# joeyee/Onet

Measured on AMD Instinct MI355X. Metric: training images/sec (twin 256x256 pass), higher is better.
Workload: dtype f32

## Files before the change

include/onet_hip.h:

```cpp
#ifndef ONET_HIP_H
#define ONET_HIP_H

#include <stdint.h>

#ifdef __cplusplus
extern "C" {
#endif

#define ONET_OK 0
#define ONET_EINVAL (-1)
#define ONET_EHIP (-2)

const char* onet_last_error(void);
int onet_abi_version(void);
int onet_device_info(int* cu_count, int* lds_bytes, int* wave_size, char* arch, int arch_len);

int onet_conv3x3_pack_weights(const float* w, float* wp_fwd, float* wp_dgrad,
                              int Cout, int Cin, void* stream);
int onet_convT2x2_pack_weights(const float* w, float* wp_fwd, float* wp_dgrad,
                               int Cin, int Cout, void* stream);
int onet_convT2x2_pack_weights_fused(const float* w, float* wq, int Cin, int Cout, void* stream);
int onet_convT2x2_fwd(const float* x, int64_t x_bs, const float* wq, const float* bias, float* y, int64_t y_bs,
                      int B, int Cin, int Ct, int h, int w, int Ho, int Wo, int pt, int pl, int operand_bf16,
        void* stream);
int onet_convT2x2_dgrad(const float* dy, int64_t dy_bs, const float* wp_dgrad, float* dx, int64_t dx_bs, int B,
                        int Cin, int Ct, int h, int w, int Ho, int Wo, int pt, int pl, int operand_bf16,
        void* stream);
int64_t onet_convT2x2_dgrad_dbias_ws_bytes(int B, int Ct, int h, int w);
int onet_convT2x2_dgrad_dbias(const float* dy, int64_t dy_bs, const float* wp_dgrad, float* dx, int64_t dx_bs, float* dbias,
                              void* ws, int64_t ws_bytes, int B, int Cin, int Ct, int h, int w, int Ho, int Wo, int pt, int pl, int operand_bf16,
        void* stream);
int64_t onet_convT2x2_wgrad_ws_bytes(int B, int Cin, int Ct, int h, int w);
int onet_convT2x2_wgrad(const float* x, int64_t x_bs, const float* dy, int64_t dy_bs, float* dw, void* ws,
                        int64_t ws_bytes, int B, int Cin, int Ct, int h, int w, int Ho, int Wo, int pt, int pl, int operand_bf16,
        void* stream);
int onet_convT2x2_dbias(const float* dy, int64_t dy_bs, float* dbias, double* scratch, int accumulate, int B,
                        int C, int h, int w, int Ho, int Wo, int pt, int pl, void* stream);

int onet_conv_fwd(const float* x, int64_t x_bs, const float* wp, float* z, int64_t z_bs,
                  float* bn_part, int B, int Cin, int Cout, int H, int W, int ks, void* stream);
int onet_conv_fwd_nparts(int B, int Cout, int H, int W);

int onet_conv3x3_pack_weights_winograd4(const float* w, float* wq_fwd, float* wq_dgrad,
                                        int Cout, int Cin, void* stream);
int onet_conv3x3_winograd4_fwd(const float* x, int64_t x_bs, const float* wq, float* z, int64_t z_bs,
                               int B, int Cin, int Cout, int H, int W, void* stream);
int onet_conv3x3_winograd4_nparts(int B, int H, int W);
int onet_conv3x3_winograd4_fwd_stats(const float* x, int64_t x_bs, const float* wq, float* z, int64_t z_bs,
                                     float* part, int B, int Cin, int Cout, int H, int W, void* stream);
int onet_conv3x3_winograd4_dgrad_bnreduce(const float* dz, int64_t dz_bs, const float* wq_dgrad, float* da,
                                          int64_t da_bs, const float* z_prev, int64_t z_prev_bs,
                                          const float* save_prev, int group_images, float* part2,
                                          int B, int Cdz, int Cda, int H, int W, void* stream);
int onet_convT2x2_fwd_p(const float* x, int64_t x_bs, const float* wq, const float* bias, void* yP, int64_t yP_bs, const void* y_amax,
                        int nparts, int B, int Cin, int Ct, int h, int w, int Ho, int Wo, int pt, int pl, int operand_bf16, void* stream);
int onet_convT2x2_pack_weights_slots(const float* w, void* wP, void* wdP, void* amax_ws, int Cin, int Ct, int nparts, void* stream);
int onet_convT2x2_fwd_slots(const void* xP, int64_t xP_bs, const void* x_amax, const void* wP, const float* bias, void* yP, int64_t yP_bs,
                            const void* y_amax, int nparts, int B, int Cin, int Ct, int h, int w, void* stream);
int onet_convT2x2_dgrad_slots(const void* dyP, int64_t dyP_bs, const void* dy_amax, const void* wdP, float* dx, int64_t dx_bs, int nparts, int B,
                              int Cin, int Ct, int h, int w, void* stream);
int64_t onet_convT2x2_wgrad_slots_ws_bytes(int B, int Cin, int Ct, int h, int w);
int onet_convT2x2_wgrad_slots(const void* xP, int64_t xP_bs, const void* x_amax, const void* dyP, int64_t dyP_bs, const void* dy_amax, float* dw,
                              float* dbias, void* ws, int64_t ws_bytes, int nparts, int B, int Cin, int Ct, int h, int w, void* stream);
int onet_convT2x2_out_bound(const float* w, const float* bias, int Cin, int Ct, const void* x_amax, void* y_amax, void* stream);

int onet_conv3x3_split_pack_weights(const float* w, void* wq_fwd, void* wq_dgrad, void* amax_ws, int Cout, int Cin, int fwd_f16,
                                    int dgrad_f16, void* stream);
int onet_absmax_slots(const float* x, int64_t n, void* slots, void* stream);
int onet_conv3x3_split_conv_amax(const float* x, int64_t x_bs, const void* x_amax, int scale_always, const void* wq, float* z, int64_t z_bs,
                                 float* part, int B, int Cin, int Cout, int H, int W, void* stream);
int onet_conv3x3_split_wgrad_f16(const float* x, int64_t x_bs, const void* x_amax, const float* save, int n_groups, const float* dz,
                                 int64_t dz_bs, const void* dz_amax, float* dw, void* ws, int64_t ws_bytes, int B, int Cin, int Cout,
                                 int H, int W, int accumulate, void* stream);
int onet_conv3x3_split_fwd(const float* x, int64_t x_bs, const void* wq, int wq_f16, float* z, int64_t z_bs, int B, int Cin, int Cout,
                           int H, int W, void* stream);
int onet_conv3x3_split_nparts(int B, int H, int W);
int onet_split_pack_act(const float* x, int64_t x_bs, void* xs, int64_t xs_bs, int B, int C, int H, int W, int f16, float scale,
                        const void* slots ,
                        void* stream);
int onet_conv3x3_split_dgrad_pre_bnreduce(const void* dzs, int64_t dzs_bs, const void* dz_amax, int scale_always, const void* wq, int wq_f16,
                                          float* da, int64_t da_bs, const void* z_prev, int z_bf16, int64_t z_bs, const float* save, int group_images,
                                          float* rec4, void* da_amax, int B, int Cin, int Cout, int H, int W, void* stream);
int onet_conv3x3_split_fwd_pre(const void* xs, int64_t xs_bs, const void* x_amax, int scale_always, const void* x_amax2, int split_ch,
                               const void* wq, int wq_f16, void* z, int z_bf16 , int64_t z_bs,
                               float* part, int B, int Cin, int Cout, int H, int W,
                               void* stream);
int onet_conv3x3_split_dgrad_pre_slots(const void* dzs, int64_t dzs_bs, const void* dz_amax, int scale_always, const void* wq, int wq_f16,
                                       float* da, int64_t da_bs, void* daP, int64_t daP_bs, int ch0, const void* daP_amax, int B, int Cin,
                                       int Cout, int H, int W, void* stream);
int onet_conv3x3_dgrad_bound(const float* w, int Cout, int Cin, int ci0, const void* dz_amax, void* out_slots, void* stream);
int onet_conv3x3_split_fwd_pre_act(const void* xs, int64_t xs_bs, const void* x_amax, int scale_always, const void* x_amax2, int split_ch,
                                   const void* wq, const float* save, void* aP, int64_t aP_bs, const void* aP_slots, void* a_amax, float* a,
                                   int64_t a_bs, int B, int Cin, int Cout, int H, int W, void* stream);
int onet_conv3x3_act_bound(const float* w, int Cout, int Cin, const float* save, const void* x_amax, const void* x_amax2, int split_ch,
                           void* out_slots, void* stream);
int onet_conv3x3_plain16_fwd_pre_act(const void* xs, int64_t xs_bs, const void* wq, const float* save, void* aP, int64_t aP_bs, void* a_amax,
                                     float* a, int64_t a_bs, int B, int Cin, int Cout, int H, int W, void* stream);
int onet_conv3x3_plain16_fwd_pre_head(const void* xs, int64_t xs_bs, const void* wq, const float* save, const float* L, int64_t L_bs, float* V,
                                      int B, int Cin, int Cout, int H, int W, void* stream);
int onet_conv3x3_split_fwd_pre_head(const void* xs, int64_t xs_bs, const void* x_amax, int scale_always, const void* x_amax2, int split_ch,
                                    const void* wq, const float* save, const float* L, int64_t L_bs, float* V, int B, int Cin, int Cout, int H,
                                    int W, void* stream);
int onet_softmax2_labels(const float* Vt, const float* Vd, float* S, int64_t* Y, int B, int HW, void* stream);
int onet_conv3x3_split_pre_nparts(int B, int H, int W);
int onet_conv3x3_split_wgrad_pre_ok(int B, int Cin, int Cout, int H, int W);
int onet_conv3x3_split_wgrad_pre(const void* xs, int64_t xs_bs, const void* x_amax, const void* x_amax2, int split_ch, const void* dzs,
                                 int64_t dzs_bs, const void* dz_amax, int f16, float* dw, void* ws, int64_t ws_bytes, int B, int Cin,
                                 int Cout, int H, int W, int accumulate, void* stream);
int onet_conv3x3_split_fwd_stats(const float* x, int64_t x_bs, const void* wq, int wq_f16, float* z, int64_t z_bs, float* part, int B,
                                 int Cin, int Cout, int H, int W, void* stream);
int onet_conv3x3_split_wgrad_ok(int B, int Cin, int Cout, int H, int W);
int onet_conv3x3_split_fwd_norm(const float* z_prev, int64_t z_bs, const float* save, int n_groups, const void* wq, int wq_f16,
                                const void* x_amax, float* z, int64_t zo_bs, float* part, int B, int Cin, int Cout, int H, int W,
                                void* stream);
int onet_conv3x3_split_wgrad_norm(const float* z_prev, int64_t z_bs, const float* save, int n_groups, const float* dz, int64_t dz_bs,
                                  float* dw, void* ws, int64_t ws_bytes, int B, int Cin, int Cout, int H, int W, int accumulate,
                                  void* stream);
int64_t onet_conv3x3_split_wgrad_ws_bytes(int B, int Cin, int Cout, int H, int W);
int onet_conv3x3_split_wgrad(const float* x, int64_t x_bs, const float* dz, int64_t dz_bs, float* dw, void* ws, int64_t ws_bytes,
                             int B, int Cin, int Cout, int H, int W, int accumulate, void* stream);

int onet_conv3x3_stem_nparts(int B, int Cin, int Cout, int H, int W);
int onet_conv3x3_stem_fwd_stats(const float* x, int64_t x_bs, const float* w, float* z, int64_t z_bs, float* part, int B, int Cin,
                                int Cout, int H, int W, int twin_B, float twin_bias, void* stream);

int onet_conv3x3_winograd4_wgrad_ok(int B, int Cin, int Cout, int H, int W);
int64_t onet_conv3x3_winograd4_wgrad_ws_bytes(int B, int Cin, int Cout, int H, int W);
int onet_conv3x3_winograd4_wgrad(const float* x, int64_t x_bs, const float* dz, int64_t dz_bs, float* dw, void* ws,
                                 int64_t ws_bytes, int B, int Cin, int Cout, int H, int W, int accumulate, void* stream);

int onet_conv_wgrad(const float* x, int64_t x_bs, const float* dz, int64_t dz_bs, float* dw,
                    void* ws, int64_t ws_bytes, int B, int Cin, int Cout, int H, int W, int ks,
                    int out_layout, int accumulate, void* stream);
int onet_conv3x3_stem_wgrad_bn(const float* x, int64_t x_bs, const float* da, int64_t da_bs, const float* z, int64_t z_bs, const float* save,
                               const float* coef, int group_images, float* dw, void* ws, int64_t ws_bytes, int B, int Cin, int Cout, int H,
                               int W, int accumulate, int twin_B, float twin_bias, void* stream);
int64_t onet_conv_wgrad_ws_bytes(int B, int Cin, int Cout, int H, int W, int ks);

int onet_bn_stats_partial(const float* z, int64_t z_bs, float* part, int nparts,
                          int B, int C, int HW, void* stream);
int onet_bn_finalize(const float* part, int nparts, int64_t count, const float* gamma, const float* beta, float* running_mean,
                     float* running_var, float momentum, float eps, float* save, void* act_amax, int C, void* stream);
int onet_bn_finalize_cm(const float* part, int nparts, int64_t c_stride, const float* gamma, const float* beta, float* running_mean,
                        float* running_var, float momentum, float eps, float* save, void* act_amax, int groups, int C, void* stream);
int onet_bn_eval_coeffs(const float* gamma, const float* beta, const float* running_mean,
                        const float* running_var, float eps, float* save, int C, void* stream);
int onet_bn_relu_apply(const void* z, int z_bf16, int64_t z_bs, float* a, int64_t a_bs, const float* save, void* amax, int group_images,
                       int B, int C, int HW, void* stream);
int onet_bn_relu_apply_pool(const float* z, int64_t z_bs, float* a, int64_t a_bs, float* y, int64_t y_bs, const float* save,
                            void* amax, int B, int C, int H, int W, void* stream);

int onet_bn_relu_bwd_reduce(const float* da, int64_t da_bs, const void* z, int z_bf16, int64_t z_bs, const float* save, float* part2,
                            int nparts, void* da_amax, int group_images, int B, int C, int HW, void* stream);
int onet_bn_bwd_finalize(const float* part2, int nparts, int64_t count, float* dgamma, float* dbeta, float* coef, int accumulate,
                         int groups, int C, const float* save, const void* da_amax, void* dz_amax, void* stream);
int onet_bn_bwd_finalize_cm(const float* part2, int nparts, int64_t c_stride, int64_t count, float* dgamma,
                            float* dbeta, float* coef, int accumulate, int C, void* stream);
int onet_bn_relu_bwd_apply(const float* da, int64_t da_bs, const float* z, int64_t z_bs, const float* save, const float* coef,
                           float* dz, int64_t dz_bs, void* amax, int group_images, int B, int C, int HW, void* stream);
int onet_bn_relu_apply_split(const void* z, int z_bf16, int64_t z_bs, void* xs, int64_t xs_bs, float* a, int64_t a_bs, const float* save,
                             const void* act_amax, int nparts, int group_images, int B, int C, int H, int W, void* stream);
int onet_bn_relu_apply_pool_split(const void* z, int z_bf16, int64_t z_bs, void* xs, int64_t xs_bs, float* a, int64_t a_bs, void* ys, int64_t ys_bs,
                                  float* y, int64_t y_bs, const float* save, const void* act_amax, int nparts, int group_images, int B, int C,
                                  int H, int W, void* stream);
int onet_bn_bwd_bound(const float* save, const float* coef, const void* da_amax, int64_t count, void* dz_amax, int C, void* stream);
int onet_bn_relu_bwd_apply_split(const float* da, int64_t da_bs, const void* z, int z_bf16, int64_t z_bs, const float* save, const float* coef,
                                 void* dzs, int64_t dzs_bs, const void* dz_amax, int nparts, int group_images, int B, int C, int H, int W,
                                 void* stream);
int onet_bn_relu_bwd_apply_split_gl(const float* L, int64_t L_bs, const float* g, const float* z, int64_t z_bs, const float* save,
                                    const float* coef, void* dzs, int64_t dzs_bs, const void* dz_amax, int nparts, int group_images, int B, int C,
                                    int H, int W, void* stream);

int onet_maxpool2_fwd(const float* x, int64_t x_bs, float* y, int64_t y_bs,
                      int B, int C, int H, int W, void* stream);
int onet_maxpool2_bwd(const float* x, int64_t x_bs, const float* dy, int64_t dy_bs, const float* add, int64_t add_bs,
                      const float* add2, int64_t add2_bs, float* dx, int64_t dx_bs, int B, int C, int H, int W, int accumulate,
                      void* stream);
int onet_maxpool2_bwd_bn_bands(int H, int W);
int onet_maxpool2_bwd_add_bnreduce(const float* x, int64_t x_bs, const float* dy, int64_t dy_bs, const float* add, int64_t add_bs,
                                        const float* add2, int64_t add2_bs, float* dx, int64_t dx_bs, const void* z, int z_bf16, int64_t z_bs,
                                        const float* save, int group_images, float* part2, void* dx_amax, int B, int C, int H, int W,
                                        void* stream);

int onet_pixel_shuffle2_bias(const float* sub, const float* bias, float* y, int64_t y_bs,
                             int B, int C, int h, int w, int Ho, int Wo, int pt, int pl, void* stream);
int onet_space_to_depth2(const float* dy, int64_t dy_bs, float* sub, float* dbias, double* scratch,
                         int accumulate, int B, int C, int h, int w, int Ho, int Wo, int pt, int pl,
                         void* stream);
int onet_copy_strided(const float* src, int64_t src_bs, float* dst, int64_t dst_bs,
                      int B, int64_t n, void* stream);

int onet_bilinear2x_fwd(const float* x, int64_t x_bs, float* y, int64_t y_bs, int B, int C,
                        int h, int w, int Ho, int Wo, int pt, int pl, void* stream);
int onet_bilinear2x_bwd(const float* dy, int64_t dy_bs, float* dx, int64_t dx_bs, int B, int C,
                        int h, int w, int Ho, int Wo, int pt, int pl, void* stream);

int onet_complement_clip(const float* x, float* y, float bias, int64_t n, void* stream);

int onet_head_softmax_fwd(const float* Lt, int64_t Lt_bs, const float* Ht, int64_t Ht_bs, const float* Ld, int64_t Ld_bs, const float* Hd,
                          int64_t Hd_bs, float* Vt, float* Vd, float* S, float* sLt, float* sLd, const float* h_save_t, const float* h_save_d,
                          int B, int C, int HW, void* stream);
int onet_head_softmax_bwd(const float* dVt, const float* dVd, const float* dS, const float* gsLt, const float* gsLd, const float* S,
                          const float* Lt, int64_t Lt_bs, const float* Ht, int64_t Ht_bs, const float* Ld, int64_t Ld_bs, const float* Hd,
                          int64_t Hd_bs, float* dLt, float* dHt, float* dLd, float* dHd, const float* h_save_t, const float* h_save_d, int B,
                          int C, int HW, void* stream);

int onet_head_grad_map(const float* dVt, const float* dVd, const float* dS, const float* S, float* g, int B, int HW, void* stream);
int onet_head_bwd_reduce(const float* L, int64_t L_bs, const float* z, int64_t z_bs, const float* g, const float* gsLt, const float* gsLd,
                         const float* save, float* dL, float* part2, int nparts, void* da_amax, int B, int C, int HW, void* stream);

int onet_jsd_fwd(const float* L, int64_t L_bs, const float* Si, int64_t Si_bs,
                 const float* Sp, int64_t Sp_bs, float* sums, double* part, float* jsd,
                 int B, int C, int HW, void* stream);
int onet_jsd_nparts(void);
int onet_jsd_bwd(const float* gscale, const float* sums, const float* Si, int64_t Si_bs,
                 const float* Sp, int64_t Sp_bs, float* gL, float* dSi, float* dSp,
                 int B, int HW, void* stream);
int onet_log1pexp_inplace(float* x, int64_t n, void* stream);
int onet_log1pexp_bwd(const float* x, const float* g, float* out, int64_t n, void* stream);

// ... 26 lines not shown
```

onet_amd/csrc/common.hpp:

```cpp
#pragma once
#include <hip/hip_runtime.h>
#include <stdint.h>
#include <atomic>
#include <stdio.h>
#include "../../include/onet_hip.h"

namespace onet {

void set_error(const char* fmt, ...);
int check_launch(const char* what);

#define ONET_REQUIRE(cond, ...)                    \
    do {                                           \
        if (!(cond)) {                             \
            onet::set_error(__VA_ARGS__);          \
            return ONET_EINVAL;                    \
        }                                          \
    } while (0)

static inline hipStream_t as_stream(void* s) { return reinterpret_cast<hipStream_t>(s); }

static inline int cdiv(int64_t a, int64_t b) { return (int)((a + b - 1) / b); }

struct PerDeviceOnce {
    std::atomic<uint64_t> seen{0};
    bool first() {
        int d = 0;
        (void)hipGetDevice(&d);
        const uint64_t bit = 1ull << (d & 63);
        return !(seen.fetch_or(bit, std::memory_order_relaxed) & bit);
    }
};

inline int device_cu_count() {
    static std::atomic<int> cached[64];
    int d = 0;
    (void)hipGetDevice(&d);
    int n = cached[d & 63].load(std::memory_order_relaxed);
    if (n <= 0) {
        if (hipDeviceGetAttribute(&n, hipDeviceAttributeMultiprocessorCount, d) != hipSuccess || n <= 0) n = 256;
        cached[d & 63].store(n, std::memory_order_relaxed);
    }
    return n;
}

__device__ __forceinline__ int xcd_block_id() {
    const int n = gridDim.x, q = n >> 3, r = n & 7, xcd = blockIdx.x & 7, j = blockIdx.x >> 3;
    return (xcd < r ? xcd * (q + 1) : r * (q + 1) + (xcd - r) * q) + j;
}

template <typename T>
__device__ __forceinline__ T wave_sum(T v) {
#pragma unroll
    for (int o = 32; o > 0; o >>= 1) v += __shfl_xor(v, o, 64);
    return v;
}

template <typename T, int NV>
__device__ __forceinline__ void block_sum_256(T (&v)[NV], T* smem ) {
    const int lane = threadIdx.x & 63, wid = threadIdx.x >> 6;
#pragma unroll
    for (int i = 0; i < NV; ++i) v[i] = wave_sum(v[i]);
    if (lane == 0) {
#pragma unroll
        for (int i = 0; i < NV; ++i) smem[wid * NV + i] = v[i];
    }
    __syncthreads();
    if (threadIdx.x == 0) {
#pragma unroll
        for (int i = 0; i < NV; ++i) v[i] = smem[i] + smem[NV + i] + smem[2 * NV + i] + smem[3 * NV + i];
    }
}

__device__ __forceinline__ void split2h_s(float a, float b, float s, unsigned& hi, unsigned& mid) {
    unsigned h, m;
    asm("v_fma_mixlo_f16 %0, %1, %3, 0 op_sel_hi:[0,0,0]\n\tv_fma_mixhi_f16 %0, %2, %3, 0 op_sel_hi:[0,0,0]"
        : "=&v"(h) : "v"(a), "v"(b), "v"(s));
    asm("v_fma_mixlo_f16 %0, %1, %3, -%4 op_sel:[0,0,0] op_sel_hi:[0,0,1]\n\tv_fma_mixhi_f16 %0, %2, %3, -%4 op_sel:[0,0,1] op_sel_hi:[0,0,1]"
        : "=&v"(m) : "v"(a), "v"(b), "v"(s), "v"(h));
    hi = h;
    mid = m;
}

constexpr int AMAX_SLOTS = 64, AMAX_STRIDE = 32;
__device__ __forceinline__ float amax_read(const unsigned* slots) {
    if (!slots) return 0.f;
    unsigned v = slots[(threadIdx.x & (AMAX_SLOTS - 1)) * AMAX_STRIDE];
#pragma unroll
    for (int o = 32; o > 0; o >>= 1) v = max(v, (unsigned)__shfl_xor((int)v, o, 64));
    return __builtin_bit_cast(float, __builtin_amdgcn_readfirstlane(v));
}
__device__ __forceinline__ float amax_scale(float amax, bool always, float& inv) {
    const unsigned bits = __builtin_bit_cast(unsigned, amax);
    const int e = (int)((bits >> 23) & 255u) - 127;
    int k = 0;
    if (bits != 0u && e < 128) k = (always || e >= 15) ? 13 - e : 0;
    k = max(-100, min(100, k));
    inv = __builtin_bit_cast(float, (unsigned)(127 - k) << 23);
    return __builtin_bit_cast(float, (unsigned)(127 + k) << 23);
}

int launch_wgrad_reduce(const float* slab, float* dw, int splitK, int taps, int Cout, int Cin, int out_layout, int accumulate,
                        hipStream_t st);

int convt_gemm_fwd(const float* x, int64_t x_bs, const float* wq, const float* bias, float* y, int64_t y_bs, void* y16, int64_t y16_bs,
                   int B, int Cin, int Ct, int h, int w, int Ho, int Wo, int pt, int pl, int prec, hipStream_t st, int y16_split = 0,
                   const void* out_slots = nullptr);
int convt_out_bound(const float* w, const float* bias, int Cin, int Ct, const void* x_slots, void* out_slots, hipStream_t st);
int64_t convt_gemm_dbias_ws_bytes(int B, int Ct, int h, int w);
int convt_gemm_dgrad(const float* dy, int64_t dy_bs, const float* wd, float* dx, int64_t dx_bs, float* dbias, float* dbias_ws, int B,
                     int Cin, int Ct, int h, int w, int Ho, int Wo, int pt, int pl, int prec, hipStream_t st);
int64_t convt_gemm_wgrad_ws_bytes(int B, int Cin, int Ct, int h, int w);
int convt_gemm_wgrad(const float* x, int64_t x_bs, const float* dy, int64_t dy_bs, float* dw, void* ws, int64_t ws_bytes, int B,
                     int Cin, int Ct, int h, int w, int Ho, int Wo, int pt, int pl, int prec, hipStream_t st);

}
```

onet_amd/csrc/conv_mfma.hip:

```cpp
#include <algorithm>
#include <cstdlib>
#include "common.hpp"

using namespace onet;

typedef float f32x16 __attribute__((ext_vector_type(16)));

__global__ void pack3x3_kernel(const float* __restrict__ w, float* __restrict__ wf,
                               float* __restrict__ wd, int Cout, int Cin) {
    int64_t n = (int64_t)Cout * Cin * 9;
    for (int64_t i = blockIdx.x * (int64_t)blockDim.x + threadIdx.x; i < n;
         i += (int64_t)gridDim.x * blockDim.x) {
        int t = (int)(i % 9);
        int64_t r = i / 9;
        int ci = (int)(r % Cin), co = (int)(r / Cin);
        float v = w[i];
        if (wf) wf[((int64_t)ci * 9 + t) * Cout + co] = v;
        if (wd) wd[((int64_t)co * 9 + (8 - t)) * Cin + ci] = v;
    }
}

__global__ void packT2x2_kernel(const float* __restrict__ w, float* __restrict__ wf,
                                float* __restrict__ wd, float* __restrict__ wq, int Cin, int Cout) {
    int64_t n = (int64_t)Cin * Cout * 4;
// ... 339 lines not shown
__global__ __launch_bounds__(256 * KS, KS == 3 ? 3 : 2) void conv_wgrad_kernel(WgArgs a) {
    using C = WgCfg<KS, PW>;
    constexpr int TAPS = C::TAPS, PAD = C::PAD, PR = C::PR, XR = C::XR, XC = C::XC;
    constexpr int DZ_STRIDE = C::DZ_STRIDE, X_STRIDE = C::X_STRIDE;
    constexpr int TG = KS;
    constexpr int NTAP = TAPS / TG;
    constexpr int NTHR = 256 * TG;
    constexpr int DZ_CSTEP = NTHR / 64;
    constexpr int NDZ = (64 + DZ_CSTEP - 1) / DZ_CSTEP;
    constexpr int ROWS_PER_K = NTHR / PW;
    constexpr int CH_PER_K = ROWS_PER_K / XR;
    constexpr int NXM = (64 + CH_PER_K - 1) / CH_PER_K;
    constexpr int NXH = (KS == 3) ? (64 * XR * 2 + NTHR - 1) / NTHR : 0;

    extern __shared__ __attribute__((aligned(16))) float smem[];
    float* dz_lds = smem;
    float* x_lds = smem + 64 * DZ_STRIDE;

    int bid = xcd_block_id();
    const int tiles = a.ciTiles * a.coTiles;
    const int ks = bid / tiles;
    const int tile = bid % tiles;
    const int ciT = tile % a.ciTiles;
    const int coT = tile / a.ciTiles;
    const int co0 = coT * 64, ci0 = ciT * 64;

    const int tid = threadIdx.x, lane = tid & 63, wid = tid >> 6;
    const int tg = wid >> 2, wm = (wid >> 1) & 1, wn = wid & 1;
    const int l31 = lane & 31, kh = lane >> 5;
    const int HW = a.H * a.W;

    f32x16 acc[NTAP];
#pragma unroll
    for (int t = 0; t < NTAP; ++t)
#pragma unroll
        for (int r = 0; r < 16; ++r) acc[t][r] = 0.f;

    const float* a_ptr = dz_lds + (wm * 32 + l31) * DZ_STRIDE + kh;
    const float* b_ptr = x_lds + (wn * 32 + l31) * X_STRIDE + kh + tg * XC;

    const int dz_c = tid >> 6, dz_p = tid & 63, dz_r = dz_p / PW, dz_col = dz_p % PW;
    const int xm_col = tid % PW, xm_rowid = tid / PW, xm_cp = xm_rowid / XR, xm_r = xm_rowid % XR;
    const bool xm_thread = xm_rowid < CH_PER_K * XR;
    const unsigned dz_kstep = (unsigned)(DZ_CSTEP * HW * 4), xm_kstep = (unsigned)(CH_PER_K * HW * 4);

    float dzv[NDZ], xmv[NXM], xhv[NXH > 0 ? NXH : 1];
    const int nunits = a.B * a.stripsY * a.stripsX;

    auto issue = [&](int u) {
        const bool live = u < nunits;
        const int uu = live ? u : 0;
        const int sx = uu % a.stripsX;
        const int sy = (uu / a.stripsX) % a.stripsY;
        const int b = uu / (a.stripsX * a.stripsY);
        const int y0 = sy * PR, x0 = sx * PW;
        const int HWo = a.Ho * a.Wo;
        const __amdgpu_buffer_rsrc_t dr = make_rsrc(a.dz + (int64_t)b * a.dz_bs, S2D ? (int64_t)a.s2d_Ct * HWo * 4 : (int64_t)a.Cout * HW * 4);
        const __amdgpu_buffer_rsrc_t xr = make_rsrc(a.x + (int64_t)b * a.x_bs, (int64_t)a.Cin * HW * 4);
        {
            const int yy = y0 + dz_r, xx = x0 + dz_col;
            const bool ok = live && yy < a.H && xx < a.W;
            unsigned base, kstep;
            if constexpr (S2D) {
                const int q = co0 / a.s2d_Ct, cc = co0 % a.s2d_Ct + dz_c;
                base = ok ? (unsigned)((cc * HWo + (a.pt + 2 * yy + (q >> 1)) * a.Wo + a.pl + 2 * xx + (q & 1)) * 4) : OOB_OFF;
                kstep = (unsigned)(DZ_CSTEP * HWo * 4);
            } else {
                base = ok ? (unsigned)(((co0 + dz_c) * HW + yy * a.W + xx) * 4) : OOB_OFF;
                kstep = dz_kstep;
            }
#pragma unroll
            for (int k = 0; k < NDZ; ++k)
                dzv[k] = bload(dr, (ok && dz_c + DZ_CSTEP * k < 64) ? base + k * kstep : OOB_OFF);
        }
        {
            const int yy = y0 - PAD + xm_r, xx = x0 + xm_col;
            const bool ok = live && xm_thread && yy >= 0 && yy < a.H && xx < a.W;
            const unsigned base = ok ? (unsigned)(((ci0 + xm_cp) * HW + yy * a.W + xx) * 4) : OOB_OFF;
#pragma unroll
            for (int k = 0; k < NXM; ++k)
                xmv[k] = bload(xr, (xm_cp + CH_PER_K * k < 64) ? base + k * xm_kstep : OOB_OFF);
        }
#pragma unroll
        for (int j = 0; j < NXH; ++j) {
            const int e = tid + NTHR * j;
            const int c = e / (2 * XR), q = e % (2 * XR);
            const int r = q >> 1, side = q & 1;
            const int yy = y0 - PAD + r, xx = side ? x0 + PW : x0 - 1;
            const bool ok = live && e < 64 * XR * 2 && yy >= 0 && yy < a.H && xx >= 0 && xx < a.W;
            xhv[j] = bload(xr, ok ? (unsigned)(((ci0 + c) * HW + yy * a.W + xx) * 4) : OOB_OFF);
        }
    };
    auto commit = [&]() {
#pragma unroll
        for (int k = 0; k < NDZ; ++k)
            if (dz_c + DZ_CSTEP * k < 64) dz_lds[(dz_c + DZ_CSTEP * k) * DZ_STRIDE + dz_p] = dzv[k];
        if (xm_thread) {
#pragma unroll
            for (int k = 0; k < NXM; ++k)
                if (xm_cp + CH_PER_K * k < 64)
                    x_lds[(xm_cp + CH_PER_K * k) * X_STRIDE + xm_r * XC + xm_col + PAD] = xmv[k];
        }
#pragma unroll
        for (int j = 0; j < NXH; ++j) {
            const int e = tid + NTHR * j;
            const int c = e / (2 * XR), q = e % (2 * XR);
            if (e < 64 * XR * 2) x_lds[c * X_STRIDE + (q >> 1) * XC + ((q & 1) ? XC - 1 : 0)] = xhv[j];
        }
    };

    issue(ks);
    for (int u = ks; u < nunits; u += a.splitK) {
        commit();
        __syncthreads();
        issue(u + a.splitK);
        __builtin_amdgcn_sched_barrier(0);
#pragma unroll
        for (int r = 0; r < PR; ++r) {
#pragma unroll
            for (int j = 0; j < PW / 2; ++j) {
                const float av = a_ptr[r * PW + 2 * j];
#pragma unroll
                for (int t = 0; t < NTAP; ++t) {
                    const float bv = b_ptr[r * XC + 2 * j + t];
                    acc[t] = __builtin_amdgcn_mfma_f32_32x32x2f32(av, bv, acc[t], 0, 0, 0);
                }
            }
        }
        __syncthreads();
    }
    float* sl = a.slab + (int64_t)ks * TAPS * a.Cout * a.Cin;
    const int ci = ci0 + wn * 32 + l31;
    if (ci < a.Cin) {
#pragma unroll
        for (int t = 0; t < NTAP; ++t) {
#pragma unroll
            for (int r = 0; r < 16; ++r) {
                const int co = co0 + wm * 32 + (r & 3) + 8 * (r >> 2) + 4 * kh;
                if (co < a.Cout) sl[((int64_t)(tg * NTAP + t) * a.Cout + co) * a.Cin + ci] = acc[t][r];
            }
        }
    }
}

__global__ __launch_bounds__(256) void wgrad_reduce_kernel(const float* __restrict__ slab, float* __restrict__ dw,
                                                           int splitK, int taps, int Cout, int Cin, int out_layout,
                                                           int accumulate) {
    __shared__ float red[256];
    const int64_t n = (int64_t)Cout * Cin;
    const int t = blockIdx.y;
    const int64_t i = (int64_t)blockIdx.x * 64 + (threadIdx.x & 63);
    const int g = threadIdx.x >> 6;
    float s = 0.f;
    if (i < n)
        for (int k = g; k < splitK; k += 4) s += slab[((int64_t)k * taps + t) * n + i];
    red[threadIdx.x] = s;
    __syncthreads();
    if (g == 0 && i < n) {
        s = (red[threadIdx.x] + red[threadIdx.x + 64]) + (red[threadIdx.x + 128] + red[threadIdx.x + 192]);
        const int ci = (int)(i % Cin), co = (int)(i / Cin);
        int64_t o;
        if (out_layout == 0) {
            o = i * taps + t;
        } else {
            const int Ct = Cout / 4, q = co / Ct, cot = co % Ct;
            o = ((int64_t)ci * Ct + cot) * 4 + q;
        }
        dw[o] = accumulate ? dw[o] + s : s;
    }
}

namespace onet {
int launch_wgrad_reduce(const float* slab, float* dw, int splitK, int taps, int Cout, int Cin, int out_layout, int accumulate,
                        hipStream_t st) {
    const int64_t n = (int64_t)Cout * Cin;
    hipLaunchKernelGGL(wgrad_reduce_kernel, dim3((unsigned)cdiv(n, 64), (unsigned)taps), dim3(256), 0, st, slab, dw, splitK,
                       taps, Cout, Cin, out_layout, accumulate);
    return check_launch("wgrad_reduce_kernel");
}
}

constexpr int STEM_ROWS = 32;
template <int CIN, int COG, bool BN = false>
__global__ __launch_bounds__(256) void conv3x3_stem_wgrad_kernel(WgArgs a) {
    constexpr int NV = COG * CIN * 9;
    __shared__ float red[4][NV];
    const int cogs = (a.Cout + COG - 1) / COG;
    const int bandsY = (a.H + STEM_ROWS - 1) / STEM_ROWS;
    const int cg = blockIdx.x % cogs, bb = blockIdx.x / cogs;
    const int b = bb / bandsY, yb = (bb % bandsY) * STEM_ROWS;
    const int tid = threadIdx.x, lane = tid & 63, wid = tid >> 6;
    const int HW = a.H * a.W, W = a.W, H = a.H;
    const bool comp = a.twin_B > 0 && b >= a.twin_B;
    const float* xb = a.x + (int64_t)(comp ? b - a.twin_B : b) * a.x_bs;
    const float* dzb = a.dz + (int64_t)b * a.dz_bs + (int64_t)cg * COG * HW;
    const float* zb = BN ? a.bn_z + (int64_t)b * a.bn_z_bs + (int64_t)cg * COG * HW : nullptr;
    const int y0 = yb + wid * (STEM_ROWS / 4), y1 = min(y0 + STEM_ROWS / 4, H);
    const bool vec = (W & 3) == 0 && (a.dz_bs & 3) == 0 && (reinterpret_cast<uintptr_t>(a.dz) & 15) == 0 &&
                     (!BN || ((a.bn_z_bs & 3) == 0 && (reinterpret_cast<uintptr_t>(a.bn_z) & 15) == 0));
    float bmean[COG], binv[COG], bsc[COG], bsh[COG];
    double bc1[COG], bc2[COG];
    if (BN) {
        const int grp = a.bn_gimg ? b / a.bn_gimg : 0;
        const float* sv = a.bn_save + (int64_t)grp * 4 * a.Cout;
        const float* cf = a.bn_coef ? a.bn_coef + (int64_t)grp * 4 * a.Cout : nullptr;
#pragma unroll
        for (int g = 0; g < COG; ++g) {
            const int c = min(cg * COG + g, a.Cout - 1);
            bmean[g] = sv[c];
            binv[g] = sv[a.Cout + c];
            bsc[g] = sv[2 * a.Cout + c];
            bsh[g] = sv[3 * a.Cout + c];
            bc1[g] = cf ? (double)cf[c] + (double)cf[a.Cout + c] : 0.0;
            bc2[g] = cf ? (double)cf[2 * a.Cout + c] + (double)cf[3 * a.Cout + c] : 0.0;
        }
    }
    float acc[COG][CIN][9];
#pragma unroll
    for (int g = 0; g < COG; ++g)
#pragma unroll
        for (int c = 0; c < CIN; ++c)
#pragma unroll
            for (int t = 0; t < 9; ++t) acc[g][c][t] = 0.f;
    auto in_row = [&](int c, int yy, int x0, float (&r)[6]) __attribute__((always_inline)) {
        const bool rowok = yy >= 0 && yy < H;
        const float* p = xb + (int64_t)c * HW + (int64_t)yy * W;
#pragma unroll
        for (int k = 0; k < 6; ++k) {
            const int xx = x0 - 1 + k;
            const bool ok = rowok && xx >= 0 && xx < W;
            float v = ok ? p[xx] : 0.f;
            if (comp && ok) v = fminf(fmaxf(1.f - v + a.twin_bias, 0.f), 1.f);
            r[k] = v;
        }
    };
    for (int x0 = lane * 4; x0 < W && y0 < y1; x0 += 256) {
        float win[CIN][3][6];
#pragma unroll
        for (int c = 0; c < CIN; ++c) {
            in_row(c, y0 - 1, x0, win[c][1]);
            in_row(c, y0, x0, win[c][2]);
        }
        for (int y = y0; y < y1; ++y) {
#pragma unroll
            for (int c = 0; c < CIN; ++c) {
#pragma unroll
                for (int k = 0; k < 6; ++k) {
                    win[c][0][k] = win[c][1][k];
                    win[c][1][k] = win[c][2][k];
                }
                in_row(c, y + 1, x0, win[c][2]);
            }
#pragma unroll
            for (int g = 0; g < COG; ++g) {
                float gz[4] = {0.f, 0.f, 0.f, 0.f}, zz[4] = {0.f, 0.f, 0.f, 0.f};
                if (cg * COG + g < a.Cout) {
                    const int64_t o = (int64_t)g * HW + (int64_t)y * W + x0;
                    if (vec) {
                        const float4 q = *reinterpret_cast<const float4*>(dzb + o);
                        gz[0] = q.x; gz[1] = q.y; gz[2] = q.z; gz[3] = q.w;
                        if (BN) {
                            const float4 r = *reinterpret_cast<const float4*>(zb + o);
                            zz[0] = r.x; zz[1] = r.y; zz[2] = r.z; zz[3] = r.w;
                        }
                    } else {
#pragma unroll
                        for (int p = 0; p < 4; ++p)
                            if (x0 + p < W) {
                                gz[p] = dzb[o + p];
                                if (BN) zz[p] = zb[o + p];
                            }
                    }
                    if (BN) {
#pragma unroll
                        for (int p = 0; p < 4; ++p) {
                            const double dy = fmaf(zz[p] - bmean[g], bsc[g], bsh[g]) > 0.f ? (double)gz[p] : 0.0;
                            const float v = (float)((double)bsc[g] * (dy - bc1[g] - (((double)zz[p] - (double)bmean[g]) * (double)binv[g]) * bc2[g]));
                            gz[p] = (vec || x0 + p < W) ? v : 0.f;
                        }
                    }
                }
#pragma unroll
                for (int p = 0; p < 4; ++p)
#pragma unroll
                    for (int c = 0; c < CIN; ++c)
#pragma unroll
                        for (int t = 0; t < 9; ++t) acc[g][c][t] = fmaf(gz[p], win[c][t / 3][p + t % 3], acc[g][c][t]);
            }
        }
    }
#pragma unroll
    for (int g = 0; g < COG; ++g)
#pragma unroll
        for (int c = 0; c < CIN; ++c)
#pragma unroll
            for (int t = 0; t < 9; ++t) {
                const float s = wave_sum(acc[g][c][t]);
                if (lane == 0) red[wid][(g * CIN + c) * 9 + t] = s;
            }
    __syncthreads();
    float* sl = a.slab + (int64_t)bb * 9 * a.Cout * CIN;
    for (int i = tid; i < NV; i += 256) {
        const int g = i / (CIN * 9), c = (i / 9) % CIN, t = i % 9;
        const int co = cg * COG + g;
        if (co < a.Cout)
            sl[((int64_t)t * a.Cout + co) * CIN + c] = (red[0][i] + red[1][i]) + (red[2][i] + red[3][i]);
    }
}

template <int KS, int PW, bool S2D = false>
static void launch_wgrad(const WgArgs& a, int64_t blocks, hipStream_t st) {
    using C = WgCfg<KS, PW>;
    auto kern = conv_wgrad_kernel<KS, PW, S2D>;
    static PerDeviceOnce attr_once;
    if (attr_once.first()) {
        (void)hipFuncSetAttribute(reinterpret_cast<const void*>(kern), hipFuncAttributeMaxDynamicSharedMemorySize,
                                  C::LDS_BYTES);
    }
    hipLaunchKernelGGL(kern, dim3((unsigned)blocks), dim3(256 * KS), C::LDS_BYTES, st, a);
}

static void wgrad_plan(int B, int Cin, int Cout, int H, int W, int ks, int& pw, int& splitK,
                       int& stripsX, int& stripsY) {
    pw = (W > 16) ? 32 : 16;
    const int pr = 64 / pw;
    stripsX = cdiv(W, pw);
    stripsY = cdiv(H, pr);
    const int64_t nunits = (int64_t)B * stripsX * stripsY;
    const int64_t tiles = (int64_t)cdiv(Cout, 64) * cdiv(Cin, 64);
    int64_t s = (1024 + tiles - 1) / tiles;
// ... 1 lines not shown
    const int64_t cap = (192ll << 20) / (per > 0 ? per : 1);
    if (s > cap) s = cap;
    if (s > nunits) s = nunits;
    if (s < 1) s = 1;
    splitK = (int)s;
}

extern "C" {

int onet_conv3x3_pack_weights(const float* w, float* wp_fwd, float* wp_dgrad, int Cout, int Cin,
                              void* stream) {
    ONET_REQUIRE(w && Cout > 0 && Cin > 0, "pack3x3: bad args");
    const int64_t n = (int64_t)Cout * Cin * 9;
    hipLaunchKernelGGL(pack3x3_kernel, dim3((unsigned)std::min<int64_t>(cdiv(n, 256), 4096)), dim3(256), 0,
                       as_stream(stream), w, wp_fwd, wp_dgrad, Cout, Cin);
    return check_launch("pack3x3_kernel");
}

int onet_convT2x2_pack_weights(const float* w, float* wp_fwd, float* wp_dgrad, int Cin, int Cout,
                               void* stream) {
    ONET_REQUIRE(w && Cout > 0 && Cin > 0, "packT2x2: bad args");
    const int64_t n = (int64_t)Cout * Cin * 4;
    hipLaunchKernelGGL(packT2x2_kernel, dim3((unsigned)std::min<int64_t>(cdiv(n, 256), 4096)), dim3(256), 0,
                       as_stream(stream), w, wp_fwd, wp_dgrad, (float*)nullptr, Cin, Cout);
    return check_launch("packT2x2_kernel");
}

int onet_convT2x2_pack_weights_fused(const float* w, float* wq, int Cin, int Cout, void* stream) {
    ONET_REQUIRE(w && wq && Cout > 0 && Cin > 0, "packT2x2_fused: bad args");
    const int64_t n = (int64_t)Cout * Cin * 4;
    hipLaunchKernelGGL(packT2x2_kernel, dim3((unsigned)std::min<int64_t>(cdiv(n, 256), 4096)), dim3(256), 0,
                       as_stream(stream), w, (float*)nullptr, (float*)nullptr, wq, Cin, Cout);
    return check_launch("packT2x2_kernel");
}

static bool convt_gemm_enabled() {
    static int on = -1;
    if (on < 0) { const char* e = getenv("ONET_CONVT_GEMM"); on = (e && e[0] == '0') ? 0 : 1; }
    return on != 0;
}

int64_t onet_convT2x2_wgrad_ws_bytes(int B, int Cin, int Ct, int h, int w) {
    return std::max<int64_t>(onet_conv_wgrad_ws_bytes(B, Cin, 4 * Ct, h, w, 1), convt_gemm_wgrad_ws_bytes(B, Cin, Ct, h, w));
}

int onet_convT2x2_fwd(const float* x, int64_t x_bs, const float* wq, const float* bias, float* y, int64_t y_bs,
                      int B, int Cin, int Ct, int h, int w, int Ho, int Wo, int pt, int pl, int operand_bf16, void* stream) {
    ONET_REQUIRE(x && wq && y, "convT2x2_fwd: null pointer");
    ONET_REQUIRE(B > 0 && Cin > 0 && Ct > 0 && h > 0 && w > 0, "convT2x2_fwd: bad shape");
    ONET_REQUIRE(pt >= 0 && pl >= 0 && pt + 2 * h <= Ho && pl + 2 * w <= Wo, "convT2x2_fwd: window outside plane");
    ONET_REQUIRE(x_bs >= (int64_t)Cin * h * w && y_bs >= (int64_t)Ct * Ho * Wo, "convT2x2_fwd: batch stride too small");
    if (convt_gemm_enabled()) {
        const int rc = convt_gemm_fwd(x, x_bs, wq, bias, y, y_bs, nullptr, 0, B, Cin, Ct, h, w, Ho, Wo, pt, pl, operand_bf16, as_stream(stream));
        if (rc <= 0) return rc;
    }
    ConvArgs a{x, x_bs, wq, y, y_bs, nullptr, B, Cin, 4 * Ct, h, w, 0, 0, 0, bias, Ho, Wo, pt, pl};
    return (w > 16) ? launch_fwd<1, 2, 2, 1, 4, 32, 1>(a, as_stream(stream))
                    : launch_fwd<1, 2, 2, 1, 4, 16, 1>(a, as_stream(stream));
}

int onet_convT2x2_fwd_p(const float* x, int64_t x_bs, const float* wq, const float* bias, void* yP, int64_t yP_bs, const void* y_amax,
                        int nparts, int B, int Cin, int Ct, int h, int w, int Ho, int Wo, int pt, int pl, int operand_bf16, void* stream) {
    ONET_REQUIRE(x && wq && yP && B > 0 && Cin > 0 && Ct > 0 && h > 0 && w > 0 && (nparts == 1 || nparts == 2), "convT2x2_fwd_p: bad args");
    return convt_gemm_fwd(x, x_bs, wq, bias, nullptr, 0, yP, yP_bs, B, Cin, Ct, h, w, Ho, Wo, pt, pl, operand_bf16, as_stream(stream),
                          nparts == 1 ? 2 : 1, y_amax);
}

int onet_convT2x2_out_bound(const float* w, const float* bias, int Cin, int Ct, const void* x_amax, void* y_amax, void* stream) {
    ONET_REQUIRE(w && x_amax && y_amax && Cin > 0 && Ct > 0 && (reinterpret_cast<uintptr_t>(w) & 15) == 0, "convT2x2_out_bound: bad args");
    return convt_out_bound(w, bias, Cin, Ct, x_amax, y_amax, as_stream(stream));
}

int onet_convT2x2_dgrad(const float* dy, int64_t dy_bs, const float* wp_dgrad, float* dx, int64_t dx_bs, int B,
                        int Cin, int Ct, int h, int w, int Ho, int Wo, int pt, int pl, int operand_bf16, void* stream) {
    ONET_REQUIRE(dy && wp_dgrad && dx, "convT2x2_dgrad: null pointer");
    ONET_REQUIRE(B > 0 && Cin > 0 && Ct > 0 && h > 0 && w > 0, "convT2x2_dgrad: bad shape");
    ONET_REQUIRE(Ct % CI_T == 0, "convT2x2_dgrad: Ct must be a multiple of %d (use onet_space_to_depth2 + onet_conv_fwd)", CI_T);
    ONET_REQUIRE(pt >= 0 && pl >= 0 && pt + 2 * h <= Ho && pl + 2 * w <= Wo, "convT2x2_dgrad: window outside plane");
    ONET_REQUIRE(dy_bs >= (int64_t)Ct * Ho * Wo && dx_bs >= (int64_t)Cin * h * w, "convT2x2_dgrad: batch stride too small");
    if (convt_gemm_enabled()) {
        const int rc = convt_gemm_dgrad(dy, dy_bs, wp_dgrad, dx, dx_bs, nullptr, nullptr, B, Cin, Ct, h, w, Ho, Wo, pt, pl, operand_bf16, as_stream(stream));
        if (rc <= 0) return rc;
    }
    ConvArgs a{dy, dy_bs, wp_dgrad, dx, dx_bs, nullptr, B, 4 * Ct, Cin, h, w, 0, 0, 0, nullptr, Ho, Wo, pt, pl};
    return (w > 16) ? launch_fwd<1, 2, 2, 1, 4, 32, 2>(a, as_stream(stream))
                    : launch_fwd<1, 2, 2, 1, 4, 16, 2>(a, as_stream(stream));
}

int64_t onet_convT2x2_dgrad_dbias_ws_bytes(int B, int Ct, int h, int w) { return convt_gemm_dbias_ws_bytes(B, Ct, h, w); }

int onet_convT2x2_dgrad_dbias(const float* dy, int64_t dy_bs, const float* wp_dgrad, float* dx, int64_t dx_bs, float* dbias, void* ws,
                              int64_t ws_bytes, int B, int Cin, int Ct, int h, int w, int Ho, int Wo, int pt, int pl, int operand_bf16, void* stream) {
    ONET_REQUIRE(dy && wp_dgrad && dx && dbias && ws, "convT2x2_dgrad_dbias: null pointer");
    ONET_REQUIRE(B > 0 && Cin > 0 && Ct > 0 && h > 0 && w > 0, "convT2x2_dgrad_dbias: bad shape");
    ONET_REQUIRE(dy_bs >= (int64_t)Ct * Ho * Wo && dx_bs >= (int64_t)Cin * h * w, "convT2x2_dgrad_dbias: batch stride too small");
    if (!convt_gemm_enabled() || ws_bytes < convt_gemm_dbias_ws_bytes(B, Ct, h, w)) return 1;
    return convt_gemm_dgrad(dy, dy_bs, wp_dgrad, dx, dx_bs, dbias, (float*)ws, B, Cin, Ct, h, w, Ho, Wo, pt, pl, operand_bf16, as_stream(stream));
}

int onet_conv_fwd_nparts(int B, int Cout, int H, int W) {
    (void)B; (void)Cout; (void)H; (void)W;
    return 0;
}

int onet_conv_fwd(const float* x, int64_t x_bs, const float* wp, float* z, int64_t z_bs, float* bn_part,
                  int B, int Cin, int Cout, int H, int W, int ks, void* stream) {
    ONET_REQUIRE(x && wp && z, "conv_fwd: null pointer");
    ONET_REQUIRE(B > 0 && Cin > 0 && Cout > 0 && H > 0 && W > 0, "conv_fwd: bad shape B=%d Cin=%d Cout=%d H=%d W=%d",
                 B, Cin, Cout, H, W);
    ONET_REQUIRE(ks == 1 || ks == 3, "conv_fwd: ks must be 1 or 3 (got %d)", ks);
    ONET_REQUIRE(bn_part == nullptr, "conv_fwd: fused BN partials not available in this build");
    ONET_REQUIRE(x_bs >= (int64_t)Cin * H * W && z_bs >= (int64_t)Cout * H * W, "conv_fwd: batch stride too small");
    ConvArgs a{x, x_bs, wp, z, z_bs, bn_part, B, Cin, Cout, H, W, 0, 0, 0};
    return ks == 3 ? dispatch_fwd<3>(a, as_stream(stream)) : dispatch_fwd<1>(a, as_stream(stream));
}

static inline bool use_stem_wgrad(int Cin, int ks) { return ks == 3 && Cin <= 4; }
static inline int stem_blocks(int B, int H) { return B * ((H + STEM_ROWS - 1) / STEM_ROWS); }

int64_t onet_conv_wgrad_ws_bytes(int B, int Cin, int Cout, int H, int W, int ks) {
    if (use_stem_wgrad(Cin, ks)) return (int64_t)stem_blocks(B, H) * 9 * Cout * Cin * 4;
    int pw, splitK, sx, sy;
    wgrad_plan(B, Cin, Cout, H, W, ks, pw, splitK, sx, sy);
    return (int64_t)splitK * ks * ks * Cout * Cin * 4;
}

int onet_conv3x3_stem_wgrad_bn(const float* x, int64_t x_bs, const float* da, int64_t da_bs, const float* z, int64_t z_bs, const float* save,
                               const float* coef, int group_images, float* dw, void* ws, int64_t ws_bytes, int B, int Cin, int Cout, int H,
                               int W, int accumulate, int twin_B, float twin_bias, void* stream) {
    ONET_REQUIRE(x && da && z && save && dw && ws, "conv3x3_stem_wgrad_bn: null pointer");
    ONET_REQUIRE(B > 0 && Cin > 0 && Cin <= 4 && Cout > 0 && H > 0 && W > 0 && group_images >= 0 && (group_images == 0 || B % group_images == 0),
                 "conv3x3_stem_wgrad_bn: bad shape (Cin <= 4)");
    WgArgs a{x, x_bs, da, da_bs, (float*)ws, B, Cin, Cout, H, W, 1, cdiv(Cout, 64), 1, 1, 1};
    a.bn_z = z;
    a.bn_z_bs = z_bs;
    a.bn_save = save;
    a.bn_coef = coef;
    a.bn_gimg = group_images;
    ONET_REQUIRE(twin_B == 0 || 2 * twin_B == B, "conv3x3_stem_wgrad_bn: a twin batch holds twin_B = B / 2 images in memory");
    a.twin_B = twin_B;
    a.twin_bias = twin_bias;
    const int nb = stem_blocks(B, H);
    const int64_t need = (int64_t)nb * 9 * Cout * Cin * 4;
    ONET_REQUIRE(ws_bytes >= need, "conv3x3_stem_wgrad_bn: workspace %lld < %lld bytes", (long long)ws_bytes, (long long)need);
    hipStream_t st = as_stream(stream);
    switch (Cin) {
        case 1: hipLaunchKernelGGL((conv3x3_stem_wgrad_kernel<1, 4, true>), dim3(nb * cdiv(Cout, 4)), dim3(256), 0, st, a); break;
        case 2: hipLaunchKernelGGL((conv3x3_stem_wgrad_kernel<2, 2, true>), dim3(nb * cdiv(Cout, 2)), dim3(256), 0, st, a); break;
        case 3: hipLaunchKernelGGL((conv3x3_stem_wgrad_kernel<3, 2, true>), dim3(nb * cdiv(Cout, 2)), dim3(256), 0, st, a); break;
        default: hipLaunchKernelGGL((conv3x3_stem_wgrad_kernel<4, 1, true>), dim3(nb * cdiv(Cout, 1)), dim3(256), 0, st, a); break;
    }
    int rc = check_launch("conv3x3_stem_wgrad_kernel");
    if (rc) return rc;
    const int64_t n = (int64_t)Cout * Cin;
    hipLaunchKernelGGL(wgrad_reduce_kernel, dim3((unsigned)cdiv(n, 64), 9u), dim3(256), 0, st, (const float*)ws, dw, nb, 9, Cout, Cin, 0, accumulate);
    return check_launch("wgrad_reduce_kernel");
}

int onet_conv_wgrad(const float* x, int64_t x_bs, const float* dz, int64_t dz_bs, float* dw, void* ws,
                    int64_t ws_bytes, int B, int Cin, int Cout, int H, int W, int ks, int out_layout,
                    int accumulate, void* stream) {
    ONET_REQUIRE(x && dz && dw && ws, "conv_wgrad: null pointer");
    ONET_REQUIRE(B > 0 && Cin > 0 && Cout > 0 && H > 0 && W > 0, "conv_wgrad: bad shape");
    ONET_REQUIRE(ks == 1 || ks == 3, "conv_wgrad: ks must be 1 or 3 (got %d)", ks);
    ONET_REQUIRE(out_layout == 0 || (out_layout == 1 && ks == 1 && Cout % 4 == 0), "conv_wgrad: bad out_layout");
    WgArgs a{x, x_bs, dz, dz_bs, (float*)ws, B, Cin, Cout, H, W, cdiv(Cin, 64), cdiv(Cout, 64), 1, 1, 1};
    if (use_stem_wgrad(Cin, ks) && out_layout == 0) {
        const int nb = stem_blocks(B, H);
        const int64_t need = (int64_t)nb * 9 * Cout * Cin * 4;
        ONET_REQUIRE(ws_bytes >= need, "conv_wgrad(stem): workspace %lld < %lld bytes", (long long)ws_bytes, (long long)need);
        hipStream_t st = as_stream(stream);
        switch (Cin) {
            case 1: hipLaunchKernelGGL((conv3x3_stem_wgrad_kernel<1, 4>), dim3(nb * cdiv(Cout, 4)), dim3(256), 0, st, a); break;
            case 2: hipLaunchKernelGGL((conv3x3_stem_wgrad_kernel<2, 2>), dim3(nb * cdiv(Cout, 2)), dim3(256), 0, st, a); break;
            case 3: hipLaunchKernelGGL((conv3x3_stem_wgrad_kernel<3, 2>), dim3(nb * cdiv(Cout, 2)), dim3(256), 0, st, a); break;
            default: hipLaunchKernelGGL((conv3x3_stem_wgrad_kernel<4, 1>), dim3(nb * cdiv(Cout, 1)), dim3(256), 0, st, a); break;
        }
        int rc = check_launch("conv3x3_stem_wgrad_kernel");
        if (rc) return rc;
        const int64_t n = (int64_t)Cout * Cin;
        hipLaunchKernelGGL(wgrad_reduce_kernel, dim3((unsigned)cdiv(n, 64), 9u), dim3(256), 0, st,
                           (const float*)ws, dw, nb, 9, Cout, Cin, 0, accumulate);
        return check_launch("wgrad_reduce_kernel");
    }
    int pw;
    wgrad_plan(B, Cin, Cout, H, W, ks, pw, a.splitK, a.stripsX, a.stripsY);
    const int64_t need = (int64_t)a.splitK * ks * ks * Cout * Cin * 4;
    ONET_REQUIRE(ws_bytes >= need, "conv_wgrad: workspace %lld < %lld bytes", (long long)ws_bytes, (long long)need);
    const int64_t blocks = (int64_t)a.splitK * a.ciTiles * a.coTiles;
    hipStream_t st = as_stream(stream);
    if (ks == 3) {
        if (pw == 32) launch_wgrad<3, 32>(a, blocks, st); else launch_wgrad<3, 16>(a, blocks, st);
    } else {
        if (pw == 32) launch_wgrad<1, 32>(a, blocks, st); else launch_wgrad<1, 16>(a, blocks, st);
    }
    int rc = check_launch("conv_wgrad_kernel");
    if (rc) return rc;
    const int64_t n = (int64_t)Cout * Cin;
    hipLaunchKernelGGL(wgrad_reduce_kernel, dim3((unsigned)cdiv(n, 64), (unsigned)(ks * ks)), dim3(256), 0, st,
                       (const float*)ws, dw, a.splitK, ks * ks, Cout, Cin, out_layout, accumulate);
    return check_launch("wgrad_reduce_kernel");
}

int onet_convT2x2_wgrad(const float* x, int64_t x_bs, const float* dy, int64_t dy_bs, float* dw, void* ws,
                        int64_t ws_bytes, int B, int Cin, int Ct, int h, int w, int Ho, int Wo, int pt, int pl, int operand_bf16,
                        void* stream) {
    ONET_REQUIRE(x && dy && dw && ws, "convT2x2_wgrad: null pointer");
    ONET_REQUIRE(B > 0 && Cin > 0 && Ct > 0 && h > 0 && w > 0, "convT2x2_wgrad: bad shape");
    ONET_REQUIRE(Ct % 64 == 0, "convT2x2_wgrad: Ct must be a multiple of 64 (use onet_space_to_depth2 + onet_conv_wgrad)");
    ONET_REQUIRE(pt >= 0 && pl >= 0 && pt + 2 * h <= Ho && pl + 2 * w <= Wo, "convT2x2_wgrad: window outside plane");
    ONET_REQUIRE(dy_bs >= (int64_t)Ct * Ho * Wo && x_bs >= (int64_t)Cin * h * w, "convT2x2_wgrad: batch stride too small");
    if (convt_gemm_enabled()) {
        const int rc = convt_gemm_wgrad(x, x_bs, dy, dy_bs, dw, ws, ws_bytes, B, Cin, Ct, h, w, Ho, Wo, pt, pl, operand_bf16, as_stream(stream));
        if (rc <= 0) return rc;
    }
    const int Cout = 4 * Ct;
    WgArgs a{x, x_bs, dy, dy_bs, (float*)ws, B, Cin, Cout, h, w, cdiv(Cin, 64), cdiv(Cout, 64), 1, 1, 1, Ct, Ho, Wo, pt, pl};
    int pw;
    wgrad_plan(B, Cin, Cout, h, w, 1, pw, a.splitK, a.stripsX, a.stripsY);
    const int64_t need = (int64_t)a.splitK * Cout * Cin * 4;
    ONET_REQUIRE(ws_bytes >= need, "convT2x2_wgrad: workspace %lld < %lld bytes", (long long)ws_bytes, (long long)need);
    const int64_t blocks = (int64_t)a.splitK * a.ciTiles * a.coTiles;
    hipStream_t st = as_stream(stream);
    if (pw == 32) launch_wgrad<1, 32, true>(a, blocks, st); else launch_wgrad<1, 16, true>(a, blocks, st);
    int rc = check_launch("conv_wgrad_kernel");
    if (rc) return rc;
    const int64_t n = (int64_t)Cout * Cin;
    hipLaunchKernelGGL(wgrad_reduce_kernel, dim3((unsigned)cdiv(n, 64), 1u), dim3(256), 0, st, (const float*)ws, dw,
                       a.splitK, 1, Cout, Cin, 1, 0);
    return check_launch("wgrad_reduce_kernel");
}

}
```

onet_amd/csrc/conv_split.hip:

```cpp
#include <algorithm>
#include <cstdlib>
#include "common.hpp"

using namespace onet;

typedef float f32x16 __attribute__((ext_vector_type(16)));
typedef __bf16 bf16x8 __attribute__((ext_vector_type(8)));
typedef __bf16 bf16x2 __attribute__((ext_vector_type(2)));
typedef unsigned int u32x4s __attribute__((ext_vector_type(4)));
typedef float f32x4s __attribute__((ext_vector_type(4)));

namespace {

constexpr unsigned OOB_S = 0x80000000u;

__device__ __forceinline__ __amdgpu_buffer_rsrc_t s_rsrc(const void* base, int64_t bytes) {
    const int n = bytes > 0x7fffffffll ? 0x7fffffff : (int)bytes;
    return __builtin_amdgcn_make_buffer_rsrc(const_cast<void*>(base), 0, n, 0x00020000);
}
__device__ __forceinline__ void split2(float a, float b, unsigned& hi, unsigned& mid) {
    const bf16x2 h = {(__bf16)a, (__bf16)b};
    const bf16x2 m = {(__bf16)(a - (float)h[0]), (__bf16)(b - (float)h[1])};
    hi = __builtin_bit_cast(unsigned, h);
    mid = __builtin_bit_cast(unsigned, m);
}

typedef _Float16 f16x2 __attribute__((ext_vector_type(2)));
typedef _Float16 f16x8 __attribute__((ext_vector_type(8)));
__device__ __forceinline__ unsigned pack2bf(float lo, float hi) {
    const bf16x2 v = {(__bf16)lo, (__bf16)hi};
    return __builtin_bit_cast(unsigned, v);
}
__device__ __forceinline__ void split2h(float a, float b, unsigned& hi, unsigned& mid) {
    const f16x2 h = {(_Float16)a, (_Float16)b};
    const f16x2 m = {(_Float16)(a - (float)h[0]), (_Float16)(b - (float)h[1])};
    hi = __builtin_bit_cast(unsigned, h);
    mid = __builtin_bit_cast(unsigned, m);
}

__global__ void absmax_slots_kernel(const float* __restrict__ v, int64_t n, unsigned* __restrict__ slots) {
    float m = 0.f;
    for (int64_t i = blockIdx.x * (int64_t)blockDim.x + threadIdx.x; i < n; i += (int64_t)gridDim.x * blockDim.x) m = fmaxf(m, fabsf(v[i]));
#pragma unroll
    for (int o = 32; o > 0; o >>= 1) m = fmaxf(m, __shfl_xor(m, o, 64));
    if ((threadIdx.x & 63) == 0)
        atomicMax(slots + ((blockIdx.x * (blockDim.x >> 6) + (threadIdx.x >> 6)) & (AMAX_SLOTS - 1)) * AMAX_STRIDE, __builtin_bit_cast(unsigned, m));
}

__global__ void pack3x3_split_kernel(const float* __restrict__ w, __bf16* __restrict__ wq, int Cout, int Cin, int which, int f16,
                                     const unsigned* __restrict__ wamax) {
    const int K = which == 0 ? Cin : ((Cout + 15) / 16) * 16, N = which == 0 ? Cout : Cin;
    const int64_t n = (int64_t)K * 9 * N;
    const int nparts = f16 == 2 ? 1 : 2;
    float winv = 1.f;
    const float wscale = f16 == 1 ? amax_scale(amax_read(wamax), true, winv) : 1.f;
    if (blockIdx.x == 0 && threadIdx.x == 0) {
        float* meta = reinterpret_cast<float*>(wq + nparts * n);
        meta[0] = wscale;
        meta[1] = winv;
    }
    for (int64_t i = blockIdx.x * (int64_t)blockDim.x + threadIdx.x; i < n; i += (int64_t)gridDim.x * blockDim.x) {
        const int kc = (int)(i & 7);
        int64_t r = i >> 3;
        const int nn = (int)(r % N);
        r /= N;
        const int half = (int)(r & 1);
        r >>= 1;
        const int t = (int)(r % 9), kg = (int)(r / 9);
        const int k = kg * 16 + half * 8 + kc;
        float v = 0.f;
        if (which == 0) v = w[((int64_t)nn * Cin + k) * 9 + t];
        else if (k < Cout) v = w[((int64_t)k * Cin + nn) * 9 + (8 - t)];
        const int64_t per_chunk_part = (int64_t)9 * 2 * N * 8;
        const int64_t within = i - (int64_t)kg * per_chunk_part;
        if (f16 == 2) {
            wq[(int64_t)kg * per_chunk_part + within] = (__bf16)v;
        } else if (f16) {
            _Float16* wh = reinterpret_cast<_Float16*>(wq);
            const float vs = v * wscale;
            const _Float16 hi = (_Float16)vs;
            wh[((int64_t)kg * 2 + 0) * per_chunk_part + within] = hi;
            wh[((int64_t)kg * 2 + 1) * per_chunk_part + within] = (_Float16)(vs - (float)hi);
        } else {
            const __bf16 hi = (__bf16)v;
            wq[((int64_t)kg * 2 + 0) * per_chunk_part + within] = hi;
            wq[((int64_t)kg * 2 + 1) * per_chunk_part + within] = (__bf16)(v - (float)hi);
        }
    }
}

struct SpArgs {
    const float* x;
    int64_t x_bs;
    const __bf16* wq;
    float* z;
    int64_t z_bs;
    int B, Cin, Cout, H, W, tilesX, tilesY, coTiles;
    float* stats;
    const float* nsave;
    int nimg;
    const unsigned* x_amax;
    int x_always;
};

#define ONET_SP_DPP_ADD(v, ctrl, rmask) \
    v += __builtin_bit_cast(float, __builtin_amdgcn_update_dpp(0, __builtin_bit_cast(int, v), ctrl, rmask, 0xf, false))
__device__ __forceinline__ float sp_half_sum(float v) {
    ONET_SP_DPP_ADD(v, 0x128, 0xf);
    ONET_SP_DPP_ADD(v, 0x124, 0xf);
    ONET_SP_DPP_ADD(v, 0x122, 0xf);
    ONET_SP_DPP_ADD(v, 0x121, 0xf);
    ONET_SP_DPP_ADD(v, 0x142, 0xa);
    return v;
}
#undef ONET_SP_DPP_ADD

struct SpCfg {
    static constexpr int NW = 8, NT = 2, TW = 32, CO_T = 64;
    static constexpr int ROWS = NW * NT;
    static constexpr int IN_ROWS = ROWS + 2, IN_COLS = TW + 2;
    static constexpr int NPIX = IN_ROWS * IN_COLS;
    static constexpr int NROUND = (NPIX + 31) / 32;
    static constexpr int NPIXP = NROUND * 32;
    static constexpr int W_PART = 9 * 2 * CO_T;
    static constexpr int W_SLOTS = 2 * W_PART;
    static constexpr int NWI = (W_SLOTS + 511) / 512;
    static constexpr int IN_PART = 2 * NPIXP;
    static constexpr int BUF_SLOTS = W_SLOTS + 2 * IN_PART;
    static constexpr int LDS_BYTES = 2 * BUF_SLOTS * 16;
    static constexpr int NB = (NT - 1) + 3;
};


__device__ __forceinline__ void sp_tile_range(int ntiles, int& t_first, int& t_end, int& t_stride) {
    const int xcd = blockIdx.x & 7, j = blockIdx.x >> 3;
    const int q = ntiles >> 3, r = ntiles & 7;
    const int start = xcd * q + min(xcd, r);
    t_stride = (gridDim.x + 7 - xcd) >> 3;
    t_first = start + j;
    t_end = start + q + (xcd < r ? 1 : 0);
}
struct SpTile {
    int co0, tx, ty, b, y0, x0;
};
__device__ __forceinline__ SpTile sp_tile(int v, int coTiles, int tilesX, int tilesY) {
    SpTile t;
    t.co0 = (v % coTiles) * SpCfg::CO_T;
    v /= coTiles;
    t.tx = v % tilesX;
    v /= tilesX;
    t.ty = v % tilesY;
    t.b = v / tilesY;
    t.y0 = t.ty * SpCfg::ROWS;
    t.x0 = t.tx * SpCfg::TW;
    return t;
}

template <bool ST, bool NORM, bool F16>
__global__ __launch_bounds__(512, 2) void conv3x3_split_kernel(SpArgs a) {
    using C = SpCfg;
    constexpr int NT = C::NT, IN_COLS = C::IN_COLS, NWI = C::NWI, CO_T = C::CO_T, NPIXP = C::NPIXP, NB = C::NB;
    constexpr int BUF = C::BUF_SLOTS, W_PART = C::W_PART, IN_PART = C::IN_PART, TW = C::TW;
    extern __shared__ __attribute__((aligned(16))) unsigned char smem_s[];
    u32x4s* lds = reinterpret_cast<u32x4s*>(smem_s);

    int t_first, t_end, t_stride;
    sp_tile_range(a.tilesX * a.tilesY * a.B * a.coTiles, t_first, t_end, t_stride);
    if (t_first >= t_end) return;

    const int tid = threadIdx.x, lane = tid & 63, wn = __builtin_amdgcn_readfirstlane(tid >> 6);
    const int l31 = lane & 31, kh = lane >> 5;
    const int HW = a.H * a.W;
    const int nchunks = a.Cin >> 4;
    float xs_inv = 1.f;
    const float xs_scale = F16 ? amax_scale(amax_read(a.x_amax), a.x_always != 0, xs_inv) : 1.f;
    const float acc_scale = F16 ? xs_inv * reinterpret_cast<const float*>(a.wq + (int64_t)a.Cin * 2 * 9 * a.Cout)[1] : 1.f;

    const __amdgpu_buffer_rsrc_t wr = s_rsrc(a.wq, (int64_t)a.Cin * 2 * 9 * a.Cout * 2);
    const unsigned in_step = (unsigned)(16 * HW * 4), w_step = (unsigned)(2 * 9 * 2 * a.Cout * 16);
    const unsigned plane = (unsigned)(HW * 4);

    unsigned in_off, w_off[NWI];
    const int role = wn < 5 ? 0 : (wn < 7 ? 1 : 2);
    const int it = role == 0 ? tid : tid - 320;
    const int it_h = role == 0 ? it / 144 : it / 36;
    const int it_r = role == 0 ? (it % 144) / 8 : (it % 36) / 2;
    const int it_g = role == 0 ? (it & 7) : (it & 1);
    const bool it_ok = role == 0 ? it < 288 : (role == 1 && it < 72);
    __amdgpu_buffer_rsrc_t xr;
    int st_tile = t_first, st_chunk = 0, st_b = 0;
    unsigned cin_bytes = 0, cw_bytes = 0;
    float* const coef = reinterpret_cast<float*>(lds + 2 * BUF) + (ST ? C::NW * 64 * 2 : 0);
    float pend_cv = 0.f;
    bool pend_keep = false;
    auto setup_stage = [&]() __attribute__((always_inline)) {
        const bool live = st_tile < t_end;
        const auto [co0, tx, ty, b, y0, x0] = sp_tile(live ? st_tile : t_first, a.coTiles, a.tilesX, a.tilesY);
        st_b = b;
        xr = s_rsrc(a.x + (int64_t)b * a.x_bs, (int64_t)a.Cin * HW * 4);
        {
            const int yy = y0 - 1 + it_r;
            const int xx = role == 0 ? x0 + 4 * it_g : (it_g ? x0 + TW : x0 - 1);
            const bool ok = live && it_ok && yy >= 0 && yy < a.H && xx >= 0 && xx < a.W;
            in_off = ok ? (unsigned)(((it_h * 8) * HW + yy * a.W + xx) * 4) : OOB_S;
        }
#pragma unroll
        for (int k = 0; k < NWI; ++k) {
            const int i = tid + 512 * k;
            const int co = i & (CO_T - 1), pth = i >> 6;
            const bool ok = live && (i < C::W_SLOTS) && (co0 + co < a.Cout);
            w_off[k] = ok ? (unsigned)((pth * a.Cout + co0 + co) * 16) : OOB_S;
        }
    };
    auto advance = [&]() __attribute__((always_inline)) {
        ++st_chunk;
        cin_bytes += in_step;
        cw_bytes += w_step;
        if (st_chunk == nchunks) {
            st_chunk = 0;
            cin_bytes = cw_bytes = 0;
            st_tile += t_stride;
            setup_stage();
        }
    };

    u32x4s xin[8];
    u32x4s wv[NWI];
    auto issue_in = [&](int c0, int c1) __attribute__((always_inline)) {
        if (NORM && c0 == 0) {
            pend_keep = in_off != OOB_S;
            if (wn == 7 && lane < 48) {
                const int k = lane >> 4, row = k == 0 ? 0 : k + 1;
                pend_cv = st_tile < t_end ? a.nsave[(int64_t)((st_b / a.nimg) * 4 + row) * a.Cin + st_chunk * 16 + (lane & 15)] : 0.f;
            }
        }
        if (role == 0) {
#pragma unroll
            for (int c = 0; c < 8; ++c)
                if (c >= c0 && c < c1) xin[c] = __builtin_amdgcn_raw_buffer_load_b128(xr, in_off, (int)(cin_bytes + c * plane), 0);
        } else if (role == 1) {
// ... 1755 lines not shown
extern "C" {

int onet_conv3x3_split_wgrad_ok(int B, int Cin, int Cout, int H, int W) {
    if (B <= 0 || Cin <= 0 || Cout <= 0 || H <= 0) return 0;
    if (W >= 64) return (W & 3) == 0 ? 1 : 0;
    return ((W == 32 || W == 16) && B % (64 / W) == 0) ? 1 : 0;
}

int64_t onet_conv3x3_split_wgrad_ws_bytes(int B, int Cin, int Cout, int H, int W) {
    int splitK, tx;
    split_wgrad_plan(B, Cin, Cout, H, W, splitK, tx);
    return (int64_t)splitK * (split_wgrad_cot(Cout, W) == 64 ? 2 : 1) * 9 * Cout * Cin * 4;
}

static int split_wgrad_impl(const float* x, int64_t x_bs, const float* dz, int64_t dz_bs, float* dw, void* ws, int64_t ws_bytes,
                            int B, int Cin, int Cout, int H, int W, int accumulate, void* stream, const float* nsave, int n_groups,
                            int f16 = 0, const unsigned* x_amax = nullptr, const unsigned* dz_amax = nullptr) {
    ONET_REQUIRE(x && dz && dw && ws, "conv3x3_split_wgrad: null pointer");
    ONET_REQUIRE(!nsave || ((n_groups == 1 || n_groups == 2) && B % n_groups == 0),
                 "conv3x3_split_wgrad_norm: one or two statistics groups of equal size");
    ONET_REQUIRE(onet_conv3x3_split_wgrad_ok(B, Cin, Cout, H, W),
                 "conv3x3_split_wgrad: needs W >= 64 with W %% 4 == 0, or W = 32 / 16 with B %% (64 / W) == 0 (use onet_conv3x3_winograd_wgrad)");
    ONET_REQUIRE((x_bs & 3) == 0 && (dz_bs & 3) == 0 && (reinterpret_cast<uintptr_t>(x) & 15) == 0 && (reinterpret_cast<uintptr_t>(dz) & 15) == 0,
                 "conv3x3_split_wgrad: 16-byte aligned image rows required");
    ONET_REQUIRE(x_bs >= (int64_t)Cin * H * W && dz_bs >= (int64_t)Cout * H * W, "conv3x3_split_wgrad: batch stride too small");
    ONET_REQUIRE((int64_t)std::max(Cin, Cout) * H * W * 4 < (1ll << 31), "conv3x3_split_wgrad: image exceeds the 2 GiB buffer-resource range");
    const int G = split_wgrad_group(W);
    ONET_REQUIRE(G == 1 || (((int64_t)(B - 1) * x_bs + (int64_t)Cin * H * W) * 4 < (1ll << 31) &&
                            ((int64_t)(B - 1) * dz_bs + (int64_t)Cout * H * W) * 4 < (1ll << 31)),
                 "conv3x3_split_wgrad: on maps narrower than 64 pixels the whole batch must lie within the 2 GiB buffer-resource range");
    const int COT = split_wgrad_cot(Cout, W), slabs = COT == 64 ? 2 : 1;
    ONET_REQUIRE(!f16 || dz_amax, "conv3x3_split_wgrad_f16: the fp16 parts need the magnitude slots of dz");
    SwArgs a{x, x_bs, dz, dz_bs, (float*)ws, B, Cin, Cout, H, W, cdiv(Cin, 64), cdiv(Cout, COT), 1, 1, nsave, nsave ? B / n_groups : B,
             x_amax, dz_amax};
    split_wgrad_plan(B, Cin, Cout, H, W, a.splitK, a.tilesX);
    const int64_t need = (int64_t)a.splitK * slabs * 9 * Cout * Cin * 4;
    ONET_REQUIRE(ws_bytes >= need, "conv3x3_split_wgrad: workspace %lld < %lld bytes", (long long)ws_bytes, (long long)need);
    const int64_t blocks = (int64_t)a.splitK * a.ciTiles * a.coTiles;
    const dim3 grid((unsigned)blocks), blk(512);
    hipStream_t st = as_stream(stream);
#define ONET_SW_LAUNCH(G_, COT_)                                                                                      \
    do {                                                                                                              \
        if (nsave && f16) hipLaunchKernelGGL((conv3x3_split_wgrad_kernel<G_, COT_, true, true>), grid, blk, 0, st, a);    \
        else if (nsave) hipLaunchKernelGGL((conv3x3_split_wgrad_kernel<G_, COT_, true, false>), grid, blk, 0, st, a);     \
        else if (f16) hipLaunchKernelGGL((conv3x3_split_wgrad_kernel<G_, COT_, false, true>), grid, blk, 0, st, a);       \
        else hipLaunchKernelGGL((conv3x3_split_wgrad_kernel<G_, COT_, false, false>), grid, blk, 0, st, a);               \
    } while (0)
    if (COT == 128) {
        if (G == 1) ONET_SW_LAUNCH(1, 128);
        else ONET_SW_LAUNCH(2, 128);
    } else if (G == 1) ONET_SW_LAUNCH(1, 64);
    else if (G == 2) ONET_SW_LAUNCH(2, 64);
    else ONET_SW_LAUNCH(4, 64);
#undef ONET_SW_LAUNCH
    int rc = check_launch("conv3x3_split_wgrad_kernel");
    if (rc) return rc;
    return launch_wgrad_reduce((const float*)ws, dw, a.splitK * slabs, 9, Cout, Cin, 0, accumulate, as_stream(stream));
}

int onet_conv3x3_split_wgrad(const float* x, int64_t x_bs, const float* dz, int64_t dz_bs, float* dw, void* ws, int64_t ws_bytes,
                             int B, int Cin, int Cout, int H, int W, int accumulate, void* stream) {
    return split_wgrad_impl(x, x_bs, dz, dz_bs, dw, ws, ws_bytes, B, Cin, Cout, H, W, accumulate, stream, nullptr, 0);
}

int onet_conv3x3_split_wgrad_norm(const float* z_prev, int64_t z_bs, const float* save, int n_groups, const float* dz, int64_t dz_bs,
                                  float* dw, void* ws, int64_t ws_bytes, int B, int Cin, int Cout, int H, int W, int accumulate,
                                  void* stream) {
    ONET_REQUIRE(save, "conv3x3_split_wgrad_norm: null pointer");
    return split_wgrad_impl(z_prev, z_bs, dz, dz_bs, dw, ws, ws_bytes, B, Cin, Cout, H, W, accumulate, stream, save, n_groups);
}

int onet_conv3x3_split_wgrad_pre_ok(int B, int Cin, int Cout, int H, int W) {
    if (B <= 0 || Cin <= 0 || Cout <= 0 || H <= 0 || (Cin % 8) || (Cout % 8)) return 0;
    if (W >= 64) return 1;
    return ((W == 32 && B % 2 == 0) || (W == 16 && B % 4 == 0)) ? 1 : 0;
}

int onet_conv3x3_split_wgrad_pre(const void* xs, int64_t xs_bs, const void* x_amax, const void* x_amax2, int split_ch, const void* dzs,
                                 int64_t dzs_bs, const void* dz_amax, int f16, float* dw, void* ws, int64_t ws_bytes, int B, int Cin,
                                 int Cout, int H, int W, int accumulate, void* stream) {
    ONET_REQUIRE(split_ch >= 0 && split_ch < Cin && (split_ch % 64) == 0, "conv3x3_split_wgrad_pre: split_ch must be a multiple of 64 inside Cin");
    ONET_REQUIRE(xs && dzs && dw && ws, "conv3x3_split_wgrad_pre: null pointer");
    ONET_REQUIRE(onet_conv3x3_split_wgrad_pre_ok(B, Cin, Cout, H, W),
                 "conv3x3_split_wgrad_pre: needs Cin, Cout %% 8 == 0 and W >= 64, or W = 32 / 16 with a batch multiple of 2 / 4");
    ONET_REQUIRE((xs_bs & 3) == 0 && (dzs_bs & 3) == 0 && (reinterpret_cast<uintptr_t>(xs) & 15) == 0 && (reinterpret_cast<uintptr_t>(dzs) & 15) == 0,
                 "conv3x3_split_wgrad_pre: 16-byte aligned slots required");
    ONET_REQUIRE(xs_bs >= (int64_t)Cin * H * W / (f16 == 2 ? 2 : 1) && dzs_bs >= (int64_t)Cout * H * W / (f16 == 2 ? 2 : 1),
                 "conv3x3_split_wgrad_pre: batch stride too small");
    ONET_REQUIRE((int64_t)std::max(Cin, Cout) * H * W * 4 < (1ll << 31), "conv3x3_split_wgrad_pre: image exceeds the 2 GiB buffer-resource range");
    const int G = split_wgrad_group(W);
    ONET_REQUIRE(G == 1 || (((int64_t)(B - 1) * xs_bs + (int64_t)Cin * H * W) * 4 < (1ll << 31) &&
                            ((int64_t)(B - 1) * dzs_bs + (int64_t)Cout * H * W) * 4 < (1ll << 31)),
                 "conv3x3_split_wgrad_pre: on 32-pixel maps the whole batch must lie within the 2 GiB buffer-resource range");
    const int COT = split_wgrad_cot(Cout, W), slabs = COT == 64 ? 2 : 1;
    SwPreArgs a{xs, xs_bs, dzs, dzs_bs, (float*)ws, B, Cin, Cout, H, W, cdiv(Cin, 64), cdiv(Cout, COT), 1, 1, (const unsigned*)x_amax,
                (const unsigned*)dz_amax, (const unsigned*)x_amax2, split_ch};
    split_wgrad_plan(B, Cin, Cout, H, W, a.splitK, a.tilesX);
    const int64_t need = (int64_t)a.splitK * slabs * 9 * Cout * Cin * 4;
    ONET_REQUIRE(ws_bytes >= need, "conv3x3_split_wgrad_pre: workspace %lld < %lld bytes", (long long)ws_bytes, (long long)need);
    const int64_t blocks = (int64_t)a.splitK * a.ciTiles * a.coTiles;
    const dim3 grid((unsigned)blocks), blk(512);
    hipStream_t st = as_stream(stream);
    const int np = f16 == 2 ? 1 : 2, pxp = G == 4 ? 76 : SWP_PXP;
    const int lds = (4 * ((np * 8 * pxp + 63) / 64 * 64) + 2 * ((np * (COT / 8) * pxp + 63) / 64 * 64)) * 16;
#define ONET_SWP_LAUNCH(G_, COT_, F_)                                                                              \
    do {                                                                                                           \
        auto kern = conv3x3_wgrad_pre16_kernel<G_, COT_, F_>;                                                      \
        static PerDeviceOnce once;                                                                                 \
        if (once.first()) (void)hipFuncSetAttribute(reinterpret_cast<const void*>(kern), hipFuncAttributeMaxDynamicSharedMemorySize, lds); \
        hipLaunchKernelGGL(kern, grid, blk, lds, st, a);                                                           \
    } while (0)
#define ONET_SWP_F(G_, COT_) do { if (f16 == 2) ONET_SWP_LAUNCH(G_, COT_, 2); else if (f16) ONET_SWP_LAUNCH(G_, COT_, 1); else ONET_SWP_LAUNCH(G_, COT_, 0); } while (0)
    if (COT == 128) {
        if (G == 1) ONET_SWP_F(1, 128);
        else if (G == 2) ONET_SWP_F(2, 128);
        else ONET_SWP_F(4, 128);
    } else if (G == 1) ONET_SWP_F(1, 64);
    else if (G == 2) ONET_SWP_F(2, 64);
    else ONET_SWP_F(4, 64);
#undef ONET_SWP_F
#undef ONET_SWP_LAUNCH
    int rc = check_launch("conv3x3_split_wgrad_pre_kernel");
    if (rc) return rc;
    return launch_wgrad_reduce((const float*)ws, dw, a.splitK * slabs, 9, Cout, Cin, 0, accumulate, as_stream(stream));
}

int onet_conv3x3_split_pack_weights(const float* w, void* wq_fwd, void* wq_dgrad, void* amax_ws, int Cout, int Cin, int fwd_f16,
                                    int dgrad_f16, void* stream) {
    ONET_REQUIRE(w && (wq_fwd || wq_dgrad), "conv3x3_split_pack_weights: null pointer");
    ONET_REQUIRE(amax_ws || !(fwd_f16 == 1 || dgrad_f16 == 1), "conv3x3_split_pack_weights: the fp16 packs need the 8 KB magnitude workspace");
    if (fwd_f16 == 1 || dgrad_f16 == 1) {
        (void)hipMemsetAsync(amax_ws, 0, AMAX_SLOTS * AMAX_STRIDE * sizeof(unsigned), as_stream(stream));
        const int64_t nw = (int64_t)Cout * Cin * 9;
        hipLaunchKernelGGL(absmax_slots_kernel, dim3((unsigned)std::min<int64_t>((nw + 1023) / 1024, 1024)), dim3(256), 0, as_stream(stream), w,
                           nw, (unsigned*)amax_ws);
        int rc0 = check_launch("absmax_slots_kernel");
        if (rc0) return rc0;
    }
    ONET_REQUIRE(Cout > 0 && Cin > 0, "conv3x3_split_pack_weights: bad shape");
    ONET_REQUIRE(!wq_fwd || (Cin % 16) == 0, "conv3x3_split_pack_weights: the forward pack needs Cin %% 16 == 0");
    const int64_t n = (int64_t)std::max(Cin, ((Cout + 15) / 16) * 16) * 9 * std::max(Cin, Cout);
    const int blocks = (int)std::min<int64_t>((n + 255) / 256, 8192);
    if (wq_fwd) {
        hipLaunchKernelGGL(pack3x3_split_kernel, dim3(blocks), dim3(256), 0, as_stream(stream), w, (__bf16*)wq_fwd, Cout, Cin, 0, fwd_f16,
                           (const unsigned*)amax_ws);
        int rc = check_launch("pack3x3_split_kernel");
        if (rc) return rc;
    }
    if (wq_dgrad) hipLaunchKernelGGL(pack3x3_split_kernel, dim3(blocks), dim3(256), 0, as_stream(stream), w, (__bf16*)wq_dgrad, Cout, Cin, 1,
                                     dgrad_f16, (const unsigned*)amax_ws);
    return check_launch("pack3x3_split_kernel");
}

int onet_conv3x3_split_fwd(const float* x, int64_t x_bs, const void* wq, int wq_f16, float* z, int64_t z_bs, int B, int Cin, int Cout,
                           int H, int W, void* stream) {
    return split_fwd(x, x_bs, wq, z, z_bs, B, Cin, Cout, H, W, stream, nullptr, wq_f16);
}

int onet_absmax_slots(const float* x, int64_t n, void* slots, void* stream) {
    ONET_REQUIRE(x && slots && n > 0, "absmax_slots: bad args");
    hipLaunchKernelGGL(absmax_slots_kernel, dim3((unsigned)std::min<int64_t>((n + 1023) / 1024, 4096)), dim3(256), 0, as_stream(stream), x, n,
                       (unsigned*)slots);
    return check_launch("absmax_slots_kernel");
}

int onet_conv3x3_split_conv_amax(const float* x, int64_t x_bs, const void* x_amax, int scale_always, const void* wq, float* z, int64_t z_bs,
                                 float* part, int B, int Cin, int Cout, int H, int W, void* stream) {
    return split_fwd(x, x_bs, wq, z, z_bs, B, Cin, Cout, H, W, stream, part, 1, nullptr, 0, (const unsigned*)x_amax, scale_always);
}

int onet_conv3x3_split_wgrad_f16(const float* x, int64_t x_bs, const void* x_amax, const float* save, int n_groups, const float* dz,
                                 int64_t dz_bs, const void* dz_amax, float* dw, void* ws, int64_t ws_bytes, int B, int Cin, int Cout,
                                 int H, int W, int accumulate, void* stream) {
    return split_wgrad_impl(x, x_bs, dz, dz_bs, dw, ws, ws_bytes, B, Cin, Cout, H, W, accumulate, stream, save, save ? n_groups : 0, 1,
                            (const unsigned*)x_amax, (const unsigned*)dz_amax);
}

int onet_conv3x3_split_fwd_norm(const float* z_prev, int64_t z_bs, const float* save, int n_groups, const void* wq, int wq_f16,
                                const void* x_amax, float* z, int64_t zo_bs, float* part, int B, int Cin, int Cout, int H, int W,
                                void* stream) {
    ONET_REQUIRE(save, "conv3x3_split_fwd_norm: null pointer");
    return split_fwd(z_prev, z_bs, wq, z, zo_bs, B, Cin, Cout, H, W, stream, part, wq_f16, save, n_groups, (const unsigned*)x_amax);
}

int onet_split_pack_act(const float* x, int64_t x_bs, void* xs, int64_t xs_bs, int B, int C, int H, int W, int f16, float scale,
                        const void* slots, void* stream) {
    ONET_REQUIRE(x && xs, "split_pack_act: null pointer");
    ONET_REQUIRE(B > 0 && C > 0 && (C % 8) == 0 && H > 0 && W > 0, "split_pack_act: C must be a multiple of 8");
    ONET_REQUIRE((reinterpret_cast<uintptr_t>(xs) & 15) == 0 && (xs_bs & 3) == 0, "split_pack_act: 16-byte aligned slots required");
    const int64_t n = (int64_t)B * (C / 8) * H * W;
    const int blocks = (int)std::min<int64_t>((n + 255) / 256, 1 << 20);
    hipLaunchKernelGGL(split_pack_act_kernel, dim3(blocks), dim3(256), 0, as_stream(stream), x, x_bs, (unsigned*)xs, xs_bs, B, C / 8, H, W,
                       f16, scale, (const unsigned*)slots);
    return check_launch("split_pack_act_kernel");
}

static int pre_operand_checks(const char* entry, const void* xs, int64_t xs_bs, int wq_f16, int Cin, int Cout, int H, int W) {
    ONET_REQUIRE((Cin % (wq_f16 == 2 ? 32 : 16)) == 0, "%s: Cin must be a multiple of 16 (32 for plain bf16 operands)", entry);
    ONET_REQUIRE((xs_bs & 3) == 0 && (reinterpret_cast<uintptr_t>(xs) & 15) == 0, "%s: 16-byte aligned slots required", entry);
    ONET_REQUIRE(xs_bs >= (int64_t)Cin * H * W / (wq_f16 == 2 ? 2 : 1), "%s: batch stride too small", entry);
    ONET_REQUIRE((int64_t)(Cin + 32) * H * W * 4 < (1ll << 31) && (int64_t)(Cin + 32) * 2 * 9 * Cout * 2 < (1ll << 31),
                 "%s: operand exceeds the 2 GiB buffer-resource range", entry);
    ONET_REQUIRE(W != 16 || xs_bs * 4 + (int64_t)Cin * H * W * 4 < (1ll << 31), "%s: image pair exceeds the buffer-resource range", entry);
    return 0;
}

int onet_conv3x3_split_pre_nparts(int B, int H, int W) {
    if (W == 16) return (B > 0 && (B % 2) == 0 && (H % 16) == 0) ? (B / 2) * (H / 16) : 0;
    return split_nparts(B, H, W);
}

int onet_conv3x3_split_fwd_pre(const void* xs, int64_t xs_bs, const void* x_amax, int scale_always, const void* x_amax2, int split_ch,
                               const void* wq, int wq_f16, void* z, int z_bf16, int64_t z_bs, float* part, int B, int Cin, int Cout, int H, int W,
                               void* stream) {
    ONET_REQUIRE(!z_bf16 || (wq_f16 == 2 && (z_bs & 3) == 0 && (reinterpret_cast<uintptr_t>(z) & 7) == 0),
                 "conv3x3_split_fwd_pre: a bf16 output goes with plain bf16 operands (wq_f16 == 2), 8-byte aligned rows");
    ONET_REQUIRE(split_ch >= 0 && split_ch < Cin && (split_ch % 32) == 0, "conv3x3_split_fwd_pre: split_ch must be a multiple of 32 inside Cin");
    ONET_REQUIRE(xs && wq && z, "conv3x3_split_fwd_pre: null pointer");
    ONET_REQUIRE(B > 0 && Cin > 0 && Cout > 0 && H > 0 && (W > 16 || (W == 16 && (B % 2) == 0 && (H % 16) == 0)),
                 "conv3x3_split_fwd_pre: bad shape (maps wider than 16 pixels, or exactly 16 wide with an even batch and H %% 16 == 0)");
    ONET_REQUIRE(wq_f16 != 2 || (W % 4) == 0, "conv3x3_split_fwd_pre: plain bf16 operands need W %% 4 == 0");
    if (const int rc = pre_operand_checks("conv3x3_split_fwd_pre", xs, xs_bs, wq_f16, Cin, Cout, H, W)) return rc;
    ONET_REQUIRE(z_bs >= (int64_t)Cout * H * W, "conv3x3_split_fwd_pre: batch stride too small");
    SpPreArgs a{xs, xs_bs, (const __bf16*)wq, (float*)z, z_bs, B, Cin, Cout, H, W, 0, 0, 0, part, (const unsigned*)x_amax, scale_always,
                (const unsigned*)x_amax2, split_ch};
    a.z16 = z_bf16 ? 1 : 0;
    if (part) ONET_REQUIRE(onet_conv3x3_split_pre_nparts(B, H, W) > 0, "conv3x3_split_fwd_pre: statistics need a map made of full 16 x 32 tiles");
    hipStream_t st = as_stream(stream);
    if (W == 16) {
        if (wq_f16 == 2) return part ? launch_split_pre<true, 2, true>(a, st) : launch_split_pre<false, 2, true>(a, st);
        if (wq_f16) return part ? launch_split_pre<true, 1, true>(a, st) : launch_split_pre<false, 1, true>(a, st);
        return part ? launch_split_pre<true, 0, true>(a, st) : launch_split_pre<false, 0, true>(a, st);
    }
    if (wq_f16 == 2) return part ? launch_split_pre<true, 2, false>(a, st) : launch_split_pre<false, 2, false>(a, st);
    if (wq_f16) return part ? launch_split_pre<true, 1, false>(a, st) : launch_split_pre<false, 1, false>(a, st);
    return part ? launch_split_pre<true, 0, false>(a, st) : launch_split_pre<false, 0, false>(a, st);
}

int onet_conv3x3_split_dgrad_pre_bnreduce(const void* dzs, int64_t dzs_bs, const void* dz_amax, int scale_always, const void* wq, int wq_f16,
                                          float* da, int64_t da_bs, const void* z_prev, int z_bf16, int64_t z_bs, const float* save, int group_images,
                                          float* rec4, void* da_amax, int B, int Cin, int Cout, int H, int W, void* stream) {
    ONET_REQUIRE(dzs && wq && da && z_prev && save && rec4, "conv3x3_split_dgrad_pre_bnreduce: null pointer");
    if (onet_conv3x3_split_pre_nparts(B, H, W) <= 0 || (W != 16 && (W % 32)) || (Cout % 16)) return 1;
    if (W == 16 && ((group_images % 2) || wq_f16 != 2)) return 1;
    if (Cin / (wq_f16 == 2 ? 32 : 16) < 4) return 1;
    ONET_REQUIRE(B > 0 && Cin > 0 && Cout > 0, "conv3x3_split_dgrad_pre_bnreduce: bad shape");
    ONET_REQUIRE(group_images >= 0 && (group_images == 0 || B % group_images == 0), "conv3x3_split_dgrad_pre_bnreduce: bad statistics groups");
    if (const int rc = pre_operand_checks("conv3x3_split_dgrad_pre_bnreduce", dzs, dzs_bs, wq_f16, Cin, Cout, H, W)) return rc;
    ONET_REQUIRE((z_bs & 3) == 0 && (reinterpret_cast<uintptr_t>(z_prev) & (z_bf16 ? 7 : 15)) == 0 && (da_bs & 3) == 0 && (reinterpret_cast<uintptr_t>(da) & 15) == 0,
                 "conv3x3_split_dgrad_pre_bnreduce: 16-byte aligned rows required");
    ONET_REQUIRE(da_bs >= (int64_t)Cout * H * W && z_bs >= (int64_t)Cout * H * W, "conv3x3_split_dgrad_pre_bnreduce: batch stride too small");
    SpPreArgs a{dzs, dzs_bs, (const __bf16*)wq, da, da_bs, B, Cin, Cout, H, W, 0, 0, 0, nullptr, (const unsigned*)dz_amax, scale_always, nullptr, 0};
    a.rd_z = (const float*)z_prev;
    a.rd_z16 = z_bf16 ? 1 : 0;
    a.rd_z_bs = z_bs;
    a.rd_save = save;
    a.rd_gimg = group_images;
    a.rd_rec = rec4;
    a.rd_amax = (unsigned*)da_amax;
    hipStream_t st = as_stream(stream);
    if (W == 16) return launch_split_pre<false, 2, true, true>(a, st);
    if (wq_f16 == 2) return launch_split_pre<false, 2, false, true>(a, st);
    return wq_f16 ? launch_split_pre<false, 1, false, true>(a, st) : launch_split_pre<false, 0, false, true>(a, st);
}

int onet_conv3x3_split_dgrad_pre_slots(const void* dzs, int64_t dzs_bs, const void* dz_amax, int scale_always, const void* wq, int wq_f16,
                                       float* da, int64_t da_bs, void* daP, int64_t daP_bs, int ch0, const void* daP_amax, int B, int Cin,
                                       int Cout, int H, int W, void* stream) {
    ONET_REQUIRE(dzs && wq && da && daP && (daP_amax || wq_f16 == 2) && (wq_f16 == 1 || wq_f16 == 2), "conv3x3_split_dgrad_pre_slots: bad args");
    ONET_REQUIRE(B > 0 && Cin > 0 && Cout > 0 && H > 0 && W >= 32 && (W % 32) == 0 && (H % 16) == 0,
                 "conv3x3_split_dgrad_pre_slots: maps made of full 16 x 32 tiles");
    ONET_REQUIRE(ch0 > 0 && ch0 < Cout && (ch0 % 64) == 0 && (Cout % 64) == 0, "conv3x3_split_dgrad_pre_slots: ch0 and Cout must be multiples of 64");
    if (const int rc = pre_operand_checks("conv3x3_split_dgrad_pre_slots", dzs, dzs_bs, wq_f16, Cin, Cout, H, W)) return rc;
    ONET_REQUIRE((daP_bs & 3) == 0 && (reinterpret_cast<uintptr_t>(daP) & 15) == 0, "conv3x3_split_dgrad_pre_slots: 16-byte aligned slots required");
    ONET_REQUIRE(da_bs >= (int64_t)ch0 * H * W && daP_bs >= (int64_t)(Cout - ch0) * H * W / (wq_f16 == 2 ? 2 : 1),
                 "conv3x3_split_dgrad_pre_slots: batch stride too small");
    SpPreArgs a{dzs, dzs_bs, (const __bf16*)wq, da, da_bs, B, Cin, Cout, H, W, 0, 0, 0, nullptr, (const unsigned*)dz_amax, scale_always, nullptr, 0};
    a.zP = daP;
    a.zP_bs = daP_bs;
    a.zP_ch0 = ch0;
    a.zP_slots = (const unsigned*)daP_amax;
    if (wq_f16 == 2) return launch_split_pre<false, 2, false>(a, as_stream(stream));
    return launch_split_pre<false, 1, false>(a, as_stream(stream));
}

int onet_conv3x3_split_fwd_pre_act(const void* xs, int64_t xs_bs, const void* x_amax, int scale_always, const void* x_amax2, int split_ch,
                                   const void* wq, const float* save, void* aP, int64_t aP_bs, const void* aP_slots, void* a_amax, float* a,
                                   int64_t a_bs, int B, int Cin, int Cout, int H, int W, void* stream) {
    ONET_REQUIRE(xs && wq && save && aP && aP_slots, "conv3x3_split_fwd_pre_act: null pointer");
    ONET_REQUIRE(B > 0 && Cin > 0 && Cout > 0 && H > 0 && W > 0, "conv3x3_split_fwd_pre_act: bad shape");
    if (W < 32 || (W % 32) || (H % 16) || (Cin % 16) || (Cout % 64)) return 1;
    ONET_REQUIRE(split_ch >= 0 && split_ch < Cin && (split_ch % 32) == 0, "conv3x3_split_fwd_pre_act: split_ch must be a multiple of 32 inside Cin");
    if (const int rc = pre_operand_checks("conv3x3_split_fwd_pre_act", xs, xs_bs, 1, Cin, Cout, H, W)) return rc;
    ONET_REQUIRE((aP_bs & 3) == 0 && (reinterpret_cast<uintptr_t>(aP) & 15) == 0, "conv3x3_split_fwd_pre_act: 16-byte aligned slots required");
    ONET_REQUIRE(aP_bs >= (int64_t)Cout * H * W && (!a || a_bs >= (int64_t)Cout * H * W), "conv3x3_split_fwd_pre_act: batch stride too small");
    SpPreArgs p{xs, xs_bs, (const __bf16*)wq, nullptr, 0, B, Cin, Cout, H, W, 0, 0, 0, nullptr, (const unsigned*)x_amax, scale_always,
                (const unsigned*)x_amax2, split_ch};
    p.zP = aP;
    p.zP_bs = aP_bs;
    p.zP_ch0 = 0;
    p.zP_slots = (const unsigned*)aP_slots;
    p.act_save = save;
    p.act_amax = (unsigned*)a_amax;
    p.act_a = a;
    p.act_a_bs = a_bs;
    return launch_split_pre<false, 1, false, false, true>(p, as_stream(stream));
// ... 131 lines not shown
```

onet_amd/csrc/convt_gemm.hip:

```cpp
#include <algorithm>
#include <cstdlib>
#include "common.hpp"

using namespace onet;

typedef float f32x16 __attribute__((ext_vector_type(16)));
typedef float f32x4g __attribute__((ext_vector_type(4)));
typedef float f32x2g __attribute__((ext_vector_type(2)));
typedef int i32x4g __attribute__((ext_vector_type(4)));
typedef __bf16 bf16x8g __attribute__((ext_vector_type(8)));
typedef __bf16 bf16x2g __attribute__((ext_vector_type(2)));
typedef unsigned u32x4g __attribute__((ext_vector_type(4)));

namespace {

__device__ __forceinline__ i32x4g g_rsrc(const void* base, int64_t bytes) {
    const uint64_t p = reinterpret_cast<uint64_t>(base);
    i32x4g r;
    r.x = (int)(p & 0xffffffffu);
    r.y = (int)((p >> 32) & 0xffffu);
    r.z = bytes > 0x7fffffffll ? 0x7fffffff : (int)bytes;
    r.w = 0x00020000;
    return r;
}
// ... 269 lines not shown
#pragma unroll
            for (int u = 0; u < 2; ++u) {
                const int p = p0 + wc * 64 + u * 32 + l31;
#pragma unroll
                for (int r = 0; r < 16; ++r) {
                    const int ci = m0 + wr * 64 + t * 32 + (r & 3) + 8 * (r >> 2) + 4 * kh;
                    xb[(int64_t)ci * hw + p] = acc[t][u][r];
                }
            }
    }
}

constexpr int KP = 32;
constexpr int WA_F = 128 * KP;
constexpr int WB_F = 64 * 2 * KP;

template <int PREC = 0>
__global__ __launch_bounds__(256, 2) void convt_wgrad_gemm_kernel(GArgs g) {
    __shared__ __attribute__((aligned(16))) float lds[2 * (WA_F + WB_F)];
    int bid = xcd_block_id();
    const int tiles = g.mTiles * g.nTiles;
    const int ks = bid / tiles, tile = bid % tiles;
    const int mt = tile % g.mTiles, nt = tile / g.mTiles;
    const int tid = threadIdx.x, lane = tid & 63, wid = __builtin_amdgcn_readfirstlane(tid >> 6);
    const int wr = wid >> 1, wc = wid & 1, l31 = lane & 31, kh = lane >> 5;
    const int hw = g.h * g.w;
    const int ci0 = mt * 128, c0 = nt * 32;
    const int ch0 = ks * g.chunksPerSplit;
    const int nchunks_all = (int)(((int64_t)g.B * hw) / KP);
    const int ch1 = min(ch0 + g.chunksPerSplit, nchunks_all);

    auto issue = [&](int chunk, int buf) __attribute__((always_inline)) {
        const int64_t pix = (int64_t)chunk * KP;
        const int b = (int)(pix / hw), p0 = (int)(pix % hw);
        const i32x4g rx = g_rsrc(g.a + (int64_t)b * g.a_bs, (int64_t)g.Cin * hw * 4);
        const i32x4g rd = g_rsrc(g.b + (int64_t)b * g.b_bs, (int64_t)g.Ct * g.HoWo * 4);
        const unsigned la = g_lds(lds) + (unsigned)(buf * (WA_F + WB_F) * 4), lb = la + WA_F * 4;
#pragma unroll
        for (int j = 0; j < 4; ++j) {
            const int p = 4 * wid + j;
            {
                const int row = 8 * p + (lane >> 3), src = (lane & 7) ^ ((row >> 1) & 7);
                g_dma16(rx, la + p * 1024, (unsigned)((((int64_t)(ci0 + row)) * hw + p0 + src * 4) * 4));
            }
            {
                const int row = 4 * p + (lane >> 4), src = (lane & 15) ^ (row & 7);
                const int px = p0 + 2 * src, y = px / g.w, x = px % g.w;
                g_dma16(rd, lb + p * 1024,
                        (unsigned)((((int64_t)(c0 + (row >> 1))) * g.HoWo + (int64_t)(2 * y + (row & 1)) * g.Wo + 2 * x) * 4));
            }
        }
    };

    f32x16 acc[2][2];
#pragma unroll
    for (int t = 0; t < 2; ++t)
#pragma unroll
        for (int u = 0; u < 2; ++u)
#pragma unroll
            for (int r = 0; r < 16; ++r) acc[t][u][r] = 0.f;

    int a_row[2], b_row[2];
#pragma unroll
    for (int t = 0; t < 2; ++t) a_row[t] = wr * 64 + t * 32 + l31;
#pragma unroll
    for (int u = 0; u < 2; ++u) b_row[u] = (wc * 64 + u * 32 + l31) >> 1;
    const bool dj = (l31 & 1) != 0;

    if (ch0 < ch1) {
        issue(ch0, 0);
        asm volatile("s_waitcnt vmcnt(0)" ::: "memory");
        __syncthreads();
    }
    for (int c = ch0; c < ch1; ++c) {
        const int buf = (c - ch0) & 1;
        const bool more = c + 1 < ch1;
        const float* A = lds + buf * (WA_F + WB_F);
        const float* Bt = A + WA_F;
        if constexpr (PREC != 0) {
            if (more) issue(c + 1, buf ^ 1);
#pragma unroll
            for (int g2 = 0; g2 < KP / 16; ++g2) {
                float af[2][8], bf[2][8];
#pragma unroll
                for (int h2 = 0; h2 < 2; ++h2) {
                    const int gg = 2 * g2 + h2;
#pragma unroll
                    for (int t = 0; t < 2; ++t) {
                        const f32x4g v = *reinterpret_cast<const f32x4g*>(A + a_row[t] * KP + (((2 * gg + kh) ^ ((a_row[t] >> 1) & 7)) << 2));
#pragma unroll
                        for (int i = 0; i < 4; ++i) af[t][4 * h2 + i] = v[i];
                    }
#pragma unroll
                    for (int u = 0; u < 2; ++u)
#pragma unroll
                        for (int e = 0; e < 2; ++e) {
                            const f32x4g v = *reinterpret_cast<const f32x4g*>(Bt + b_row[u] * (2 * KP) + (((4 * gg + 2 * kh + e) ^ (b_row[u] & 7)) << 2));
                            bf[u][4 * h2 + 2 * e] = dj ? v[1] : v[0];
                            bf[u][4 * h2 + 2 * e + 1] = dj ? v[3] : v[2];
                        }
                }
                g_mma16<PREC>(af, bf, acc);
            }
        } else {
#pragma unroll
        for (int gg = 0; gg < KP / 8; ++gg) {
            if (gg == 0 && more) issue(c + 1, buf ^ 1);
            f32x4g a4[2], b4[2][2];
#pragma unroll
            for (int t = 0; t < 2; ++t)
                a4[t] = *reinterpret_cast<const f32x4g*>(A + a_row[t] * KP + (((2 * gg + kh) ^ ((a_row[t] >> 1) & 7)) << 2));
#pragma unroll
            for (int u = 0; u < 2; ++u)
#pragma unroll
                for (int e = 0; e < 2; ++e)
                    b4[u][e] = *reinterpret_cast<const f32x4g*>(Bt + b_row[u] * (2 * KP) + (((4 * gg + 2 * kh + e) ^ (b_row[u] & 7)) << 2));
#pragma unroll
            for (int tt = 0; tt < 4; ++tt) {
                float bv[2];
#pragma unroll
                for (int u = 0; u < 2; ++u) {
                    const f32x4g v = b4[u][tt >> 1];
                    bv[u] = dj ? v[(tt & 1) * 2 + 1] : v[(tt & 1) * 2];
                }
#pragma unroll
                for (int t = 0; t < 2; ++t)
#pragma unroll
                    for (int u = 0; u < 2; ++u) acc[t][u] = __builtin_amdgcn_mfma_f32_32x32x2f32(a4[t][tt], bv[u], acc[t][u], 0, 0, 0);
            }
        }
        }
        asm volatile("s_waitcnt vmcnt(0)" ::: "memory");
        __syncthreads();
    }

    float* slab = g.out + (int64_t)ks * g.Cin * 4 * g.Ct;
#pragma unroll
    for (int t = 0; t < 2; ++t)
#pragma unroll
        for (int u = 0; u < 2; ++u) {
            const int m = 4 * c0 + wc * 64 + u * 32 + l31;
#pragma unroll
            for (int r = 0; r < 16; ++r) {
                const int ci = ci0 + wr * 64 + t * 32 + (r & 3) + 8 * (r >> 2) + 4 * kh;
                slab[(int64_t)ci * 4 * g.Ct + m] = acc[t][u][r];
            }
        }
}

__global__ __launch_bounds__(256) void convt_wgrad_reduce_kernel(const float* __restrict__ slab, float* __restrict__ dw, int splitK,
                                                                 int64_t n4, int accumulate) {
    const int64_t i = blockIdx.x * (int64_t)blockDim.x + threadIdx.x;
    if (i >= n4) return;
    float4 s = reinterpret_cast<const float4*>(slab)[i];
    for (int k = 1; k < splitK; ++k) {
        const float4 v = reinterpret_cast<const float4*>(slab)[(int64_t)k * n4 + i];
        s.x += v.x; s.y += v.y; s.z += v.z; s.w += v.w;
    }
    if (accumulate) {
        const float4 o = reinterpret_cast<float4*>(dw)[i];
        s.x += o.x; s.y += o.y; s.z += o.z; s.w += o.w;
    }
    reinterpret_cast<float4*>(dw)[i] = s;
}

__global__ __launch_bounds__(256) void convt_dbias_reduce_kernel(const float* __restrict__ part, float* __restrict__ db, int ntiles, int Ct) {
    const int c = blockIdx.x;
    double s = 0.0;
    for (int t = threadIdx.x; t < ntiles; t += 256) s += (double)part[(int64_t)t * Ct + c];
    __shared__ double sh[4];
    double v[1] = {s};
    block_sum_256<double, 1>(v, sh);
    if (threadIdx.x == 0) db[c] = (float)v[0];
}


typedef _Float16 f16x8g __attribute__((ext_vector_type(8)));

struct SArgs {
    const void* wP;
    const void* xP;
    int64_t x_bs;
    const float* bias;
    void* yP;
    int64_t y_bs;
    const unsigned* x_slots;
    const unsigned* y_slots;
    int B, Cin, Ct, h, w, mTiles, nTiles;
};

template <int NP>
__device__ __forceinline__ f32x16 s_mfma(u32x4g a, u32x4g b, f32x16 c) {
    if constexpr (NP == 2) return __builtin_amdgcn_mfma_f32_32x32x16_f16(__builtin_bit_cast(f16x8g, a), __builtin_bit_cast(f16x8g, b), c, 0, 0, 0);
    else return __builtin_amdgcn_mfma_f32_32x32x16_bf16(__builtin_bit_cast(bf16x8g, a), __builtin_bit_cast(bf16x8g, b), c, 0, 0, 0);
}

constexpr int SLOT_NST = 2, SLOT_OCC = 4;
template <int N>
__device__ __forceinline__ void slot_wait() {
    asm volatile("s_waitcnt vmcnt(%0)" ::"n"(N) : "memory");
}

template <int NP>
__global__ __launch_bounds__(256, SLOT_OCC) void convt_slot_fwd_kernel(SArgs g) {
    constexpr int KS = 4 / NP;
    constexpr int TILE = KS * NP * 128;
    constexpr int NPC = TILE / 256;
    constexpr int NST = SLOT_NST;
    __shared__ __attribute__((aligned(16))) u32x4g lds[NST * 2 * TILE];
    const int bid = xcd_block_id();
    const int mt = bid % g.mTiles;
    const int nt = bid / g.mTiles;
    const int tid = threadIdx.x, lane = tid & 63, wid = __builtin_amdgcn_readfirstlane(tid >> 6);
    const int wr = wid >> 1, wc = wid & 1, l31 = lane & 31, kh = lane >> 5;
    const int hw = g.h * g.w, M = 4 * g.Ct;
    const int m0 = mt * 128, n0 = nt * 128;
    const int b = n0 / hw, p0 = n0 % hw;

    const i32x4g ra = g_rsrc(g.wP, (int64_t)(g.Cin / 8) * NP * M * 16);
    const i32x4g rb = g_rsrc(reinterpret_cast<const unsigned*>(g.xP) + (int64_t)b * g.x_bs, (int64_t)(g.Cin / 8) * hw * NP * 16);
    unsigned a_off[NPC], b_off[NPC];
#pragma unroll
    for (int j = 0; j < NPC; ++j) {
        const int s = (wid * NPC + j) * 64 + lane;
        const int c8 = s / (NP * 128), part = (s >> 7) % NP, r = s & 127;
        a_off[j] = (unsigned)((((int64_t)c8 * NP + part) * M + m0 + r) * 16);
        const int p = p0 + r, i = p / g.w, jx = p % g.w;
        b_off[j] = (unsigned)(((((int64_t)c8 * g.h + i) * NP + part) * g.w + jx) * 16);
    }
    const unsigned a_step = (unsigned)((int64_t)KS * NP * M * 16), b_step = (unsigned)((int64_t)KS * hw * NP * 16);
    const unsigned lds0 = (unsigned)(uintptr_t)(__attribute__((address_space(3))) u32x4g*)lds;
    auto issue = [&](int chunk, int buf) __attribute__((always_inline)) {
        const unsigned la = lds0 + (unsigned)(buf * 2 * TILE * 16), lb = la + TILE * 16;
#pragma unroll
        for (int j = 0; j < NPC; ++j) g_dma16(ra, la + (wid * NPC + j) * 1024, a_off[j] + chunk * a_step);
#pragma unroll
        for (int j = 0; j < NPC; ++j) g_dma16(rb, lb + (wid * NPC + j) * 1024, b_off[j] + chunk * b_step);
    };
    static_assert(NST >= 2 && NST <= 4, "the tail waits below cover rings of two to four stages");

    f32x16 acc[2][2];
#pragma unroll
    for (int t = 0; t < 2; ++t)
#pragma unroll
        for (int u = 0; u < 2; ++u)
#pragma unroll
            for (int r = 0; r < 16; ++r) acc[t][u][r] = 0.f;

    const int nch = g.Cin / (8 * KS);
#pragma unroll
    for (int c = 0; c < NST - 1; ++c) issue(c, c);
    float undo = 1.f;
    if constexpr (NP == 2) {
        const float* meta = reinterpret_cast<const float*>(reinterpret_cast<const _Float16*>(g.wP) + (int64_t)NP * g.Cin * M);
        float x_inv;
        (void)amax_scale(amax_read(g.x_slots), false, x_inv);
        undo = meta[1] * x_inv;
    }
    float s_inv;
    const float s_up = NP == 1 ? 1.f : amax_scale(amax_read(g.y_slots), false, s_inv);
    float bsv[2][4];
#pragma unroll
    for (int t = 0; t < 2; ++t)
#pragma unroll
        for (int gq = 0; gq < 4; ++gq) bsv[t][gq] = g.bias ? g.bias[(m0 + wr * 64 + t * 32 + 8 * gq + 4 * kh) >> 2] : 0.f;
    slot_wait<(NST - 2) * 2 * NPC>();
    __syncthreads();
    for (int c = 0; c < nch; ++c) {
        const int buf = c % NST;
        if (c + NST - 1 < nch) issue(c + NST - 1, (c + NST - 1) % NST);
        const u32x4g* A = lds + buf * 2 * TILE + wr * 64 + l31;
        const u32x4g* Bt = lds + buf * 2 * TILE + TILE + wc * 64 + l31;
#pragma unroll
        for (int s = 0; s < KS / 2; ++s) {
            u32x4g af[2][NP], bf[2][NP];
#pragma unroll
            for (int t = 0; t < 2; ++t)
#pragma unroll
                for (int q = 0; q < NP; ++q) af[t][q] = A[((2 * s + kh) * NP + q) * 128 + t * 32];
#pragma unroll
            for (int u = 0; u < 2; ++u)
#pragma unroll
                for (int q = 0; q < NP; ++q) bf[u][q] = Bt[((2 * s + kh) * NP + q) * 128 + u * 32];
            if constexpr (NP == 2) {
#pragma unroll
                for (int t = 0; t < 2; ++t)
#pragma unroll
                    for (int u = 0; u < 2; ++u) acc[t][u] = s_mfma<NP>(af[t][1], bf[u][0], acc[t][u]);
#pragma unroll
                for (int t = 0; t < 2; ++t)
#pragma unroll
                    for (int u = 0; u < 2; ++u) acc[t][u] = s_mfma<NP>(af[t][0], bf[u][1], acc[t][u]);
            }
#pragma unroll
            for (int t = 0; t < 2; ++t)
#pragma unroll
                for (int u = 0; u < 2; ++u) acc[t][u] = s_mfma<NP>(af[t][0], bf[u][0], acc[t][u]);
        }
        const int behind = min(NST - 2, nch - 2 - c);
        constexpr int PPC = 2 * NPC;
        if (behind >= 2) slot_wait<2 * PPC>();
        else if (behind == 1) slot_wait<1 * PPC>();
        else slot_wait<0>();
        __syncthreads();
    }

#pragma unroll
    for (int t = 0; t < 2; ++t)
#pragma unroll
// ... 245 lines not shown
        is_p0 = (int)(pix - (int64_t)is_b * hw);
    }
    i32x4g rx = g_rsrc(reinterpret_cast<const unsigned*>(g.xP) + (int64_t)is_b * g.x_bs, (int64_t)(g.Cin / 8) * hw * NP * 16);
    i32x4g rd = g_rsrc(reinterpret_cast<const unsigned*>(g.dyP) + (int64_t)is_b * g.dy_bs, (int64_t)(g.Ct / 8) * Ho * NP * Wo * 16);
    auto issue = [&](int chunk, int buf) __attribute__((always_inline)) {
        (void)chunk;
        const int p0 = is_p0;
        const unsigned lb = lds0 + (unsigned)(buf * STAGE * 16);
#pragma unroll
        for (int k = 0; k < NPW; ++k) {
            const int pc = wid * NPW + k;
            if (pc >= NPIECE) continue;
            const bool is_x = ((pc / (A_SLOTS / 64)) & 1) == 0;
            const int p = p0 + st_px[k], i = p >> g.lw, j = p & (g.w - 1);
            unsigned off;
            if (st_kind[k] == 0) off = st_base[k] + (unsigned)((i * NP * g.w + j) * 16);
            else if (st_kind[k] == 1) off = st_base[k] + (unsigned)((2 * i * NP * Wo + 2 * j) * 16);
            else off = 0x80000000u;
            if (is_x) g_dma16(rx, lb + (unsigned)(pc * 1024), off);
            else g_dma16(rd, lb + (unsigned)(pc * 1024), off);
        }
        is_p0 += CP;
        if (is_p0 >= hw) {
            is_p0 = 0;
            ++is_b;
            rx = g_rsrc(reinterpret_cast<const unsigned*>(g.xP) + (int64_t)is_b * g.x_bs, (int64_t)(g.Cin / 8) * hw * NP * 16);
            rd = g_rsrc(reinterpret_cast<const unsigned*>(g.dyP) + (int64_t)is_b * g.dy_bs, (int64_t)(g.Ct / 8) * Ho * NP * Wo * 16);
        }
    };
    const int my_pieces = min(NPW, max(0, NPIECE - wid * NPW));

    f32x16 acc[TM][2], accb[2];
#pragma unroll
    for (int t = 0; t < TM; ++t)
#pragma unroll
        for (int u = 0; u < 2; ++u)
#pragma unroll
            for (int r = 0; r < 16; ++r) acc[t][u][r] = 0.f;
#pragma unroll
    for (int u = 0; u < 2; ++u)
#pragma unroll
        for (int r = 0; r < 16; ++r) accb[u][r] = 0.f;
    const bool bias_wave = g.db_part != nullptr && mt == 0 && wr == 0;
    u32x4g ones;
    {
        const unsigned one2 = NP == 2 ? 0x3c003c00u : 0x3f803f80u;
        ones = u32x4g{one2, one2, one2, one2};
    }

    const int tq = (lane >> 2) & 3, tp = lane & 3, tg = (lane >> 4) & 1;
    const unsigned lane_off = (unsigned)((((2 * tg + (tp >> 1)) * PXP + 8 * kh + tq) * 16) + (tp & 1) * 8);
    const unsigned a_lane = lane_off + (unsigned)((wr * TM * 4) * PXP * 16);
    const unsigned b_lane = lane_off + (unsigned)((A_SLOTS + ((2 * di) * GB + chf * 4) * PXP) * 16);
    constexpr unsigned PART = (A_SLOTS + B_SLOTS) * 16;

    const int n_my = ch1 - ch0;
#pragma unroll
    for (int c = 0; c < NST - 1; ++c)
        if (c < n_my) issue(ch0 + c, c);
    auto wait_behind = [&](int behind) __attribute__((always_inline)) {
        if (behind >= 1 && NST > 2) {
            if (my_pieces == NPW) slot_wait<NPW>();
            else slot_wait<(NPW > 1 ? NPW - 1 : 0)>();
        } else {
            slot_wait<0>();
        }
    };
    if (n_my > 0) {
        wait_behind(min(NST - 2, n_my - 1));
        __syncthreads();
    }
    for (int c = ch0; c < ch1; ++c) {
        const int buf = (c - ch0) % NST;
        if (c + NST - 1 < ch1) issue(c + NST - 1, (c - ch0 + NST - 1) % NST);
        const unsigned base = lds0 + (unsigned)(buf * STAGE * 16);
#pragma unroll
        for (int s = 0; s < CP / 16; ++s) {
            u32x4g af[TM][NP], bf[2][NP];
#pragma unroll
            for (int t = 0; t < TM; ++t)
#pragma unroll
                for (int q = 0; q < NP; ++q) af[t][q] = sw_frag(base + a_lane + (unsigned)(t * 4 * PXP * 16 + s * 256) + q * PART);
#pragma unroll
            for (int u = 0; u < 2; ++u)
#pragma unroll
                for (int q = 0; q < NP; ++q) bf[u][q] = sw_frag(base + b_lane + (unsigned)(u * GB * PXP * 16 + s * 256) + q * PART);
            if constexpr (NP == 2) {
#pragma unroll
                for (int t = 0; t < TM; ++t)
#pragma unroll
                    for (int u = 0; u < 2; ++u) acc[t][u] = s_mfma<NP>(af[t][1], bf[u][0], acc[t][u]);
#pragma unroll
                for (int t = 0; t < TM; ++t)
#pragma unroll
                    for (int u = 0; u < 2; ++u) acc[t][u] = s_mfma<NP>(af[t][0], bf[u][1], acc[t][u]);
            }
#pragma unroll
            for (int t = 0; t < TM; ++t)
#pragma unroll
                for (int u = 0; u < 2; ++u) acc[t][u] = s_mfma<NP>(af[t][0], bf[u][0], acc[t][u]);
            if (bias_wave) {
#pragma unroll
                for (int u = 0; u < 2; ++u) {
                    accb[u] = s_mfma<NP>(ones, bf[u][0], accb[u]);
                    if constexpr (NP == 2) accb[u] = s_mfma<NP>(ones, bf[u][1], accb[u]);
                }
            }
        }
        wait_behind(min(NST - 2, ch1 - 2 - c));
        __syncthreads();
    }

    float undo = 1.f, dy_inv = 1.f;
    if constexpr (NP == 2) {
        float x_inv;
        (void)amax_scale(amax_read(g.x_slots), false, x_inv);
        (void)amax_scale(amax_read(g.dy_slots), true, dy_inv);
        undo = x_inv * dy_inv;
    }
    float* slab = g.slab + (int64_t)ks * g.Cin * 4 * g.Ct;
#pragma unroll
    for (int t = 0; t < TM; ++t)
#pragma unroll
        for (int u = 0; u < 2; ++u) {
            const int col = (GB * 8 * nt + chf * 32 + l31) * 4 + 2 * di + u;
#pragma unroll
            for (int r = 0; r < 16; ++r) {
                const int ci = C::MT * mt + wr * (TM * 32) + t * 32 + (r & 3) + 8 * (r >> 2) + 4 * kh;
                slab[(int64_t)ci * 4 * g.Ct + col] = acc[t][u][r] * undo;
            }
        }
    if (bias_wave && kh == 0) {
#pragma unroll
        for (int u = 0; u < 2; ++u) g.db_part[((int64_t)ks * 4 + 2 * di + u) * g.Ct + GB * 8 * nt + chf * 32 + l31] = accb[u][0] * dy_inv;
    }
}

__global__ void convt_pack_slots_kernel(const float* __restrict__ w, void* __restrict__ wP, void* __restrict__ wdP, int Cin, int Ct, int np,
                                        const unsigned* __restrict__ wamax) {
    const int M = 4 * Ct;
    const int64_t n = (int64_t)Cin * M;
    float winv = 1.f;
    const float wscale = np == 2 ? amax_scale(amax_read(wamax), true, winv) : 1.f;
    if (np == 2 && blockIdx.x == 0 && threadIdx.x == 0) {
        float* meta = reinterpret_cast<float*>(reinterpret_cast<_Float16*>(wP) + 2 * n);
        meta[0] = wscale;
        meta[1] = winv;
        if (wdP) {
            float* md = reinterpret_cast<float*>(reinterpret_cast<_Float16*>(wdP) + 2 * n);
            md[0] = wscale;
            md[1] = winv;
        }
    }
    for (int64_t i2 = blockIdx.x * (int64_t)blockDim.x + threadIdx.x; i2 < (wdP ? 2 * n : n); i2 += (int64_t)gridDim.x * blockDim.x) {
        if (i2 >= n) {
            const int64_t i = i2 - n;
            const int kc = (int)(i & 7);
            const int64_t r = i >> 3;
            const int ci = (int)(r % Cin), ks = (int)(r / Cin);
            const int c = (ks >> 2) * 8 + kc, q = ks & 3;
            const float v = w[((int64_t)ci * Ct + c) * 4 + q];
            if (np == 2) {
                _Float16* o = reinterpret_cast<_Float16*>(wdP);
                const float vs = v * wscale;
                const _Float16 hi = (_Float16)vs;
                o[(((int64_t)ks * 2 + 0) * Cin + ci) * 8 + kc] = hi;
                o[(((int64_t)ks * 2 + 1) * Cin + ci) * 8 + kc] = (_Float16)(vs - (float)hi);
            } else {
                reinterpret_cast<__bf16*>(wdP)[((int64_t)ks * Cin + ci) * 8 + kc] = (__bf16)v;
            }
            continue;
        }
        const int64_t i = i2;
        const int kc = (int)(i & 7);
        const int64_t r = i >> 3;
        const int m = (int)(r % M), c8 = (int)(r / M);
        const float v = w[(int64_t)(c8 * 8 + kc) * M + m];
        if (np == 2) {
            _Float16* o = reinterpret_cast<_Float16*>(wP);
            const float vs = v * wscale;
            const _Float16 hi = (_Float16)vs;
            o[(((int64_t)c8 * 2 + 0) * M + m) * 8 + kc] = hi;
            o[(((int64_t)c8 * 2 + 1) * M + m) * 8 + kc] = (_Float16)(vs - (float)hi);
        } else {
            reinterpret_cast<__bf16*>(wP)[((int64_t)c8 * M + m) * 8 + kc] = (__bf16)v;
        }
    }
}

__global__ void convt_absmax_kernel(const float* __restrict__ x, int64_t n, unsigned* __restrict__ slots) {
    float m = 0.f;
    for (int64_t i = blockIdx.x * (int64_t)blockDim.x + threadIdx.x; i < n; i += (int64_t)gridDim.x * blockDim.x) m = fmaxf(m, fabsf(x[i]));
#pragma unroll
    for (int o = 32; o > 0; o >>= 1) m = fmaxf(m, __shfl_xor(m, o, 64));
    if ((threadIdx.x & 63) == 0 && m == m)
        atomicMax(slots + ((blockIdx.x * (blockDim.x >> 6) + (threadIdx.x >> 6)) & (AMAX_SLOTS - 1)) * AMAX_STRIDE, __builtin_bit_cast(unsigned, m));
}

bool aligned16(const void* p) { return (reinterpret_cast<uintptr_t>(p) & 15) == 0; }

void wgrad_plan(int B, int Cin, int Ct, int h, int w, int& splitK, int& per) {
    const int64_t chunks = (int64_t)B * h * w / KP;
    const int64_t tiles = (int64_t)(Cin / 128) * (Ct / 32);
    int64_t k = std::max<int64_t>(1, (512 + tiles - 1) / tiles);
    k = std::min<int64_t>(k, std::max<int64_t>(1, chunks / 16));
    k = std::min<int64_t>(k, std::max<int64_t>(1, (256ll << 20) / ((int64_t)Cin * 4 * Ct * 4)));
    per = (int)((chunks + k - 1) / k);
    splitK = (int)((chunks + per - 1) / per);
}

}

namespace onet {


int convt_gemm_fwd(const float* x, int64_t x_bs, const float* wq, const float* bias, float* y, int64_t y_bs, void* y16, int64_t y16_bs,
                   int B, int Cin, int Ct, int h, int w, int Ho, int Wo, int pt, int pl, int prec, hipStream_t st, int y16_split,
                   const void* out_slots) {
    const int64_t hw = (int64_t)h * w;
    if (pt || pl || Ho != 2 * h || Wo != 2 * w || (Cin % KC) || (Ct % 32) || (hw % 128) || (w & 1) || !aligned16(x) || !aligned16(wq) ||
        (x_bs & 3) || (reinterpret_cast<uintptr_t>(y) & 7) || (y_bs & 1) || (int64_t)Cin * hw * 4 >= (1ll << 31) ||
        (int64_t)Cin * 4 * Ct * 4 >= (1ll << 31))
        return 1;
    if (y16 && !y16_split) return 1;
    if (y16 && y16_split && ((reinterpret_cast<uintptr_t>(y16) & 15) || (y16_bs & 3) || (Ct % 32))) return 1;
    if (!y && !y16) return 1;
    GArgs g{wq, x, y, bias, nullptr, (__bf16*)y16, y16_bs, 0, x_bs, y_bs, B, Cin, Ct, h, w, Wo, Ho * Wo, (4 * Ct) / 128, (int)(B * hw / 128), 1, 0, y16_split, (const unsigned*)out_slots};
    const int64_t blocks = (int64_t)g.mTiles * g.nTiles;
    if (blocks <= 0 || blocks >= (1ll << 31)) return 1;
    if (prec == 2) hipLaunchKernelGGL((convt_gemm_kernel<0, 2>), dim3((unsigned)blocks), dim3(256), 0, st, g);
    else if (prec) hipLaunchKernelGGL((convt_gemm_kernel<0, 1>), dim3((unsigned)blocks), dim3(256), 0, st, g);
    else hipLaunchKernelGGL((convt_gemm_kernel<0, 0>), dim3((unsigned)blocks), dim3(256), 0, st, g);
    return check_launch("convt_gemm_kernel<0>");
}

__global__ __launch_bounds__(256) void convt_out_bound_kernel(const float* __restrict__ w, const float* __restrict__ bias, int Cin, int Ct,
                                                              const unsigned* __restrict__ x_slots, unsigned* __restrict__ out_slots) {
    __shared__ float red[4][4];
    const float xmax = amax_read(x_slots);
    const int co = blockIdx.x;
    float sm[4] = {0.f, 0.f, 0.f, 0.f};
    for (int ci = threadIdx.x; ci < Cin; ci += 256) {
        const f32x4g v = *reinterpret_cast<const f32x4g*>(w + ((int64_t)ci * Ct + co) * 4);
        sm[0] += fabsf(v[0]);
        sm[1] += fabsf(v[1]);
        sm[2] += fabsf(v[2]);
        sm[3] += fabsf(v[3]);
    }
#pragma unroll
    for (int k = 0; k < 4; ++k) {
#pragma unroll
        for (int o = 32; o > 0; o >>= 1) sm[k] += __shfl_xor(sm[k], o, 64);
        if ((threadIdx.x & 63) == 0) red[threadIdx.x >> 6][k] = sm[k];
    }
    __syncthreads();
    if (threadIdx.x == 0) {
        float m = 0.f;
#pragma unroll
        for (int k = 0; k < 4; ++k) m = fmaxf(m, (red[0][k] + red[1][k]) + (red[2][k] + red[3][k]));
        const float bound = m * xmax * 1.00001f + (bias ? fabsf(bias[co]) : 0.f);
        if (bound == bound) atomicMax(out_slots + (co & 63) * AMAX_STRIDE, __builtin_bit_cast(unsigned, bound));
    }
}

int convt_out_bound(const float* w, const float* bias, int Cin, int Ct, const void* x_slots, void* out_slots, hipStream_t st) {
    hipLaunchKernelGGL(convt_out_bound_kernel, dim3((unsigned)Ct), dim3(256), 0, st, w, bias, Cin, Ct, (const unsigned*)x_slots,
                       (unsigned*)out_slots);
    return check_launch("convt_out_bound_kernel");
}

int64_t convt_gemm_dbias_ws_bytes(int B, int Ct, int h, int w) { return (int64_t)B * h * w / 128 * Ct * 4; }

int convt_gemm_dgrad(const float* dy, int64_t dy_bs, const float* wd, float* dx, int64_t dx_bs, float* dbias, float* dbias_ws, int B,
                     int Cin, int Ct, int h, int w, int Ho, int Wo, int pt, int pl, int prec, hipStream_t st) {
    const int64_t hw = (int64_t)h * w;
    if (pt || pl || Ho != 2 * h || Wo != 2 * w || (Cin % 128) || (Ct % 4) || (hw % 128) || (w & 1) || !aligned16(dy) || !aligned16(wd) ||
        (dy_bs & 3) || (int64_t)Ct * Ho * Wo * 4 >= (1ll << 31) || (int64_t)Cin * 4 * Ct * 4 >= (1ll << 31))
        return 1;
    if (dbias && !dbias_ws) return 1;
    GArgs g{wd, dy, dx, nullptr, dbias ? dbias_ws : nullptr, nullptr, 0, 0, dy_bs, dx_bs, B, Cin, Ct, h, w, Wo, Ho * Wo, Cin / 128, (int)(B * hw / 128), 1, 0};
    const int64_t blocks = (int64_t)g.mTiles * g.nTiles;
    if (blocks <= 0 || blocks >= (1ll << 31)) return 1;
    if (prec == 2) hipLaunchKernelGGL((convt_gemm_kernel<1, 2>), dim3((unsigned)blocks), dim3(256), 0, st, g);
    else if (prec) hipLaunchKernelGGL((convt_gemm_kernel<1, 1>), dim3((unsigned)blocks), dim3(256), 0, st, g);
    else hipLaunchKernelGGL((convt_gemm_kernel<1, 0>), dim3((unsigned)blocks), dim3(256), 0, st, g);
    int rc = check_launch("convt_gemm_kernel<1>");
    if (rc || !dbias) return rc;
    hipLaunchKernelGGL(convt_dbias_reduce_kernel, dim3((unsigned)Ct), dim3(256), 0, st, (const float*)dbias_ws, dbias, g.nTiles, Ct);
    return check_launch("convt_dbias_reduce_kernel");
}

int64_t convt_gemm_wgrad_ws_bytes(int B, int Cin, int Ct, int h, int w) {
    if ((Cin % 128) || (Ct % 32) || (((int64_t)h * w) % KP)) return 0;
    int k, per;
    wgrad_plan(B, Cin, Ct, h, w, k, per);
    return (int64_t)k * Cin * 4 * Ct * 4;
}

int convt_gemm_wgrad(const float* x, int64_t x_bs, const float* dy, int64_t dy_bs, float* dw, void* ws, int64_t ws_bytes, int B,
                     int Cin, int Ct, int h, int w, int Ho, int Wo, int pt, int pl, int prec, hipStream_t st) {
    const int64_t hw = (int64_t)h * w;
    if (pt || pl || Ho != 2 * h || Wo != 2 * w || (Cin % 128) || (Ct % 32) || (hw % KP) || (w & 1) || !aligned16(x) || !aligned16(dy) ||
        !aligned16(dw) || (x_bs & 3) || (dy_bs & 3) || (int64_t)Cin * hw * 4 >= (1ll << 31) || (int64_t)Ct * Ho * Wo * 4 >= (1ll << 31))
        return 1;
    GArgs g{x, dy, (float*)ws, nullptr, nullptr, nullptr, 0, x_bs, dy_bs, 0, B, Cin, Ct, h, w, Wo, Ho * Wo, Cin / 128, Ct / 32, 1, 0};
    wgrad_plan(B, Cin, Ct, h, w, g.splitK, g.chunksPerSplit);
    const int64_t n = (int64_t)Cin * 4 * Ct;
    if (ws_bytes < (int64_t)g.splitK * n * 4) return 1;
    const int64_t blocks = (int64_t)g.splitK * g.mTiles * g.nTiles;
    if (prec == 2) hipLaunchKernelGGL(convt_wgrad_gemm_kernel<2>, dim3((unsigned)blocks), dim3(256), 0, st, g);
    else if (prec) hipLaunchKernelGGL(convt_wgrad_gemm_kernel<1>, dim3((unsigned)blocks), dim3(256), 0, st, g);
    else hipLaunchKernelGGL(convt_wgrad_gemm_kernel<0>, dim3((unsigned)blocks), dim3(256), 0, st, g);
    int rc = check_launch("convt_wgrad_gemm_kernel");
    if (rc) return rc;
    hipLaunchKernelGGL(convt_wgrad_reduce_kernel, dim3((unsigned)cdiv(n / 4, 256)), dim3(256), 0, st, (const float*)ws, dw, g.splitK,
                       n / 4, 0);
    return check_launch("convt_wgrad_reduce_kernel");
}

}

static bool wgrad_slots_plan(int B, int Cin, int Ct, int h, int w, int& splitK, int& per) {
    const bool big = (Cin % 256) == 0 && (Ct % 64) == 0;
    const int64_t chunks = (int64_t)B * h * w / SW_CP;
    const int64_t tiles = big ? (int64_t)(Cin / 256) * (Ct / 64) : (int64_t)(Cin / 128) * (Ct / 32);
    int64_t k = std::max<int64_t>(1, ((big ? 256 : 512) + tiles - 1) / tiles);
    k = std::min<int64_t>(k, std::max<int64_t>(1, chunks / (512 / SW_CP)));
    k = std::min<int64_t>(k, std::max<int64_t>(1, (256ll << 20) / ((int64_t)Cin * 4 * Ct * 4)));
    per = (int)((chunks + k - 1) / k);
    splitK = (int)((chunks + per - 1) / per);
    return big;
}

template <int NP, int BIG>
static int launch_wgrad_slots(SWArgs g, hipStream_t st) {
    using C = SwCfg<BIG>;
    const int lds = NP * (C::APL + C::BPL) * C::PXP * 16 * C::NST;
    auto kern = convt_slot_wgrad_kernel<NP, BIG>;
    static PerDeviceOnce once;
    if (once.first()) (void)hipFuncSetAttribute(reinterpret_cast<const void*>(kern), hipFuncAttributeMaxDynamicSharedMemorySize, lds);
// ... 95 lines not shown
```

onet_amd/ops.py:

```python
from __future__ import annotations

import torch

from . import _lib

F32 = torch.float32


import os as _os


def _flags_from_env():
    out = {}
    for item in _os.environ.get("ONET_FLAGS", "").split(","):
        if "=" in item:
            k, v = item.split("=", 1)
            out[k.strip()] = v.strip()
    return out


_FLAGS = _flags_from_env()


def _flag(name, default):
# ... 286 lines not shown
    Cout, Cin = w.shape[0], w.shape[1]
    wf = torch.empty(Cin * 9 * Cout, dtype=F32, device=w.device)
    wd = torch.empty(Cout * 9 * Cin, dtype=F32, device=w.device)
    _lib.call("onet_conv3x3_pack_weights", _p(w), _p(wf), _p(wd), Cout, Cin, _stream())
    return wf, wd


def packT2x2(w):
    require_gpu(w)
    w = w.detach().contiguous()
    Cin, Cout = w.shape[0], w.shape[1]
    wf = torch.empty(Cin * 4 * Cout, dtype=F32, device=w.device)
    wd = torch.empty(4 * Cout * Cin, dtype=F32, device=w.device)
    _lib.call("onet_convT2x2_pack_weights", _p(w), _p(wf), _p(wd), Cin, Cout, _stream())
    return wf, wd


def packT2x2_fused(w):
    require_gpu(w)
    w = w.detach().contiguous()
    Cin, Cout = w.shape[0], w.shape[1]
    wq = torch.empty(Cin * 4 * Cout, dtype=F32, device=w.device)
    _lib.call("onet_convT2x2_pack_weights_fused", _p(w), _p(wq), Cin, Cout, _stream())
    return wq


CONVT_BF16 = _flag("CONVT_BF16", True)


def convT2x2_fwd(x, wq, bias, out, Ct, pt, pl):
    require_gpu(x, wq, out)
    x, xbs = plane(x)
    B, Cin, h, w = x.shape
    Ho, Wo = out.shape[2], out.shape[3]
    obs = out.stride(0) if B > 1 else Ct * Ho * Wo
    e0 = _prof_begin("convt_gemm_kernel")
    _lib.call("onet_convT2x2_fwd", _p(x), xbs, _p(wq), _p(bias), _p(out), obs, B, Cin, Ct, h, w, Ho, Wo, pt, pl,
              convt_operand_bf16(B, h, w, Ct), _stream())
    _prof_end("convt_gemm_kernel", 2.0 * B * h * w * Cin * 4 * Ct, e0, 4.0 * (B * h * w * (Cin + 4 * Ct) + 4 * Cin * Ct))


def convT2x2_out_bound(weight, bias, x_amax):
    w = weight.detach()
    w = w if w.is_contiguous() else w.contiguous()
    slots = new_amax(w.device)
    _lib.call("onet_convT2x2_out_bound", _p(w), _p(bias), w.shape[0], w.shape[1], _p(x_amax), _p(slots), _stream())
    return slots


def packT2x2_slots(w, parts=2, dgrad=False):
    require_gpu(w)
    w = w.detach().contiguous()
    Cin, Ct = w.shape[0], w.shape[1]
    dt = torch.float16 if parts == 2 else BF
    wP = torch.empty(Cin * 4 * Ct * parts + 4, dtype=dt, device=w.device)
    wdP = torch.empty(Cin * 4 * Ct * parts + 4, dtype=dt, device=w.device) if dgrad else None
    ws = torch.empty(2048, dtype=torch.int32, device=w.device) if parts == 2 else None
    _lib.call("onet_convT2x2_pack_weights_slots", _p(w), _p(wP), _p(wdP), _p(ws), Cin, Ct, parts, _stream())
    return (wP, wdP) if dgrad else wP


def convT2x2_dgrad_slots(dyP, wdP, Cin, dy_slots=None):
    B, C8, Ho, parts, Wo, _ = dyP.shape
    Ct, h, w = C8 * 8, Ho // 2, Wo // 2
    dx = torch.empty((B, Cin, h, w), dtype=F32, device=dyP.device)
    e0 = _prof_begin("convt_gemm_kernel")
    rc = _lib.load().onet_convT2x2_dgrad_slots(_p(dyP), _pbs(dyP), _p(dy_slots), _p(wdP), _p(dx), Cin * h * w, parts, B, Cin, Ct, h, w, _stream())
    flops, nb = 2.0 * B * h * w * Cin * 4 * Ct, B * h * w * (4.0 * Cin + 2.0 * parts * 4 * Ct)
    _prof_end("convt_gemm_kernel", flops if rc == 0 else 0.0, e0, nb if rc == 0 else 0.0)
    if rc < 0:
        raise _lib.OnetHipError(f"onet_convT2x2_dgrad_slots failed ({rc}): {_lib.last_error()}")
    return dx if rc == 0 else None


def convT2x2_wgrad_slots(xP, dyP, dw_shape, x_slots=None, dy_slots=None, want_dbias=False, out=None, db_out=None):
    B, C8, h, parts, w, _ = xP.shape
    Cin, Ct = C8 * 8, dyP.shape[1] * 8
    assert tuple(dw_shape) == (Cin, Ct, 2, 2) and dyP.shape[3] == parts and dyP.shape[2] == 2 * h and xP.dtype == dyP.dtype
    need = int(_lib.load().onet_convT2x2_wgrad_slots_ws_bytes(B, Cin, Ct, h, w))
    if need <= 0:
        return None
    ws = workspace(need, xP.device)
    dw = out if out is not None else torch.empty(dw_shape, dtype=F32, device=xP.device)
    db = (db_out if db_out is not None else torch.empty(Ct, dtype=F32, device=xP.device)) if want_dbias else None
    e0 = _prof_begin("convt_wgrad_gemm_kernel")
    rc = _lib.load().onet_convT2x2_wgrad_slots(_p(xP), _pbs(xP), _p(x_slots), _p(dyP), _pbs(dyP), _p(dy_slots), _p(dw), _p(db), _p(ws),
                                               ws.numel() * 4, parts, B, Cin, Ct, h, w, _stream())
    flops, nb = 2.0 * B * h * w * Cin * 4 * Ct, 2.0 * parts * B * h * w * (Cin + 4 * Ct)
    _prof_end("convt_wgrad_gemm_kernel", flops if rc == 0 else 0.0, e0, nb if rc == 0 else 0.0)
    if rc < 0:
        raise _lib.OnetHipError(f"onet_convT2x2_wgrad_slots failed ({rc}): {_lib.last_error()}")
    return (dw, db) if rc == 0 else None


def conv3x3_dgrad_bound(weight, dz_slots, ci0):
    w = weight.detach()
    w = w if w.is_contiguous() else w.contiguous()
    slots = new_amax(w.device)
    _lib.call("onet_conv3x3_dgrad_bound", _p(w), w.shape[0], w.shape[1], int(ci0), _p(dz_slots), _p(slots), _stream())
    return slots


def conv3x3_split_dgrad_pre_slots(dzP, wq, Cout, ch0, daP_slots, slots=None, always=False):
    B, C8, H, parts, W, _ = dzP.shape
    assert wq.dtype == dzP.dtype == (torch.float16 if parts == 2 else BF)
    da = torch.empty((B, Cout, H, W), dtype=F32, device=dzP.device)
    daP = torch.empty((B, (Cout - ch0) // 8, H, parts, W, 8), dtype=dzP.dtype, device=dzP.device)
    e0 = _prof_begin("conv3x3_split_pre_kernel")
    _lib.call("onet_conv3x3_split_dgrad_pre_slots", _p(dzP), _pbs(dzP), _p(slots), int(always), _p(wq), 2 if parts == 1 else 1, _p(da), Cout * H * W,
              _p(daP), _pbs(daP), int(ch0), _p(daP_slots), B, C8 * 8, Cout, H, W, _stream())
    eb = 2.0 * parts
    _prof_end("conv3x3_split_pre_kernel", 2.0 * B * H * W * C8 * 8 * Cout * 9, e0,
              B * H * W * (eb * C8 * 8 + 4.0 * ch0 + eb * (Cout - ch0)) + eb * 9 * C8 * 8 * Cout)
    return da, daP


CONVT_SLOTS = _flag("CONVT_SLOTS", True)


def convt_slots_ok(B, Cin, Ct, h, w, parts=None):
    parts = p16_parts() if parts is None else parts
    return bool(CONVT_SLOTS and presplit() and (parts == 2 or CONVT_BF16) and Cin % 32 == 0 and Cin >= 128 and Ct % 32 == 0 and (h * w) % 128 == 0 and w % 2 == 0
                and Cin * h * w * 2 * parts < 2 ** 31)


CONVT_BWD_SLOTS = _flag("CONVT_BWD_SLOTS", True)


def convt_bwd_slots_ok(B, Cin, Ct, C2, h, w):
    return bool(CONVT_BWD_SLOTS and convt_slots_ok(B, Cin, Ct, h, w) and Cin % 128 == 0 and (w & (w - 1)) == 0
                and C2 % 64 == 0 and (C2 + Ct) % 64 == 0 and (2 * h) % 16 == 0 and (2 * w) % 32 == 0 and Ct * 4 * h * w * 4 < 2 ** 31)


class _LazyPack:

    def __init__(self, owner, i):
        self.owner, self.i = owner, i

    def get(self):
        return self.owner[self.i]


def pack_of(p):
    return p.get() if isinstance(p, _LazyPack) else p


class PackedT:

    def __init__(self, w):
        self.w = w.detach()
        self._v = self.w._version
        self._t = [None, None]
        self._s = {}

    def _same_weight(self):
        if self.w._version != self._v:
            raise RuntimeError("onet_amd: one of the variables needed for gradient computation has been modified by an inplace operation: "
                               f"a ConvTranspose2d weight of shape {list(self.w.shape)} is at version {self.w._version}; expected version "
                               f"{self._v} instead")

    def __getitem__(self, i):
        if self._t[i] is None:
            self._same_weight()
            self._t[i] = packT2x2_fused(self.w) if i == 0 else packT2x2(self.w)[1]
        return self._t[i]

    def __iter__(self):
        return iter((_LazyPack(self, 0), _LazyPack(self, 1)))

    def __len__(self):
        return 2

    def slots(self, parts):
        if parts not in self._s:
            self._same_weight()
            self._s[parts] = packT2x2_slots(self.w, parts, dgrad=bool(CONVT_BWD_SLOTS))
        v = self._s[parts]
        return v[0] if isinstance(v, tuple) else v

    def dgrad_slots(self, parts):
        v = self._s.get(parts)
        if not isinstance(v, tuple):
            self._same_weight()
            self._s[parts] = v = packT2x2_slots(self.w, parts, dgrad=True)
        return v[1]


def convT2x2_fwd_slots(xP, wP, bias, outP, Ct, x_slots=None, slots=None, kind="convt_gemm_kernel"):
    B, C8, h, parts, w, _ = xP.shape
    assert outP.shape[3] == parts and outP.shape[2] == 2 * h and outP.shape[4] == 2 * w and xP.dtype == wP.dtype == outP.dtype
    Cin = C8 * 8
    e0 = _prof_begin(kind)
    rc = _lib.load().onet_convT2x2_fwd_slots(_p(xP), _pbs(xP), _p(x_slots), _p(wP), _p(bias), _p(outP), _pbs(outP), _p(slots), parts, B, Cin, Ct,
                                             h, w, _stream())
    eb = 2.0 * parts
    flops, nb = 2.0 * B * h * w * Cin * 4 * Ct, eb * (B * h * w * (Cin + 4 * Ct) + 4 * Cin * Ct)
    _prof_end(kind, flops if rc == 0 else 0.0, e0, nb if rc == 0 else 0.0)
    if rc < 0:
        raise _lib.OnetHipError(f"onet_convT2x2_fwd_slots failed ({rc}): {_lib.last_error()}")
    return rc == 0


def convT2x2_fwd_p(x, wq, bias, outP, Ct, pt, pl, slots=None):
    require_gpu(x, wq)
    x, xbs = plane(x)
    B, Cin, h, w = x.shape
    Ho, Wo = outP.shape[2], outP.shape[4]
    e0 = _prof_begin("convt_gemm_kernel")
    rc = _lib.load().onet_convT2x2_fwd_p(_p(x), xbs, _p(wq), _p(bias), _p(outP), _pbs(outP), _p(slots), outP.shape[3], B, Cin, Ct, h, w, Ho, Wo, pt, pl,
                                         convt_operand_bf16(B, h, w, Ct), _stream())
    flops, nb = 2.0 * B * h * w * Cin * 4 * Ct, 4.0 * (B * h * w * (Cin + 4 * Ct) + 4 * Cin * Ct)
    _prof_end("convt_gemm_kernel", flops if rc == 0 else 0.0, e0, nb if rc == 0 else 0.0)
    if rc < 0:
        raise _lib.OnetHipError(f"onet_convT2x2_fwd_p failed ({rc}): {_lib.last_error()}")
    return rc == 0


import os as _os
CONV_ALGO = _os.environ.get("ONET_CONV_ALGO", "auto")
TWIN = _flag("TWIN", True)


BF = torch.bfloat16


_SENTINEL = {}


def _sentinel(device):
    key = (device.type, device.index if device.index is not None else torch.cuda.current_device())
    s = _SENTINEL.get(key)
    if s is None:
        s = _SENTINEL[key] = torch.zeros(1, dtype=F32, device=device)
    return s


def is_placeholder(t):
    return bool(_SENTINEL) and t.is_cuda and t.dtype == F32 and \
        t.untyped_storage().data_ptr() == _sentinel(t.device).untyped_storage().data_ptr()


def fp32_placeholder(shape, device):
    t = torch.empty(0, dtype=F32, device=device)
    t.set_(_sentinel(t.device).untyped_storage(), 0, tuple(shape), (0,) * len(shape))
    return t


def twin_virtual(x, bias):
    t = fp32_placeholder((2 * x.shape[0],) + tuple(x.shape[1:]), x.device)
    t._onet_twin_src = [x, float(bias), None]
    return t


def twin_src_of(t):
    tag = getattr(t, "_onet_twin_src", None)
    return None if tag is None else (tag[0], tag[1])


def twin_materialize(t=None, src=None):
    tag = getattr(t, "_onet_twin_src", None) if t is not None else None
    if tag is not None and tag[2] is not None:
        return tag[2]
    x, bias = (tag[0], tag[1]) if tag is not None else src
    B = x.shape[0]
    xx = torch.empty((2 * B,) + tuple(x.shape[1:]), dtype=F32, device=x.device)
    xx[:B].copy_(x)
    complement_clip(x, bias, out=xx[B:])
    if tag is not None:
        tag[2] = xx
    return xx


def _z16(z):
    return int(z.dtype == torch.bfloat16)


def _wino_legal(Cin, Cout):
    return Cin >= 16 and Cin % 4 == 0 and Cout % 4 == 0


def _in_buffer_range(Cin, Cout, H, W):
    return (2 * max(Cin, Cout) + 16) * H * W * 4 < 2 ** 31 and (max(Cin, Cout) + 16) * 36 * (max(Cin, Cout) + 63) * 4 < 2 ** 31


def _split_legal(Cin, Cout, H, W):
    return Cin % 16 == 0 and W > 16 and W % 4 == 0 and H >= 8


def conv3x3_algo(B, Cin, Cout, H, W):
    algo = conv_algo()
    if algo in ("bf16", "winograd4", "auto", "split") and not _in_buffer_range(Cin, Cout, H, W):
        algo = "direct"
    if algo == "split":
        if _split_legal(Cin, Cout, H, W):
            return "split"
        algo = "auto_nosplit"
    if algo == "auto" and split_enabled() and _split_legal(Cin, Cout, H, W):
        if B * -(-H // 16) * -(-W // 32) * -(-Cout // 64) >= (n_cu() * 3) // 4:
            return "split"
    if algo == "auto_nosplit":
        algo = "auto"
    if algo == "bf16":
        if Cin % 16 == 0 and Cout % 4 == 0 and W >= 16 and H >= 8:
            return "bf16"
        algo = "auto"
    if algo == "direct" or not _wino_legal(Cin, Cout):
        return "direct"
    if min(H, W) < 8:
        return "direct"
    if algo == "winograd4":
        return "winograd4"
    if min(H, W) >= 16:
        img = 1 if W > 16 else 2
        blocks = -(-B // img) * -(-W // (32 if W > 16 else 16)) * -(-H // 16) * -(-Cout // 64)
        if blocks >= (n_cu() * 7) // 8:
            return "winograd4"
    return "direct"


def use_winograd(Cin, Cout, H, W):
    return conv_algo() != "direct" and _wino_legal(Cin, Cout) and min(H, W) >= 8


class Packed3x3(dict):

    def __init__(self, w):
        super().__init__(Cin=w.shape[1], Cout=w.shape[0])
        self.w = w.detach()

    def get_pack(self, algo):
        if algo not in self:
            self[algo] = {"direct": pack3x3, "winograd4": pack3x3_winograd4, "split": pack3x3_split, "plain16": pack3x3_plain16}[algo](self.w)
        return self[algo]


def pack3x3_auto(w):
    return Packed3x3(w)


def _fp32_algo(B, Cin, Cout, H, W):
    algo = conv3x3_algo(B, Cin, Cout, H, W)
    if algo != "bf16":
        return algo
    cur = active_settings()
    with using(cur.replace(conv="auto") if cur is not None else Settings(conv="auto")):
        return conv3x3_algo(B, Cin, Cout, H, W)


def conv3x3_auto(x, pk, direction, out=None, amax=None):
    Ci, Co = (pk["Cin"], pk["Cout"]) if direction == 0 else (pk["Cout"], pk["Cin"])
    shp = x.shape
    algo = _fp32_algo(shp[0], Ci, Co, shp[2], shp[3])
    if algo == "split" and direction == 1 and not split_dgrad():
        with using(active_settings().replace(split=False) if active_settings() is not None else Settings(split=False)):
            algo = _fp32_algo(shp[0], Ci, Co, shp[2], shp[3])
    wq = pk.get_pack(algo)[direction]
    if algo == "winograd4":
        return conv3x3_winograd4(x, wq, Co, out=out)
    if algo == "split":
        if direction == 0 and amax is None and wq.dtype == torch.float16:
            amax = absmax_slots(x)
        return conv3x3_split(x, wq, Co, out=out, amax=amax, always=direction == 1)
    return conv_fwd(x, wq, Co, 3, out=out)


BN_ON_LOAD = _flag("BN_ON_LOAD", True)
BN_ON_LOAD_MAX_COUT = 128
CONVT_SPLIT_MIN_BLOCKS = None
CONVT_SPLIT = _flag("CONVT_SPLIT", True)
SPLIT_F16 = _flag("SPLIT_F16", True)
SPLIT_DGRAD = _flag("SPLIT_DGRAD", True)
PRESPLIT = _flag("PRESPLIT", True)
PRESPLIT_W16 = _flag("PRESPLIT_W16", True)
PRESPLIT_KEEP_FP32 = _flag("PRESPLIT_KEEP_FP32", False)
SPLIT_GRAD_F16 = _flag("SPLIT_GRAD_F16", False)
SPLIT_WGRAD_MINW = 16
SPLIT_AUTO = _flag("SPLIT", True)
STEM_FUSED = _flag("STEM_FUSED", True)


def conv3x3_fwd_bn_partials(x, pk, norm=None, amax=None):
    Ci, Co = pk["Cin"], pk["Cout"]
    if norm is not None:
        z_prev, save, slots = norm
        require_gpu(z_prev, save)
        zs, zbs = plane(z_prev)
        B, _, H, W = zs.shape
        nparts = int(_lib.load().onet_conv3x3_split_nparts(B, H, W)) if not sync_bn() else 0
        out = torch.empty((B, Co, H, W), dtype=F32, device=zs.device)
        cm = torch.empty((Co, nparts, 3), dtype=F32, device=zs.device) if nparts > 0 else None
        e0 = _prof_begin("conv3x3_split_kernel")
        wq = pk.get_pack("split")[0]
        f16 = wq.dtype == torch.float16
        _lib.call("onet_conv3x3_split_fwd_norm", _p(zs), zbs, _p(save), save.shape[0], _p(wq), int(f16), _p(slots) if f16 else None,
                  _p(out), Co * H * W, _p(cm), B, Ci, Co, H, W, _stream())
        _prof_end("conv3x3_split_kernel", 2.0 * B * H * W * Ci * Co * 9, e0, 4.0 * (B * H * W * (Ci + Co) + 9 * Ci * Co))
        return out, cm
    B, _, H, W = x.shape
    if Ci <= 4 and stem_fused() and not sync_bn() and hasattr(pk, "w"):
        nparts = int(_lib.load().onet_conv3x3_stem_nparts(B, Ci, Co, H, W))
        if nparts > 0:
            require_gpu(x)
            tw = twin_src_of(x)
            xs, xbs = plane(tw[0] if tw is not None else x)
            w = pk.w if pk.w.is_contiguous() else pk.w.contiguous()
            out = torch.empty((B, Co, H, W), dtype=F32, device=x.device)
            cm = torch.empty((Co, nparts, 3), dtype=F32, device=x.device)
            e0 = _prof_begin("stem_conv_stats_kernel")
            _lib.call("onet_conv3x3_stem_fwd_stats", _p(xs), xbs, _p(w), _p(out), Co * H * W, _p(cm), B, Ci, Co, H, W,
                      B // 2 if tw is not None else 0, tw[1] if tw is not None else 0.0, _stream())
            _prof_end("stem_conv_stats_kernel", 2.0 * B * H * W * Ci * Co * 9, e0, 4.0 * (B * H * W * (Ci + Co) + 9 * Ci * Co))
            return out, cm
    algo = _fp32_algo(B, Ci, Co, H, W)
    nparts = 0
    if algo == "winograd4" and not sync_bn():
        nparts = int(_lib.load().onet_conv3x3_winograd4_nparts(B, H, W))
    if algo == "split" and not sync_bn():
        nparts = int(_lib.load().onet_conv3x3_split_nparts(B, H, W))
        if nparts > 0:
            wq = pk.get_pack(algo)[0]
            require_gpu(x)
            xs, xbs = plane(x)
            if xs.data_ptr() % 16 or xbs % 4:
                xs = xs.contiguous()
                xbs = xs.stride(0) if B > 1 else xs[0].numel()
            out = torch.empty((B, Co, H, W), dtype=F32, device=x.device)
            cm = torch.empty((Co, nparts, 3), dtype=F32, device=x.device)
            if wq.dtype == torch.float16 and amax is None:
                amax = absmax_slots(xs)
            e0 = _prof_begin("conv3x3_split_kernel")
            if wq.dtype == torch.float16:
                _lib.call("onet_conv3x3_split_conv_amax", _p(xs), xbs, _p(amax), 0, _p(wq), _p(out), Co * H * W, _p(cm), B, Ci, Co, H, W,
                          _stream())
            else:
                _lib.call("onet_conv3x3_split_fwd_stats", _p(xs), xbs, _p(wq), 0, _p(out), Co * H * W, _p(cm), B, Ci, Co, H, W, _stream())
            _prof_end("conv3x3_split_kernel", 2.0 * B * H * W * Ci * Co * 9, e0, 4.0 * (B * H * W * (Ci + Co) + 9 * Ci * Co))
            return out, cm
    if nparts <= 0:
        return conv3x3_auto(x, pk, 0, amax=amax), None
    wq = pk.get_pack(algo)[0]
    require_gpu(x, wq)
    x, xbs = plane(x)
    out = torch.empty((B, Co, H, W), dtype=F32, device=x.device)
    cm = torch.empty((Co, nparts, 3), dtype=F32, device=x.device)
    e0 = _prof_begin("conv_wino4_kernel")
    _lib.call("onet_conv3x3_winograd4_fwd_stats", _p(x), xbs, _p(wq), _p(out), Co * H * W, _p(cm), B, Ci, Co, H, W,
              _stream())
    _prof_end("conv_wino4_kernel", 2.0 * B * H * W * Ci * Co * 9, e0, 4.0 * (B * H * W * (Ci + Co) + 9 * Ci * Co))
    return out, cm


FUSE_BN_REDUCE = _flag("FUSE_BN_REDUCE", True)


def conv3x3_dgrad_bnreduce(dz, pk, z_prev, save_prev):
    if not FUSE_BN_REDUCE or sync_bn():
        return None
    Ci, Co = pk["Cout"], pk["Cin"]
    B, _, H, W = dz.shape
    if conv3x3_algo(B, Ci, Co, H, W) != "winograd4":
        return None
    nparts = int(_lib.load().onet_conv3x3_winograd4_nparts(B, H, W))
    G = save_prev.shape[0]
    if nparts <= 0 or B % G or tuple(z_prev.shape) != (B, Co, H, W) or not save_prev.is_contiguous():
        return None
    z_prev, zbs = plane(z_prev)
    if (zbs & 3) or (z_prev.data_ptr() & 15):
        return None
    wq = pk.get_pack("winograd4")[1]
    require_gpu(dz, wq, z_prev, save_prev)
    dz, dbs = plane(dz)
    da = torch.empty((B, Co, H, W), dtype=F32, device=dz.device)
    rec = torch.empty((Co, nparts, 2), dtype=F32, device=dz.device)
    e0 = _prof_begin("conv_wino4_kernel")
    _lib.call("onet_conv3x3_winograd4_dgrad_bnreduce", _p(dz), dbs, _p(wq), _p(da), Co * H * W, _p(z_prev), zbs,
              _p(save_prev), B // G, _p(rec), B, Ci, Co, H, W, _stream())
    _prof_end("conv_wino4_kernel", 2.0 * B * H * W * Ci * Co * 9, e0, 4.0 * (B * H * W * (Ci + Co) + 9 * Ci * Co))
    return da, rec






def pack3x3_winograd4(w):
    require_gpu(w)
    w = w.detach().contiguous()
    Cout, Cin = w.shape[0], w.shape[1]
    wf = torch.empty(Cin * 36 * ((Cout + 63) // 64 * 64), dtype=F32, device=w.device)
    wd = torch.empty(Cout * 36 * ((Cin + 63) // 64 * 64), dtype=F32, device=w.device)
    _lib.call("onet_conv3x3_pack_weights_winograd4", _p(w), _p(wf), _p(wd), Cout, Cin, _stream())
    return wf, wd


def conv3x3_winograd4(x, wq, Cout, out=None):
    require_gpu(x, wq)
    x, xbs = plane(x)
    B, Cin, H, W = x.shape
    if out is None:
        out = torch.empty((B, Cout, H, W), dtype=F32, device=x.device)
    zbs = out.stride(0) if B > 1 else Cout * H * W
    e0 = _prof_begin("conv_wino4_kernel")
    _lib.call("onet_conv3x3_winograd4_fwd", _p(x), xbs, _p(wq), _p(out), zbs, B, Cin, Cout, H, W, _stream())
    _prof_end("conv_wino4_kernel", 2.0 * B * H * W * Cin * Cout * 9, e0, 4.0 * (B * H * W * (Cin + Cout) + 9 * Cin * Cout))
    return out


def pack3x3_plain16(w):
    require_gpu(w)
    w = w.detach().contiguous()
    Cout, Cin = w.shape[0], w.shape[1]
    wf = torch.empty(Cin * 9 * Cout + 8, dtype=BF, device=w.device) if Cin % 16 == 0 else None
    wd = torch.empty((-(-Cout // 16) * 16) * 9 * Cin + 8, dtype=BF, device=w.device)
    _lib.call("onet_conv3x3_split_pack_weights", _p(w), _p(wf), _p(wd), None, Cout, Cin, 2, 2, _stream())
    return wf, wd


def pack3x3_split(w):
    require_gpu(w)
    w = w.detach().contiguous()
    Cout, Cin = w.shape[0], w.shape[1]
    f_fwd, f_dg = split_f16(), grad_f16() or presplit()
    wf = torch.empty(2 * Cin * 9 * Cout + 8, dtype=torch.float16 if f_fwd else BF, device=w.device) if Cin % 16 == 0 else None
    wd = torch.empty(2 * (-(-Cout // 16) * 16) * 9 * Cin + 8, dtype=torch.float16 if f_dg else BF, device=w.device)
    ws = torch.empty(AMAX_SLOTS, dtype=torch.int32, device=w.device) if (f_fwd or f_dg) else None
    _lib.call("onet_conv3x3_split_pack_weights", _p(w), _p(wf), _p(wd), _p(ws), Cout, Cin, int(f_fwd), int(f_dg), _stream())
    return wf, wd


class counting_batches:

    def __enter__(self):
        self.outer = getattr(_TLS, "counters", None)
        _TLS.counters = []
        return self

    def __exit__(self, *exc):
        pending, _TLS.counters = _TLS.counters, self.outer
        by_inc = {}
        for t, n in pending:
            by_inc.setdefault(n, []).append(t)
        for n, ts in by_inc.items():
            if len(ts) > 1 and all(t.is_cuda for t in ts):
                torch._foreach_add_(ts, n)
            else:
                for t in ts:
                    t.add_(n)
        return False


def count_batches(counter, n):
    pending = getattr(_TLS, "counters", None)
    if pending is None:
        counter.add_(n)
    else:
        pending.append((counter, n))


AMAX_SLOTS = 64 * 32


_AMAX_ARENA = {}
AMAX_ARENA_ROWS = 192


def amax_arena_reset(device):
    key = (device.type, device.index if device.index is not None else torch.cuda.current_device())
    ar = _AMAX_ARENA[key] = [torch.empty((AMAX_ARENA_ROWS, AMAX_SLOTS), dtype=torch.int32, device=device), 0]
    fill(ar[0].view(torch.float32), 0.0)


def new_amax(device):
    key = (device.type, device.index if device.index is not None else torch.cuda.current_device())
    ar = _AMAX_ARENA.get(key)
    if ar is not None and ar[1] < AMAX_ARENA_ROWS:
        ar[1] += 1
        return ar[0][ar[1] - 1]
    return torch.zeros(AMAX_SLOTS, dtype=torch.int32, device=device)


def absmax_slots(x):
    require_gpu(x)
    xc = x.contiguous()
    slots = new_amax(x.device)
    _lib.call("onet_absmax_slots", _p(xc), xc.numel(), _p(slots), _stream())
    return slots


def conv3x3_split(x, wq, Cout, out=None, norm=None, amax=None, always=False):
    if wq is None or not wq.is_cuda or wq.dtype not in (torch.bfloat16, torch.float16):
        raise TypeError("conv3x3_split: wq must be a split pack on the GPU (pack3x3_split)")
    f16 = int(wq.dtype == torch.float16)
    require_gpu(x)
    if norm is not None:
        require_gpu(norm)
        x, xbs = plane(x)
        B, Cin, H, W = x.shape
        if out is None:
            out = torch.empty((B, Cout, H, W), dtype=F32, device=x.device)
        e0 = _prof_begin("conv3x3_split_kernel")
        _lib.call("onet_conv3x3_split_fwd_norm", _p(x), xbs, _p(norm), norm.shape[0], _p(wq), f16, _p(amax) if f16 else None, _p(out),
                  out.stride(0) if B > 1 else Cout * H * W, None, B, Cin, Cout, H, W, _stream())
        _prof_end("conv3x3_split_kernel", 2.0 * B * H * W * Cin * Cout * 9, e0, 4.0 * (B * H * W * (Cin + Cout) + 9 * Cin * Cout))
        return out
    x, xbs = plane(x)
    if x.data_ptr() % 16 or xbs % 4:
        x = x.contiguous()
        xbs = x.stride(0) if x.shape[0] > 1 else x[0].numel()
    B, Cin, H, W = x.shape
    if out is None:
        out = torch.empty((B, Cout, H, W), dtype=F32, device=x.device)
    zbs = out.stride(0) if B > 1 else Cout * H * W
    if f16 and always and amax is None:
        amax = absmax_slots(x)
    e0 = _prof_begin("conv3x3_split_kernel")
    if f16:
        _lib.call("onet_conv3x3_split_conv_amax", _p(x), xbs, _p(amax), int(always), _p(wq), _p(out), zbs, None, B, Cin, Cout, H, W, _stream())
    else:
        _lib.call("onet_conv3x3_split_fwd", _p(x), xbs, _p(wq), 0, _p(out), zbs, B, Cin, Cout, H, W, _stream())
    _prof_end("conv3x3_split_kernel", 2.0 * B * H * W * Cin * Cout * 9, e0, 4.0 * (B * H * W * (Cin + Cout) + 9 * Cin * Cout))
    return out


def split_pack_act(x, f16=True, scale=1.0, out=None, parts=2, slots=None):
    require_gpu(x)
    x, xbs = plane(x)
    B, C, H, W = x.shape
    if out is not None:
        parts = out.shape[3]
    if out is None:
        out = torch.empty((B, C // 8, H, parts, W, 8), dtype=torch.float16 if (f16 and parts == 2) else BF, device=x.device)
    _lib.call("onet_split_pack_act", _p(x), xbs, _p(out), _pbs(out), B, C, H, W, 2 if parts == 1 else int(f16), float(scale), _p(slots),
              _stream())
    return out


def conv3x3_split_pre(xs, wq, Cout, out=None, slots=None, always=False, stats=None, slots2=None, split_ch=0, z16=False):
    if wq is None or not wq.is_cuda or wq.dtype not in (torch.bfloat16, torch.float16) or xs.dtype != wq.dtype:
        raise TypeError("conv3x3_split_pre: xs and wq must be split packs of the same 16-bit type on the GPU")
    B, C8, H, two, W, eight = xs.shape
    f16 = 2 if two == 1 else int(wq.dtype == torch.float16)
    Cin = C8 * 8
    if out is None:
        out = torch.empty((B, Cout, H, W), dtype=BF if (z16 and two == 1) else F32, device=xs.device)
    e0 = _prof_begin("conv3x3_split_pre_kernel")
    _lib.call("onet_conv3x3_split_fwd_pre", _p(xs), _pbs(xs), _p(slots), int(always), _p(slots2), int(split_ch if slots2 is not None or slots is not None else 0),
              _p(wq), f16, _p(out), _z16(out),
              out.stride(0) if B > 1 else Cout * H * W, _p(stats), B, Cin, Cout, H, W, _stream())
    _prof_end("conv3x3_split_pre_kernel", 2.0 * B * H * W * Cin * Cout * 9, e0,
              B * H * W * (2.0 * two * Cin + out.element_size() * Cout) + 2.0 * two * 9 * Cin * Cout)
    return out


def conv3x3_split_dgrad_pre_bnreduce(dzP, wq, Cout, z_prev, save_prev, slots=None, always=False, want_amax=False):
    if not FUSE_BN_REDUCE or sync_bn() or not FUSE_DGRAD_REDUCE:
        return None
    B, C8, H, two, W, _ = dzP.shape
    Cin = C8 * 8
    G = save_prev.shape[0]
    if tuple(z_prev.shape) != (B, Cout, H, W) or B % G or not save_prev.is_contiguous() or wq.dtype != dzP.dtype:
        return None
    lib = _lib.load()
    nparts = int(lib.onet_conv3x3_split_pre_nparts(B, H, W))
    z_prev, zbs = plane(z_prev)
    if nparts <= 0 or nparts % G or (zbs & 3) or (z_prev.data_ptr() & 15):
        return None
    f16 = 2 if two == 1 else int(wq.dtype == torch.float16)
    da = torch.empty((B, Cout, H, W), dtype=F32, device=dzP.device)
    rec4 = torch.empty((nparts, Cout, 4), dtype=F32, device=dzP.device)
    am = new_amax(dzP.device) if want_amax else None
    e0 = _prof_begin("conv3x3_split_pre_kernel")
    rc = lib.onet_conv3x3_split_dgrad_pre_bnreduce(_p(dzP), _pbs(dzP), _p(slots), int(always), _p(wq), f16, _p(da), Cout * H * W, _p(z_prev), _z16(z_prev), zbs,
                                                   _p(save_prev), B // G if G > 1 else 0, _p(rec4), _p(am), B, Cin, Cout, H, W, _stream())
    _prof_end("conv3x3_split_pre_kernel", 2.0 * B * H * W * Cin * Cout * 9 if rc == 0 else 0.0, e0,
              (B * H * W * (2.0 * two * Cin + (4.0 + z_prev.element_size()) * Cout) + 2.0 * two * 9 * Cin * Cout) if rc == 0 else 0.0)
    if rc < 0:
        raise _lib.OnetHipError(f"onet_conv3x3_split_dgrad_pre_bnreduce failed ({rc}): {_lib.last_error()}")
    return (da, rec4, am) if rc == 0 else None


def eval_layer_ok(B, Cin, Cout, H, W):
    if not presplit() or p16_parts() != 2:
# ... 932 lines not shown
```

onet_amd/trainer.py:

```python
from __future__ import annotations

import math
import os
import time

import torch
import torch.distributed as dist

from . import ops
from .modules import invalidate_packed


def sim_lr(epoch: int, base_lr: float = 5e-6) -> float:
    return base_lr * (0.5 ** max(0, (epoch - 1) // 100)) if epoch > 0 else base_lr


def cosine_warm_restarts_lr(epoch: int, base_lr: float = 1e-4, T_0: int = 300, T_mult: int = 2,
                            eta_min: float = 1e-6) -> float:
    t, Ti = epoch, T_0
    while t >= Ti:
        t -= Ti
        Ti *= T_mult
    return eta_min + (base_lr - eta_min) * (1 + math.cos(math.pi * t / Ti)) / 2

# ... 36 lines not shown
        if dist.is_available() and dist.is_initialized() and (world_size > 1 or dist.get_world_size() == 1):
            err = None
            try:
                self._flag_pg = dist.new_group(backend="gloo")
            except Exception as e:
                err = e
            ok = torch.tensor([0 if err is not None else 1], dtype=torch.int32,
                              device=dev if dist.get_backend(process_group) == "nccl" else "cpu")
            dist.all_reduce(ok, op=dist.ReduceOp.MIN, group=process_group)
            if int(ok.item()) == 0:
                import warnings
                warnings.warn("onet_amd: no host-side group for the shared NaN verdict on at least one rank"
                              + (f" (here: {err})" if err is not None else "") + "; a NaN loss raises on its own rank only")
                self._flag_pg = None

    def enable_overlap(self, bucket_mb: float = 32.0):
        if self._buckets is not None:
            return
        cap = max(1, int(bucket_mb * 2 ** 20 / 4))
        self._buckets, end, members = [], self.numel, []
        for i in reversed(range(len(self.params))):
            members.append(i)
            start = self.offsets[i]
            if end - start >= cap or i == 0:
                self._buckets.append({"start": start, "end": end, "params": members, "pending": len(members),
                                      "work": None, "launched": False})
                end, members = start, []
        self._bucket_of = {i: b for b, bk in enumerate(self._buckets) for i in bk["params"]}
        self._hooks = [p.register_post_accumulate_grad_hook(lambda _p, i=i: self._on_grad(i))
                       for i, p in enumerate(self.params)]

    def disable_overlap(self):
        if self._buckets is None:
            return
        for bk in self._buckets:
            if bk["work"] is not None:
                bk["work"].wait()
        for h in self._hooks:
            h.remove()
        self._buckets = self._hooks = None

    def _launch_bucket(self, bk, async_op=True):
        view = self.gflat[bk["start"]:bk["end"]]
        bk["work"] = dist.all_reduce(view, op=dist.ReduceOp.SUM, group=self.pg, async_op=async_op)
        bk["launched"] = True

    def _on_grad(self, i):
        p, off = self.params[i], self.offsets[i]
        if p.grad is not None and p.grad.data_ptr() != self.gflat.data_ptr() + 4 * off:
            view = self.gflat[off:off + p.numel()].view_as(p)
            view.copy_(p.grad)
            p.grad = view
        bk = self._buckets[self._bucket_of[i]]
        bk["pending"] -= 1
        if bk["pending"] == 0 and not bk["launched"] and not self.skip_allreduce and dist.is_available() and dist.is_initialized():
            self._launch_bucket(bk)

    def _finish_overlap(self):
        for bk in self._buckets:
            if not bk["launched"]:
                self._launch_bucket(bk, async_op=False)
            elif bk["work"] is not None:
                bk["work"].wait()
            bk.update(pending=len(bk["params"]), work=None, launched=False)

    def zero_grad(self, set_to_none: bool = False):
        if self.gflat.is_cuda:
            ops.fill(self.gflat, 0.0)
        else:
            self.gflat.zero_()
        if self.direct_grads:
            for p in self.params:
                p.grad = None
                p._onet_gslot_taken = False
        else:
            for p, off in zip(self.params, self.offsets):
                if p.grad is None or p.grad.data_ptr() != self.gflat.data_ptr() + 4 * off:
                    p.grad = self.gflat[off:off + p.numel()].view_as(p)
        if self._buckets is not None:
            for bk in self._buckets:
                bk.update(pending=len(bk["params"]), work=None, launched=False)

    def all_reduce_grads(self):
        if self.skip_allreduce:
            if self._buckets is not None:
                for bk in self._buckets:
                    bk.update(pending=len(bk["params"]), work=None, launched=False)
            return
        if self.world_size > 1 or (dist.is_available() and dist.is_initialized()):
            if self._buckets is not None:
                self._finish_overlap()
            else:
                dist.all_reduce(self.gflat, op=dist.ReduceOp.SUM, group=self.pg)

    def _gather_stray_grads(self):
        for p, off in zip(self.params, self.offsets):
            if p.grad is not None and p.grad.data_ptr() != self.gflat.data_ptr() + 4 * off:
                view = self.gflat[off:off + p.numel()].view_as(p)
                view.copy_(p.grad)
                p.grad = view

    def _check_nan_all_ranks(self):
        try:
            ops.check_deferred_nan()
            bad = None
        except AssertionError as e:
            bad = e
        if self._flag_pg is not None:
            flag = torch.tensor([0 if bad is None else 1], dtype=torch.int32)
            dist.all_reduce(flag, op=dist.ReduceOp.MAX, group=self._flag_pg)
            if bad is None and int(flag.item()):
                bad = AssertionError("jsd is NaN (on another rank)")
        if bad is not None:
            if self._buckets is not None:
                for bk in self._buckets:
                    if bk["work"] is not None:
                        bk["work"].wait()
                    bk.update(pending=len(bk["params"]), work=None, launched=False)
            raise bad

    def _segments_with_grads(self):
        have = [p.grad is not None for p in self.params]
        if self._steps is None:
            if all(have):
                self.step_count += 1
                return [(0, self.numel, self.step_count)]
            self._steps = [self.step_count] * len(self.params)
        segs, start, cur = [], None, None
        for i, h in enumerate(have):
            if h:
                self._steps[i] += 1
            st = self._steps[i] if h else None
            if start is not None and st != cur:
                segs.append((start, self.offsets[i], cur))
                start = None
            if h and start is None:
                start, cur = self.offsets[i], st
        if start is not None:
            segs.append((start, self.numel, cur))
        self.step_count = max(self._steps)
        return segs

    def step(self):
        self._check_nan_all_ranks()
        g = self.param_groups[0]
        segs = self._segments_with_grads()
        self._gather_stray_grads()
        self.all_reduce_grads()
        for a, b, n in segs:
            ops.adam_step(self.flat[a:b], self.gflat[a:b], self.m[a:b], self.v[a:b], g["lr"], g["betas"][0], g["betas"][1],
                          g["eps"], g["weight_decay"], n, grad_scale=1.0 / self.world_size)
        torch.autograd.graph.increment_version([p for p in self.params if p.grad is not None])
        invalidate_packed(self.model)

    def broadcast_params(self, src=0):
        if self.world_size > 1 or (dist.is_available() and dist.is_initialized()):
            dist.broadcast(self.flat, src=src, group=self.pg)
            for b in self.model.buffers():
                dist.broadcast(b, src=src, group=self.pg)
            torch.autograd.graph.increment_version(self.params)
            invalidate_packed(self.model)


def init_distributed(backend: str | None = None):
    world = int(os.environ.get("WORLD_SIZE", "1"))
    rank = int(os.environ.get("RANK", "0"))
    local = int(os.environ.get("ONET_FORCE_LOCAL_RANK", os.environ.get("LOCAL_RANK", "0")))
    if "RANK" in os.environ and not dist.is_initialized():
        os.environ.setdefault("MASTER_ADDR", "127.0.0.1")
        os.environ.setdefault("MASTER_PORT", "29500")
        backend = os.environ.get("ONET_DIST_BACKEND", backend)
        if backend is None:
            backend = "nccl" if torch.cuda.is_available() else "gloo"
        if backend == "nccl":
            torch.cuda.set_device(local)
            dist.init_process_group(backend, rank=rank, world_size=world, device_id=torch.device("cuda", local))
        else:
            dist.init_process_group(backend, rank=rank, world_size=world)
    return rank, world, local


def shard_batch(X, rank: int, world: int, drop_remainder: bool = False):
    B = X.shape[0]
    if B % world:
        if not drop_remainder or B < world:
            raise ValueError(f"batch {B} not divisible by world size {world}")
        B -= B % world
    per = B // world
    return X[rank * per:(rank + 1) * per]


def train_step(onet, opt, X):
    opt.zero_grad()
    Lt, Vt, Ld, Vd, S = onet(X)
    St = S[:, 0, :, :].unsqueeze(dim=1)
    Sd = S[:, 1, :, :].unsqueeze(dim=1)
    loss = onet.compute_loss(Lt, St, Ld, Sd)
    loss.backward()
    opt.step()
    return loss


def save_checkpoint(onet, path, epoch, key="epoch"):
    from . import io
    io.save_checkpoint(onet, path, epoch, zy3=(key == "save_epoch"))


def load_checkpoint(onet, path, map_location=None):
    from . import io
    return io.load_checkpoint(onet, path, map_location=map_location)


def fit(onet, train_loader, device, epochs, schedule="sim", base_lr=None, eval_fn=None, eval_every=None,
        out_root=None, model_name="Onet", fused_adam=True, rank=0, world=1, log=print):
    before = getattr(onet, "settings", None)
    if fused_adam and before is not None:
        onet.settings = before.replace(lazy_nan=True)
    try:
        return _fit(onet, train_loader, device, epochs, schedule, base_lr, eval_fn, eval_every, out_root, model_name,
                    fused_adam, rank, world, log)
    finally:
        if before is not None:
            onet.settings = before


def _fit(onet, train_loader, device, epochs, schedule, base_lr, eval_fn, eval_every, out_root, model_name, fused_adam,
         rank, world, log):
    if base_lr is None:
        base_lr = 5e-6 if schedule == "sim" else 1e-4
    if fused_adam:
        opt = FlatAdam(onet, lr=base_lr, world_size=world)
        opt.broadcast_params(0)
        if world > 1:
            opt.enable_overlap()
    else:
        opt = torch.optim.Adam(onet.parameters(), lr=base_lr, betas=(0.9, 0.999), eps=1e-8, weight_decay=0)
    if eval_every is None:
        eval_every = 50 if schedule == "sim" else 1
    history = []
    for epoch in range(epochs):
        onet.train()
        lr = sim_lr(epoch, base_lr) if schedule == "sim" else cosine_warm_restarts_lr(epoch, base_lr)
        opt.param_groups[0]["lr"] = lr
        losses, n_img, t0 = [], 0, time.time()
        for batch in train_loader:
            X = batch[0] if isinstance(batch, (tuple, list)) else batch
            if X.shape[0] < world:
                continue
            X = shard_batch(X, rank, world, drop_remainder=True).to(device, non_blocking=True)
            loss = train_step(onet, opt, X)
            losses.append(loss.item())
            n_img += X.shape[0] * world
        ep_loss = float(sum(losses) / max(1, len(losses)))
        rec = {"epoch": epoch, "loss": ep_loss, "lr": lr, "images_per_s": n_img / max(1e-9, time.time() - t0)}
        if eval_fn is not None and epoch % eval_every == 0:
            onet.eval()
            with torch.no_grad():
                rec["eval"] = eval_fn(onet, epoch)
        history.append(rec)
        if rank == 0:
            log("%s===Epoch: %04d loss: %.5f, lr: %.10f, %.1f img/s" % (model_name, epoch, ep_loss, lr, rec["images_per_s"]))
        last = epoch == epochs - 1
        if out_root and rank == 0 and (last or epoch == 300):
            save_checkpoint(onet, os.path.join(out_root, "%s_epoch_%d.pytorch" % (model_name, epoch)), epoch,
                            key="epoch" if schedule == "sim" else "save_epoch")
    return history
```

Baseline: 592.3.

## Batch per-step weight packing into one arena launch and vectorize wgrad reduce

After each optimizer step, all weight repacks that were used (split/plain16 3x3 and ConvT slot packs) are done by two batched kernels: one absmax pass and one pack pass. They are driven by a job table and write into a single arena. This replaces many small per-layer pack launches issued lazily during the next forward. It also adds a float4-vectorized, unrolled wgrad split-K reduction kernel for taps 9 and 1 and routes all reduce call sites through it. The cost is more complex plan and arena bookkeeping, and packs are now made eagerly even when a layer might not reuse them.

```diff
diff --git a/include/onet_hip.h b/include/onet_hip.h
--- a/include/onet_hip.h
+++ b/include/onet_hip.h
@@ -66,6 +66,8 @@
 
 int onet_conv3x3_split_pack_weights(const float* w, void* wq_fwd, void* wq_dgrad, void* amax_ws, int Cout, int Cin, int fwd_f16,
                                     int dgrad_f16, void* stream);
+int onet_weights_prepare_batch(const void* table, const int64_t* table_host, int n_amax, int n_pack, int amax_blocks, int pack_blocks,
+                               void* arena, int64_t arena_bytes, int64_t slots_off, int64_t slots_bytes, void* stream);
 int onet_absmax_slots(const float* x, int64_t n, void* slots, void* stream);
 int onet_conv3x3_split_conv_amax(const float* x, int64_t x_bs, const void* x_amax, int scale_always, const void* wq, float* z, int64_t z_bs,
                                  float* part, int B, int Cin, int Cout, int H, int W, void* stream);
diff --git a/onet_amd/csrc/common.hpp b/onet_amd/csrc/common.hpp
--- a/onet_amd/csrc/common.hpp
+++ b/onet_amd/csrc/common.hpp
@@ -100,6 +100,44 @@
     return __builtin_bit_cast(float, (unsigned)(127 + k) << 23);
 }
 
+__device__ __forceinline__ void convt_pack_slots_elem(const float* __restrict__ w, void* __restrict__ wP, void* __restrict__ wdP, int Cin,
+                                                      int Ct, int np, float wscale, int64_t i2) {
+    const int M = 4 * Ct;
+    const int64_t n = (int64_t)Cin * M;
+    if (i2 >= n) {
+        const int64_t i = i2 - n;
+        const int kc = (int)(i & 7);
+        const int64_t r = i >> 3;
+        const int ci = (int)(r % Cin), ks = (int)(r / Cin);
+        const int c = (ks >> 2) * 8 + kc, q = ks & 3;
+        const float v = w[((int64_t)ci * Ct + c) * 4 + q];
+        if (np == 2) {
+            _Float16* o = reinterpret_cast<_Float16*>(wdP);
+            const float vs = v * wscale;
+            const _Float16 hi = (_Float16)vs;
+            o[(((int64_t)ks * 2 + 0) * Cin + ci) * 8 + kc] = hi;
+            o[(((int64_t)ks * 2 + 1) * Cin + ci) * 8 + kc] = (_Float16)(vs - (float)hi);
+        } else {
+            reinterpret_cast<__bf16*>(wdP)[((int64_t)ks * Cin + ci) * 8 + kc] = (__bf16)v;
+        }
+        return;
+    }
+    const int64_t i = i2;
+    const int kc = (int)(i & 7);
+    const int64_t r = i >> 3;
+    const int m = (int)(r % M), c8 = (int)(r / M);
+    const float v = w[(int64_t)(c8 * 8 + kc) * M + m];
+    if (np == 2) {
+        _Float16* o = reinterpret_cast<_Float16*>(wP);
+        const float vs = v * wscale;
+        const _Float16 hi = (_Float16)vs;
+        o[(((int64_t)c8 * 2 + 0) * M + m) * 8 + kc] = hi;
+        o[(((int64_t)c8 * 2 + 1) * M + m) * 8 + kc] = (_Float16)(vs - (float)hi);
+    } else {
+        reinterpret_cast<__bf16*>(wP)[((int64_t)c8 * M + m) * 8 + kc] = (__bf16)v;
+    }
+}
+
 int launch_wgrad_reduce(const float* slab, float* dw, int splitK, int taps, int Cout, int Cin, int out_layout, int accumulate,
                         hipStream_t st);
 
diff --git a/onet_amd/csrc/conv_mfma.hip b/onet_amd/csrc/conv_mfma.hip
--- a/onet_amd/csrc/conv_mfma.hip
+++ b/onet_amd/csrc/conv_mfma.hip
@@ -515,8 +515,16 @@
     const int64_t i = (int64_t)blockIdx.x * 64 + (threadIdx.x & 63);
     const int g = threadIdx.x >> 6;
     float s = 0.f;
-    if (i < n)
-        for (int k = g; k < splitK; k += 4) s += slab[((int64_t)k * taps + t) * n + i];
+    if (i < n) {
+        const float* p = slab + (int64_t)t * n + i;
+        const int64_t ks = (int64_t)taps * n;
+        int k = g;
+        for (; k + 12 < splitK; k += 16) {
+            const float v0 = p[k * ks], v1 = p[(k + 4) * ks], v2 = p[(k + 8) * ks], v3 = p[(k + 12) * ks];
+            s += v0; s += v1; s += v2; s += v3;
+        }
+        for (; k < splitK; k += 4) s += p[k * ks];
+    }
     red[threadIdx.x] = s;
     __syncthreads();
     if (g == 0 && i < n) {
@@ -533,12 +541,79 @@
     }
 }
 
+template <int TAPS, int LI>
+__global__ __launch_bounds__(4 * TAPS * LI) void wgrad_reduce_v4_kernel(const float* __restrict__ slab, float* __restrict__ dw,
+                                                                      int splitK, int Cout, int Cin, int out_layout, int accumulate) {
+    constexpr int IB = 4 * LI, NT = 4 * TAPS * LI, U = 8;
+    __shared__ __attribute__((aligned(16))) float red[4 * TAPS * IB];
+    const int64_t n = (int64_t)Cout * Cin;
+    const int64_t i0 = (int64_t)blockIdx.x * IB;
+    const int l = threadIdx.x % LI, t = (threadIdx.x / LI) % TAPS, g = threadIdx.x / (LI * TAPS);
+    const int64_t i = i0 + 4 * l;
+    float4 s = make_float4(0.f, 0.f, 0.f, 0.f);
+    if (i < n) {
+        const float4* p = reinterpret_cast<const float4*>(slab + (int64_t)t * n + i);
+        const int64_t ks = (int64_t)TAPS * n / 4;
+        int k = g;
+        for (; k + 4 * (U - 1) < splitK; k += 4 * U) {
+            float4 v[U];
+#pragma unroll
+            for (int u = 0; u < U; ++u) v[u] = p[(k + 4 * u) * ks];
+#pragma unroll
+            for (int u = 0; u < U; ++u) { s.x += v[u].x; s.y += v[u].y; s.z += v[u].z; s.w += v[u].w; }
+        }
+        for (; k < splitK; k += 4) {
+            const float4 v = p[k * ks];
+            s.x += v.x; s.y += v.y; s.z += v.z; s.w += v.w;
+        }
+    }
+    *reinterpret_cast<float4*>(red + (g * TAPS + t) * IB + 4 * l) = s;
+    __syncthreads();
+    const int64_t left = n - i0;
+    const int ni = left < IB ? (int)left : IB;
+    auto total = [&](int e) {
+        const int ii = e / TAPS, tt = e % TAPS;
+        const float* r = red + tt * IB + ii;
+        return (r[0] + r[TAPS * IB]) + (r[2 * TAPS * IB] + r[3 * TAPS * IB]);
+    };
+    if (out_layout == 0) {
+        float4* o4 = reinterpret_cast<float4*>(dw + i0 * TAPS);
+        for (int q = threadIdx.x; q < ni * TAPS / 4; q += NT) {
+            float4 r = make_float4(total(4 * q), total(4 * q + 1), total(4 * q + 2), total(4 * q + 3));
+            if (accumulate) {
+                const float4 o = o4[q];
+                r.x = o.x + r.x; r.y = o.y + r.y; r.z = o.z + r.z; r.w = o.w + r.w;
+            }
+            o4[q] = r;
+        }
+    } else {
+        const int Ct = Cout / 4;
+        for (int e = threadIdx.x; e < ni; e += NT) {
+            const int64_t ie = i0 + e;
+            const int ci = (int)(ie % Cin), co = (int)(ie / Cin);
+            const int q = co / Ct, cot = co % Ct;
+            const int64_t o = ((int64_t)ci * Ct + cot) * 4 + q;
+            const float r = total(e);
+            dw[o] = accumulate ? dw[o] + r : r;
+        }
+    }
+}
+
 namespace onet {
 int launch_wgrad_reduce(const float* slab, float* dw, int splitK, int taps, int Cout, int Cin, int out_layout, int accumulate,
                         hipStream_t st) {
     const int64_t n = (int64_t)Cout * Cin;
-    hipLaunchKernelGGL(wgrad_reduce_kernel, dim3((unsigned)cdiv(n, 64), (unsigned)taps), dim3(256), 0, st, slab, dw, splitK,
-                       taps, Cout, Cin, out_layout, accumulate);
+    const bool v4 = (n % 4) == 0 && ((reinterpret_cast<uintptr_t>(slab) | reinterpret_cast<uintptr_t>(dw)) & 15) == 0;
+    if (v4 && taps == 9 && out_layout == 0) {
+        hipLaunchKernelGGL((wgrad_reduce_v4_kernel<9, 16>), dim3((unsigned)cdiv(n, 64)), dim3(576), 0, st, slab, dw, splitK, Cout, Cin,
+                           out_layout, accumulate);
+    } else if (v4 && taps == 1) {
+        hipLaunchKernelGGL((wgrad_reduce_v4_kernel<1, 64>), dim3((unsigned)cdiv(n, 256)), dim3(256), 0, st, slab, dw, splitK, Cout, Cin,
+                           out_layout, accumulate);
+    } else {
+        hipLaunchKernelGGL(wgrad_reduce_kernel, dim3((unsigned)cdiv(n, 64), (unsigned)taps), dim3(256), 0, st, slab, dw, splitK,
+                           taps, Cout, Cin, out_layout, accumulate);
+    }
     return check_launch("wgrad_reduce_kernel");
 }
 }
@@ -846,9 +921,7 @@
     }
     int rc = check_launch("conv3x3_stem_wgrad_kernel");
     if (rc) return rc;
-    const int64_t n = (int64_t)Cout * Cin;
-    hipLaunchKernelGGL(wgrad_reduce_kernel, dim3((unsigned)cdiv(n, 64), 9u), dim3(256), 0, st, (const float*)ws, dw, nb, 9, Cout, Cin, 0, accumulate);
-    return check_launch("wgrad_reduce_kernel");
+    return onet::launch_wgrad_reduce((const float*)ws, dw, nb, 9, Cout, Cin, 0, accumulate, st);
 }
 
 int onet_conv_wgrad(const float* x, int64_t x_bs, const float* dz, int64_t dz_bs, float* dw, void* ws,
@@ -872,10 +945,7 @@
         }
         int rc = check_launch("conv3x3_stem_wgrad_kernel");
         if (rc) return rc;
-        const int64_t n = (int64_t)Cout * Cin;
-        hipLaunchKernelGGL(wgrad_reduce_kernel, dim3((unsigned)cdiv(n, 64), 9u), dim3(256), 0, st,
-                           (const float*)ws, dw, nb, 9, Cout, Cin, 0, accumulate);
-        return check_launch("wgrad_reduce_kernel");
+        return onet::launch_wgrad_reduce((const float*)ws, dw, nb, 9, Cout, Cin, 0, accumulate, st);
     }
     int pw;
     wgrad_plan(B, Cin, Cout, H, W, ks, pw, a.splitK, a.stripsX, a.stripsY);
@@ -890,10 +960,7 @@
     }
     int rc = check_launch("conv_wgrad_kernel");
     if (rc) return rc;
-    const int64_t n = (int64_t)Cout * Cin;
-    hipLaunchKernelGGL(wgrad_reduce_kernel, dim3((unsigned)cdiv(n, 64), (unsigned)(ks * ks)), dim3(256), 0, st,
-                       (const float*)ws, dw, a.splitK, ks * ks, Cout, Cin, out_layout, accumulate);
-    return check_launch("wgrad_reduce_kernel");
+    return onet::launch_wgrad_reduce((const float*)ws, dw, a.splitK, ks * ks, Cout, Cin, out_layout, accumulate, st);
 }
 
 int onet_convT2x2_wgrad(const float* x, int64_t x_bs, const float* dy, int64_t dy_bs, float* dw, void* ws,
@@ -919,10 +986,7 @@
     if (pw == 32) launch_wgrad<1, 32, true>(a, blocks, st); else launch_wgrad<1, 16, true>(a, blocks, st);
     int rc = check_launch("conv_wgrad_kernel");
     if (rc) return rc;
-    const int64_t n = (int64_t)Cout * Cin;
-    hipLaunchKernelGGL(wgrad_reduce_kernel, dim3((unsigned)cdiv(n, 64), 1u), dim3(256), 0, st, (const float*)ws, dw,
-                       a.splitK, 1, Cout, Cin, 1, 0);
-    return check_launch("wgrad_reduce_kernel");
-}
-
-}
+    return onet::launch_wgrad_reduce((const float*)ws, dw, a.splitK, 1, Cout, Cin, 1, 0, st);
+}
+
+}
diff --git a/onet_amd/csrc/conv_split.hip b/onet_amd/csrc/conv_split.hip
--- a/onet_amd/csrc/conv_split.hip
+++ b/onet_amd/csrc/conv_split.hip
@@ -45,6 +45,36 @@
     for (int o = 32; o > 0; o >>= 1) m = fmaxf(m, __shfl_xor(m, o, 64));
     if ((threadIdx.x & 63) == 0)
         atomicMax(slots + ((blockIdx.x * (blockDim.x >> 6) + (threadIdx.x >> 6)) & (AMAX_SLOTS - 1)) * AMAX_STRIDE, __builtin_bit_cast(unsigned, m));
+}
+
+__device__ __forceinline__ void pack3x3_split_elem(const float* __restrict__ w, __bf16* __restrict__ wq, int Cout, int Cin, int K, int N,
+                                                   int which, int f16, float wscale, int64_t i) {
+    const int kc = (int)(i & 7);
+    int64_t r = i >> 3;
+    const int nn = (int)(r % N);
+    r /= N;
+    const int half = (int)(r & 1);
+    r >>= 1;
+    const int t = (int)(r % 9), kg = (int)(r / 9);
+    const int k = kg * 16 + half * 8 + kc;
+    float v = 0.f;
+    if (which == 0) v = w[((int64_t)nn * Cin + k) * 9 + t];
+    else if (k < Cout) v = w[((int64_t)k * Cin + nn) * 9 + (8 - t)];
+    const int64_t per_chunk_part = (int64_t)9 * 2 * N * 8;
+    const int64_t within = i - (int64_t)kg * per_chunk_part;
+    if (f16 == 2) {
+        wq[(int64_t)kg * per_chunk_part + within] = (__bf16)v;
+    } else if (f16) {
+        _Float16* wh = reinterpret_cast<_Float16*>(wq);
+        const float vs = v * wscale;
+        const _Float16 hi = (_Float16)vs;
+        wh[((int64_t)kg * 2 + 0) * per_chunk_part + within] = hi;
+        wh[((int64_t)kg * 2 + 1) * per_chunk_part + within] = (_Float16)(vs - (float)hi);
+    } else {
+        const __bf16 hi = (__bf16)v;
+        wq[((int64_t)kg * 2 + 0) * per_chunk_part + within] = hi;
+        wq[((int64_t)kg * 2 + 1) * per_chunk_part + within] = (__bf16)(v - (float)hi);
+    }
 }
 
 __global__ void pack3x3_split_kernel(const float* __restrict__ w, __bf16* __restrict__ wq, int Cout, int Cin, int which, int f16,
@@ -59,33 +89,74 @@
         meta[0] = wscale;
         meta[1] = winv;
     }
-    for (int64_t i = blockIdx.x * (int64_t)blockDim.x + threadIdx.x; i < n; i += (int64_t)gridDim.x * blockDim.x) {
-        const int kc = (int)(i & 7);
-        int64_t r = i >> 3;
-        const int nn = (int)(r % N);
-        r /= N;
-        const int half = (int)(r & 1);
-        r >>= 1;
-        const int t = (int)(r % 9), kg = (int)(r / 9);
-        const int k = kg * 16 + half * 8 + kc;
-        float v = 0.f;
-        if (which == 0) v = w[((int64_t)nn * Cin + k) * 9 + t];
-        else if (k < Cout) v = w[((int64_t)k * Cin + nn) * 9 + (8 - t)];
-        const int64_t per_chunk_part = (int64_t)9 * 2 * N * 8;
-        const int64_t within = i - (int64_t)kg * per_chunk_part;
-        if (f16 == 2) {
-            wq[(int64_t)kg * per_chunk_part + within] = (__bf16)v;
-        } else if (f16) {
-            _Float16* wh = reinterpret_cast<_Float16*>(wq);
-            const float vs = v * wscale;
-            const _Float16 hi = (_Float16)vs;
-            wh[((int64_t)kg * 2 + 0) * per_chunk_part + within] = hi;
-            wh[((int64_t)kg * 2 + 1) * per_chunk_part + within] = (_Float16)(vs - (float)hi);
-        } else {
-            const __bf16 hi = (__bf16)v;
-            wq[((int64_t)kg * 2 + 0) * per_chunk_part + within] = hi;
-            wq[((int64_t)kg * 2 + 1) * per_chunk_part + within] = (__bf16)(v - (float)hi);
-        }
+    for (int64_t i = blockIdx.x * (int64_t)blockDim.x + threadIdx.x; i < n; i += (int64_t)gridDim.x * blockDim.x)
+        pack3x3_split_elem(w, wq, Cout, Cin, K, N, which, f16, wscale, i);
+}
+
+constexpr int WPREP_REC = 12;
+constexpr int WPREP_PACK_CHUNK = 1024;
+constexpr int WPREP_AMAX_CHUNK = 4096;
+
+__device__ __forceinline__ const int64_t* wprep_job(const int64_t* __restrict__ tab, int njobs, int b) {
+    int lo = 0, hi = njobs - 1;
+    while (lo < hi) {
+        const int mid = (lo + hi + 1) >> 1;
+        if (tab[(int64_t)mid * WPREP_REC + 4] <= b) lo = mid; else hi = mid - 1;
+    }
+    return tab + (int64_t)lo * WPREP_REC;
+}
+
+__global__ __launch_bounds__(256) void weights_prepare_absmax_kernel(const int64_t* __restrict__ tab, int njobs, char* __restrict__ arena) {
+    const int64_t* rec = wprep_job(tab, njobs, blockIdx.x);
+    const float* w = reinterpret_cast<const float*>(rec[0]);
+    unsigned* slots = reinterpret_cast<unsigned*>(arena + rec[3]);
+    const int lb = blockIdx.x - (int)rec[4];
+    const int64_t n = rec[10], i0 = (int64_t)lb * WPREP_AMAX_CHUNK;
+    const int64_t i1 = i0 + WPREP_AMAX_CHUNK < n ? i0 + WPREP_AMAX_CHUNK : n;
+    float m = 0.f;
+    for (int64_t i = i0 + threadIdx.x; i < i1; i += 256) m = fmaxf(m, fabsf(w[i]));
+#pragma unroll
+    for (int o = 32; o > 0; o >>= 1) m = fmaxf(m, __shfl_xor(m, o, 64));
+    if ((threadIdx.x & 63) == 0) atomicMax(slots + ((lb * 4 + (threadIdx.x >> 6)) & (AMAX_SLOTS - 1)) * AMAX_STRIDE, __builtin_bit_cast(unsigned, m));
+}
+
+__global__ __launch_bounds__(256) void weights_prepare_pack_kernel(const int64_t* __restrict__ tab, int njobs, char* __restrict__ arena) {
+    const int64_t* rec = wprep_job(tab, njobs, blockIdx.x);
+    const float* w = reinterpret_cast<const float*>(rec[0]);
+    const unsigned* slots = rec[3] >= 0 ? reinterpret_cast<const unsigned*>(arena + rec[3]) : nullptr;
+    const int lb = blockIdx.x - (int)rec[4];
+    const int kind = (int)rec[5], A = (int)rec[6], Bd = (int)rec[7], which = (int)rec[8], fmt = (int)rec[9];
+    const int64_t n = rec[10], i0 = (int64_t)lb * WPREP_PACK_CHUNK;
+    const int64_t i1 = i0 + WPREP_PACK_CHUNK < n ? i0 + WPREP_PACK_CHUNK : n;
+    float winv = 1.f;
+    if (kind == 1) {
+        const int Cout = A, Cin = Bd;
+        const int K = which == 0 ? Cin : ((Cout + 15) / 16) * 16, N = which == 0 ? Cout : Cin;
+        __bf16* wq = reinterpret_cast<__bf16*>(arena + rec[1]);
+        const float wscale = fmt == 1 ? amax_scale(amax_read(slots), true, winv) : 1.f;
+        if (lb == 0 && threadIdx.x == 0) {
+            float* meta = reinterpret_cast<float*>(wq + (fmt == 2 ? 1 : 2) * n);
+            meta[0] = wscale;
+            meta[1] = winv;
+        }
+        for (int64_t i = i0 + threadIdx.x; i < i1; i += 256) pack3x3_split_elem(w, wq, Cout, Cin, K, N, which, fmt, wscale, i);
+    } else {
+        const int Cin = A, Ct = Bd, np = fmt;
+        void* wP = arena + rec[1];
+        void* wdP = rec[2] >= 0 ? arena + rec[2] : nullptr;
+        const int64_t n1 = (int64_t)Cin * 4 * Ct;
+        const float wscale = np == 2 ? amax_scale(amax_read(slots), true, winv) : 1.f;
+        if (np == 2 && lb == 0 && threadIdx.x == 0) {
+            float* meta = reinterpret_cast<float*>(reinterpret_cast<_Float16*>(wP) + 2 * n1);
+            meta[0] = wscale;
+            meta[1] = winv;
+            if (wdP) {
+                float* md = reinterpret_cast<float*>(reinterpret_cast<_Float16*>(wdP) + 2 * n1);
+                md[0] = wscale;
+                md[1] = winv;
+            }
+        }
+        for (int64_t i = i0 + threadIdx.x; i < i1; i += 256) convt_pack_slots_elem(w, wP, wdP, Cin, Ct, np, wscale, i);
     }
 }
 
@@ -2147,6 +2218,64 @@
     return check_launch("pack3x3_split_kernel");
 }
 
+int onet_weights_prepare_batch(const void* table, const int64_t* table_host, int n_amax, int n_pack, int amax_blocks, int pack_blocks,
+                               void* arena, int64_t arena_bytes, int64_t slots_off, int64_t slots_bytes, void* stream) {
+    ONET_REQUIRE(table && table_host && arena && n_amax >= 0 && n_pack > 0 && amax_blocks >= 0 && pack_blocks > 0 && arena_bytes > 0,
+                 "weights_prepare_batch: bad args");
+    ONET_REQUIRE((reinterpret_cast<uintptr_t>(arena) & 15) == 0 && (reinterpret_cast<uintptr_t>(table) & 7) == 0,
+                 "weights_prepare_batch: unaligned arena or table");
+    ONET_REQUIRE(slots_off >= 0 && slots_bytes >= 0 && (slots_off & 15) == 0 && slots_off + slots_bytes <= arena_bytes,
+                 "weights_prepare_batch: magnitude rows outside the arena");
+    const int64_t row = (int64_t)AMAX_SLOTS * AMAX_STRIDE * sizeof(unsigned);
+    for (int j = 0; j < n_amax + n_pack; ++j) {
+        const int64_t* r = table_host + (int64_t)j * WPREP_REC;
+        const bool amax = j < n_amax;
+        const int first = amax ? 0 : n_amax, count = amax ? n_amax : n_pack, total = amax ? amax_blocks : pack_blocks;
+        const int64_t next = j + 1 < first + count ? r[WPREP_REC + 4] : total;
+        const int64_t chunk = amax ? WPREP_AMAX_CHUNK : WPREP_PACK_CHUNK;
+        ONET_REQUIRE(r[0] && (r[0] & 3) == 0 && r[10] > 0, "weights_prepare_batch: job %d: bad weight pointer or size", j);
+        ONET_REQUIRE(r[4] == (j == first ? 0 : r[4 - WPREP_REC] + (r[10 - WPREP_REC] + chunk - 1) / chunk) && next - r[4] == (r[10] + chunk - 1) / chunk,
+                     "weights_prepare_batch: job %d: its blocks [%lld, %lld) do not cover %lld elements exactly once", j, (long long)r[4],
+                     (long long)next, (long long)r[10]);
+        const bool need_row = amax || (r[5] == 1 ? r[9] == 1 : r[9] == 2);
+        ONET_REQUIRE(need_row ? (r[3] >= slots_off && (r[3] - slots_off) % row == 0 && r[3] + row <= slots_off + slots_bytes) : r[3] < 0,
+                     "weights_prepare_batch: job %d: bad magnitude row", j);
+        if (amax) {
+            ONET_REQUIRE(r[5] == 0, "weights_prepare_batch: job %d is not an absmax job", j);
+            continue;
+        }
+        int64_t bytes, items;
+        if (r[5] == 1) {
+            ONET_REQUIRE(r[6] > 0 && r[7] > 0 && (r[8] == 0 || r[8] == 1) && r[9] >= 0 && r[9] <= 2 && (r[8] == 1 || r[7] % 16 == 0) && r[2] < 0,
+                         "weights_prepare_batch: job %d: bad 3x3 pack", j);
+            items = (r[8] == 0 ? r[7] : (r[6] + 15) / 16 * 16) * 9 * (r[8] == 0 ? r[6] : r[7]);
+            bytes = items * (r[9] == 2 ? 2 : 4) + 8;
+        } else {
+            ONET_REQUIRE(r[5] == 2 && r[6] > 0 && r[7] > 0 && r[6] % 8 == 0 && (r[2] < 0 || r[7] % 8 == 0) && (r[9] == 1 || r[9] == 2),
+                         "weights_prepare_batch: job %d: bad ConvTranspose2d pack", j);
+            items = r[6] * 4 * r[7];
+            bytes = items * 2 * r[9] + (r[9] == 2 ? 8 : 0);
+            ONET_REQUIRE(r[2] < 0 || ((r[2] & 15) == 0 && r[2] + bytes <= arena_bytes && (r[2] >= r[1] + bytes || r[2] + bytes <= r[1])),
+                         "weights_prepare_batch: job %d: input-gradient pack outside the arena", j);
+            if (r[2] >= 0) items *= 2;
+        }
+        ONET_REQUIRE(r[10] == items, "weights_prepare_batch: job %d: %lld elements, its shape has %lld", j, (long long)r[10], (long long)items);
+        ONET_REQUIRE(r[1] >= 0 && (r[1] & 15) == 0 && r[1] + bytes <= arena_bytes, "weights_prepare_batch: job %d: pack outside the arena", j);
+    }
+    hipStream_t st = as_stream(stream);
+    const int64_t* tab = reinterpret_cast<const int64_t*>(table);
+    if (n_amax) {
+        ONET_REQUIRE(slots_bytes > 0 && amax_blocks > 0, "weights_prepare_batch: absmax jobs without magnitude rows");
+        (void)hipMemsetAsync((char*)arena + slots_off, 0, (size_t)slots_bytes, st);
+        hipLaunchKernelGGL(weights_prepare_absmax_kernel, dim3((unsigned)amax_blocks), dim3(256), 0, st, tab, n_amax, (char*)arena);
+        int rc = check_launch("weights_prepare_absmax_kernel");
+        if (rc) return rc;
+    }
+    hipLaunchKernelGGL(weights_prepare_pack_kernel, dim3((unsigned)pack_blocks), dim3(256), 0, st, tab + (int64_t)n_amax * WPREP_REC, n_pack,
+                       (char*)arena);
+    return check_launch("weights_prepare_pack_kernel");
+}
+
 int onet_conv3x3_split_fwd(const float* x, int64_t x_bs, const void* wq, int wq_f16, float* z, int64_t z_bs, int B, int Cin, int Cout,
                            int H, int W, void* stream) {
     return split_fwd(x, x_bs, wq, z, z_bs, B, Cin, Cout, H, W, stream, nullptr, wq_f16);
diff --git a/onet_amd/csrc/convt_gemm.hip b/onet_amd/csrc/convt_gemm.hip
--- a/onet_amd/csrc/convt_gemm.hip
+++ b/onet_amd/csrc/convt_gemm.hip
@@ -445,9 +445,18 @@
                                                                  int64_t n4, int accumulate) {
     const int64_t i = blockIdx.x * (int64_t)blockDim.x + threadIdx.x;
     if (i >= n4) return;
-    float4 s = reinterpret_cast<const float4*>(slab)[i];
-    for (int k = 1; k < splitK; ++k) {
-        const float4 v = reinterpret_cast<const float4*>(slab)[(int64_t)k * n4 + i];
+    const float4* p = reinterpret_cast<const float4*>(slab) + i;
+    float4 s = p[0];
+    int k = 1;
+    for (; k + 7 < splitK; k += 8) {
+        float4 v[8];
+#pragma unroll
+        for (int u = 0; u < 8; ++u) v[u] = p[(int64_t)(k + u) * n4];
+#pragma unroll
+        for (int u = 0; u < 8; ++u) { s.x += v[u].x; s.y += v[u].y; s.z += v[u].z; s.w += v[u].w; }
+    }
+    for (; k < splitK; ++k) {
+        const float4 v = p[(int64_t)k * n4];
         s.x += v.x; s.y += v.y; s.z += v.z; s.w += v.w;
     }
     if (accumulate) {
@@ -999,40 +1008,8 @@
             md[1] = winv;
         }
     }
-    for (int64_t i2 = blockIdx.x * (int64_t)blockDim.x + threadIdx.x; i2 < (wdP ? 2 * n : n); i2 += (int64_t)gridDim.x * blockDim.x) {
-        if (i2 >= n) {
-            const int64_t i = i2 - n;
-            const int kc = (int)(i & 7);
-            const int64_t r = i >> 3;
-            const int ci = (int)(r % Cin), ks = (int)(r / Cin);
-            const int c = (ks >> 2) * 8 + kc, q = ks & 3;
-            const float v = w[((int64_t)ci * Ct + c) * 4 + q];
-            if (np == 2) {
-                _Float16* o = reinterpret_cast<_Float16*>(wdP);
-                const float vs = v * wscale;
-                const _Float16 hi = (_Float16)vs;
-                o[(((int64_t)ks * 2 + 0) * Cin + ci) * 8 + kc] = hi;
-                o[(((int64_t)ks * 2 + 1) * Cin + ci) * 8 + kc] = (_Float16)(vs - (float)hi);
-            } else {
-                reinterpret_cast<__bf16*>(wdP)[((int64_t)ks * Cin + ci) * 8 + kc] = (__bf16)v;
-            }
-            continue;
-        }
-        const int64_t i = i2;
-        const int kc = (int)(i & 7);
-        const int64_t r = i >> 3;
-        const int m = (int)(r % M), c8 = (int)(r / M);
-        const float v = w[(int64_t)(c8 * 8 + kc) * M + m];
-        if (np == 2) {
-            _Float16* o = reinterpret_cast<_Float16*>(wP);
-            const float vs = v * wscale;
-            const _Float16 hi = (_Float16)vs;
-            o[(((int64_t)c8 * 2 + 0) * M + m) * 8 + kc] = hi;
-            o[(((int64_t)c8 * 2 + 1) * M + m) * 8 + kc] = (_Float16)(vs - (float)hi);
-        } else {
-            reinterpret_cast<__bf16*>(wP)[((int64_t)c8 * M + m) * 8 + kc] = (__bf16)v;
-        }
-    }
+    for (int64_t i2 = blockIdx.x * (int64_t)blockDim.x + threadIdx.x; i2 < (wdP ? 2 * n : n); i2 += (int64_t)gridDim.x * blockDim.x)
+        convt_pack_slots_elem(w, wP, wdP, Cin, Ct, np, wscale, i2);
 }
 
 __global__ void convt_absmax_kernel(const float* __restrict__ x, int64_t n, unsigned* __restrict__ slots) {
diff --git a/onet_amd/ops.py b/onet_amd/ops.py
--- a/onet_amd/ops.py
+++ b/onet_amd/ops.py
@@ -462,6 +462,7 @@
         self._v = self.w._version
         self._t = [None, None]
         self._s = {}
+        self.used = set()
 
     def _same_weight(self):
         if self.w._version != self._v:
@@ -482,6 +483,7 @@
         return 2
 
     def slots(self, parts):
+        self.used.add((parts, False))
         if parts not in self._s:
             self._same_weight()
             self._s[parts] = packT2x2_slots(self.w, parts, dgrad=bool(CONVT_BWD_SLOTS))
@@ -489,6 +491,7 @@
         return v[0] if isinstance(v, tuple) else v
 
     def dgrad_slots(self, parts):
+        self.used.add((parts, True))
         v = self._s.get(parts)
         if not isinstance(v, tuple):
             self._same_weight()
@@ -637,8 +640,10 @@
     def __init__(self, w):
         super().__init__(Cin=w.shape[1], Cout=w.shape[0])
         self.w = w.detach()
+        self.used = set()
 
     def get_pack(self, algo):
+        self.used.add(algo)
         if algo not in self:
             self[algo] = {"direct": pack3x3, "winograd4": pack3x3_winograd4, "split": pack3x3_split, "plain16": pack3x3_plain16}[algo](self.w)
         return self[algo]
@@ -838,6 +843,141 @@
     return wf, wd
 
 
+WEIGHT_PREP_BATCH = _flag("WEIGHT_PREP_BATCH", True)
+WPREP_REC, WPREP_PACK_CHUNK, WPREP_AMAX_CHUNK = 12, 1024, 4096
+WPREP_ALIGN = 256
+WPREP_ROW = 64 * 32 * 4
+
+
+def weight_prep_plan(layers):
+    import numpy as np
+    rows = [i for i, l in enumerate(layers) if (l[0] == "conv3" and 1 in l[4:6]) or (l[0] == "convt" and l[4] == 2)]
+    row_off = {i: k * WPREP_ROW for k, i in enumerate(rows)}
+    slots_bytes = len(rows) * WPREP_ROW
+    off = -(-slots_bytes // WPREP_ALIGN) * WPREP_ALIGN
+    amax, packs, views = [], [], []
+    ab = pb = 0
+
+    def place(elements):
+        nonlocal off
+        o = off
+        off += -(-elements * 2 // WPREP_ALIGN) * WPREP_ALIGN
+        return o
+
+    for i, l in enumerate(layers):
+        kind, ptr = l[0], int(l[1])
+        if i in row_off:
+            n = l[2] * l[3] * (9 if kind == "conv3" else 4)
+            amax.append([ptr, -1, -1, row_off[i], ab, 0, 0, 0, 0, 0, n, 0])
+            ab += -(-n // WPREP_AMAX_CHUNK)
+        if kind == "conv3":
+            _, _, Cout, Cin, f_fwd, f_dg = l
+            v = []
+            for which, fmt in ((0, f_fwd), (1, f_dg)):
+                if fmt is None:
+                    v.append(None)
+                    continue
+                if which == 0 and Cin % 16:
+                    raise ValueError("weight_prep_plan: a forward pack needs Cin % 16 == 0")
+                n = (Cin if which == 0 else -(-Cout // 16) * 16) * 9 * (Cout if which == 0 else Cin)
+                elements = n * (1 if fmt == 2 else 2) + 8
+                o = place(elements)
+                packs.append([ptr, o, -1, row_off[i] if fmt == 1 else -1, pb, 1, Cout, Cin, which, fmt, n, 0])
+                pb += -(-n // WPREP_PACK_CHUNK)
+                v.append((o, elements, fmt))
+            if v == [None, None]:
+                raise ValueError("weight_prep_plan: a layer without a form")
+        elif kind == "convt":
+            _, _, Cin, Ct, parts, dgrad = l
+            n1 = Cin * 4 * Ct
+            elements = n1 * parts + 4
+            o0 = place(elements)
+            o1 = place(elements) if dgrad else -1
+            n = n1 * (2 if dgrad else 1)
+            packs.append([ptr, o0, o1, row_off[i] if parts == 2 else -1, pb, 2, Cin, Ct, 0, parts, n, 0])
+            pb += -(-n // WPREP_PACK_CHUNK)
+            v = [(o0, elements, parts), (o1, elements, parts) if dgrad else None]
+        else:
+            raise ValueError(f"weight_prep_plan: unknown kind {kind!r}")
+        views.append(v)
+    table = np.asarray(amax + packs, dtype=np.int64).reshape(-1, WPREP_REC)
+    return dict(table=table, n_amax=len(amax), n_pack=len(packs), amax_blocks=ab, pack_blocks=pb, arena_bytes=off,
+                slots_bytes=slots_bytes, views=views)
+
+
+_WPREP_PLANS = {}
+
+
+def weight_prep_run(layers, device):
+    key = (str(device), tuple(layers))
+    hit = _WPREP_PLANS.get(key)
+    if hit is None:
+        if len(_WPREP_PLANS) >= 8:
+            _WPREP_PLANS.clear()
+        plan = weight_prep_plan(layers)
+        hit = _WPREP_PLANS[key] = (plan, torch.from_numpy(plan["table"]).to(device))
+    plan, table = hit
+    arena = torch.empty(plan["arena_bytes"], dtype=torch.uint8, device=device)
+    _lib.call("onet_weights_prepare_batch", _p(table), plan["table"].ctypes.data, plan["n_amax"], plan["n_pack"], plan["amax_blocks"],
+              plan["pack_blocks"], _p(arena), plan["arena_bytes"], 0, plan["slots_bytes"], _stream())
+    out = []
+    for l, v in zip(layers, plan["views"]):
+        half = (lambda fmt: torch.float16 if fmt == 1 else BF) if l[0] == "conv3" else (lambda parts: torch.float16 if parts == 2 else BF)
+        out.append([None if e is None else arena[e[0]:e[0] + 2 * e[1]].view(half(e[2])) for e in v])
+    return out
+
+
+def prepare_weights(model):
+    if not WEIGHT_PREP_BATCH:
+        return 0
+    from .modules import _Packable
+    mods, layers, dev = [], [], None
+    for m in model.modules():
+        old = getattr(m, "_pack", None)
+        if not isinstance(m, _Packable) or old is None:
+            continue
+        w = m.weight
+        if not (w.is_cuda and w.dtype == F32 and w.is_contiguous()) or (dev is not None and w.device != dev):
+            continue
+        if isinstance(old, Packed3x3):
+            for algo in ("split", "plain16"):
+                if algo in old.used and algo in old:
+                    fmts = [None if t is None else (2 if algo == "plain16" else int(t.dtype == torch.float16)) for t in old[algo]]
+                    mods.append((m, algo))
+                    layers.append(("conv3", w.data_ptr(), w.shape[0], w.shape[1], fmts[0], fmts[1]))
+        elif isinstance(old, PackedT):
+            for parts in sorted(p for p, _ in old.used if p in old._s):
+                if (parts, False) not in old.used:
+                    continue
+                mods.append((m, parts))
+                layers.append(("convt", w.data_ptr(), w.shape[0], w.shape[1], parts, (parts, True) in old.used))
+        else:
+            continue
+        dev = w.device if mods and dev is None else dev
+    if not mods:
+        return 0
+    for m, what in mods:
+        old = m._pack
+        if isinstance(old, Packed3x3):
+            old.pop(what, None)
+        elif isinstance(old, PackedT):
+            old._s.pop(what, None)
+    for m, _ in mods:
+        m._pack = None
+    with torch.no_grad():
+        packs = weight_prep_run(layers, dev)
+    for (m, what), l, v in zip(mods, layers, packs):
+        w = m.weight
+        if m._pack is None:
+            m._pack = m._pack_fn(w)
+            m._pack_key = (w.data_ptr(), w._version, str(w.device))
+        if l[0] == "conv3":
+            m._pack[what] = (v[0], v[1])
+        else:
+            m._pack._s[what] = (v[0], v[1]) if v[1] is not None else v[0]
+    return len(mods)
+
+
 class counting_batches:
 
     def __enter__(self):
diff --git a/onet_amd/trainer.py b/onet_amd/trainer.py
--- a/onet_amd/trainer.py
+++ b/onet_amd/trainer.py
@@ -212,14 +212,15 @@
                           g["eps"], g["weight_decay"], n, grad_scale=1.0 / self.world_size)
         torch.autograd.graph.increment_version([p for p in self.params if p.grad is not None])
         invalidate_packed(self.model)
+        ops.prepare_weights(self.model)
 
     def broadcast_params(self, src=0):
         if self.world_size > 1 or (dist.is_available() and dist.is_initialized()):
             dist.broadcast(self.flat, src=src, group=self.pg)
             for b in self.model.buffers():
                 dist.broadcast(b, src=src, group=self.pg)
-            torch.autograd.graph.increment_version(self.params)
-            invalidate_packed(self.model)
+        torch.autograd.graph.increment_version(self.params)
+        invalidate_packed(self.model)
 
 
 def init_distributed(backend: str | None = None):
```

Result: no change. 597.9 (median of 6 runs) (+1.0%).
